# pangenome/gfasort

Measured on AMD Instinct MI355X. Metric: SGD term-updates/sec, -p Y, 1M-node synthetic GFA, higher is better.
Workload: dtype f64

## Files before the change

gfasort_amd/csrc/capi.hip:

```cpp
#include "capi_ctx.h"
#include "index_set.h"
#include "set_seed.h"
#include "set_state_plan.h"

#include <algorithm>
#include <chrono>
#include <cmath>
#include <cstdio>
#include <cstdlib>
#include <cstring>
#include <memory>
#include <new>
#include <numeric>

extern "C" {

const char *gfs_version(void) { return "gfasort_hip 0.1.0 (gfx950)"; }
int gfs_device_count(void) {
    int n = 0;
    if (hipGetDeviceCount(&n) != hipSuccess) return 0;
    return n;
}

int gfs_warmup(int device) {
// ... 39 lines not shown
    c->d_zetas.reset();
    c->d_x.reset();
    c->d_rng.reset();
    c->d_lead.reset();
    c->d_counters.reset();
    c->d_trace.reset();
    c->d_trace_cnt.reset();
    c->d_its.reset();
    c->d_its_all.reset();
    c->d_pool.reset();
    c->configured = false;
}

static int seed_streams(gfs_ctx *c) {
    const uint64_t T = c->shape.n_streams;
    std::vector<uint64_t> st(4 * T);
    for (uint64_t t = 0; t < T; ++t) {
        uint64_t sm = c->params.seed + c->cfg.stream_base + t;
        for (int k = 0; k < 4; ++k) st[(uint64_t)k * T + t] = gfs::splitmix64(sm);
    }
    HIPCHK(hipMemcpy(c->d_rng, st.data(), st.size() * 8, hipMemcpyHostToDevice));
    HIPCHK(hipMemset(c->d_counters, 0, kCounterBytes));
    if (c->d_trace_cnt) HIPCHK(hipMemset(c->d_trace_cnt, 0, T * sizeof(uint32_t)));
    c->events_used = 0; c->kernel_ms_harvested = 0.0; c->iterations = 0; c->total_ms = 0.0;
    return GFS_OK;
}

static int upload_zeta_table(gfs_ctx *c, const gfs_sgd_params *p, const double *zetas) {
    const uint64_t zlen_full = c->shape.zlen_full;
    std::vector<double> ztab;
    if (!zetas) {
        gfs_sgd_params q = *p;
        q.space = gfs::zeta_clamped_space(*p, c->shape.zlen_staged);
        std::vector<double> part(gfs_zeta_table_len(&q));
        gfs_zeta_table(&q, part.data());
        ztab.assign(zlen_full, 0.0);
        std::copy(part.begin(), part.begin() + std::min<size_t>(part.size(), ztab.size()), ztab.begin());
        zetas = ztab.data();
    }
    HIPCHK(c->d_zetas.grow(zlen_full * 8));
    HIPCHK(hipMemcpy(c->d_zetas, zetas, zlen_full * 8, hipMemcpyHostToDevice));
    return GFS_OK;
}

gfs::IterConsts gfs::iter_consts(const gfs_ctx *c, uint64_t k) { return gfs::iter_consts(c->params, c->etas, c->shape, k); }

void gfs::schedule_table(const gfs_sgd_params &p, const std::vector<double> &etas, const gfs::LaunchShape &s, gfs::IterConsts *out) {
    for (uint64_t k = 0; k <= p.iter_max; ++k) out[k] = gfs::iter_consts(p, etas, s, k);
}
static int upload_schedule(gfs_ctx *c) {
    std::vector<gfs::IterConsts> all(c->params.iter_max + 1);
    gfs::schedule_table(c->params, c->etas, c->shape, all.data());
    HIPCHK(hipMemcpy(c->d_its_all, all.data(), all.size() * sizeof(gfs::IterConsts), hipMemcpyHostToDevice));
    return GFS_OK;
}

static const void *iteration_kernel(const gfs::KernelShape &s) {
    if (s.dims == 0) return gfs::iteration_kernel_1d(s);
    if (s.bundle <= 1) return gfs::iteration_kernel_nd(s);
    return s.dims <= 3 ? gfs::iteration_kernel_nd_team(s) : gfs::iteration_kernel_nd_team_wide(s);
}
static const void *fused_kernel(const gfs::KernelShape &s, bool pooled) {
    if (s.dims == 0) return gfs::fused_kernel_1d(s, pooled);
    if (s.bundle <= 1) return gfs::fused_kernel_nd(s, pooled);
    return s.dims <= 3 ? gfs::fused_kernel_nd_team(s, pooled) : gfs::fused_kernel_nd_team_wide(s, pooled);
}
static int resident_blocks_per_cu(const gfs::LaunchShape &s, const void *fn, int *per_cu, std::string *err) {
    hipFuncAttributes attr;
    hipError_t e = hipFuncGetAttributes(&attr, fn);
    if (e != hipSuccess) { *err = std::string("hipFuncGetAttributes(&attr, fn): ") + hipGetErrorString(e); return GFS_E_HIP; }
    e = hipOccupancyMaxActiveBlocksPerMultiprocessor(per_cu, fn, (int)s.block, s.lds_bytes);
    if (e != hipSuccess) { *err = std::string("hipOccupancyMaxActiveBlocksPerMultiprocessor: ") + hipGetErrorString(e); return GFS_E_HIP; }
    return GFS_OK;
}

static hipError_t launch(const gfs_ctx *c, const void *fn, gfs::KArgs &a, const gfs::IterConsts *its, uint32_t n_iters, uint32_t *pool,
                         hipStream_t st) {
    void *args[] = {&a, &its, &n_iters, &pool};
    const gfs::LaunchShape &s = c->shape;
    const dim3 block(s.block), grid((unsigned)((s.n_streams + s.block - 1) / s.block));
    return hipLaunchKernel(fn, grid, block, args, s.lds_bytes, st);
}

static int plan_launches(int cu_count, gfs::LaunchShape &s, LaunchPlan &pl, std::string *err) {
    pl = LaunchPlan{};
    const gfs::KernelShape shape{s.dims, s.bundle, s.lds_tables, s.atomic_loads, s.trace};
    const bool team = s.team, ref = s.bundle == 1;
    const bool free_running = (s.flags & GFS_F_DBG_FREE_RUNNING) != 0;
    pl.iteration = iteration_kernel(shape);
    if (s.phased) pl.window_iteration = iteration_kernel({0, 1, s.lds_tables, s.atomic_loads, s.trace});
    const void *pooled_kernel = s.phased ? gfs::phased_fused_kernel(s.lds_tables) : (team || ref) ? fused_kernel(shape, true) : nullptr;
    const void *free_kernel = team && !s.phased && free_running ? fused_kernel(shape, false) : nullptr;
    if (!pl.iteration || (s.phased && !pl.window_iteration) || ((team || ref) && !pooled_kernel) ||
        (team && !s.phased && free_running && !free_kernel)) {
        *err = "no kernel is built for dims=" + std::to_string(s.dims) + " bundle=" + std::to_string(s.bundle) +
               " lds_tables=" + std::to_string(s.lds_tables) + " atomic_loads=" + std::to_string(s.atomic_loads) +
               " trace=" + std::to_string(s.trace) + " phased=" + std::to_string(s.phased);
        return GFS_E_UNSUPPORTED;
    }
    int per_cu = 0;
    if (team) {
        int rc = resident_blocks_per_cu(s, pooled_kernel, &per_cu, err);
        if (rc) return rc;
    }
    gfs::shape_after_residency(per_cu, gfs::DeviceFacts{cu_count}, &s);
    if (s.fused) pl.fused = s.pooled ? pooled_kernel : free_kernel;
    return GFS_OK;
}

int gfs::plan_setup(const gfs_ctx *c, const gfs_sgd_params *p, int dims, const gfs_launch_config *cfg, const double *etas,
                    gfs::SetupPlan *out, std::string *err) {
    gfs::SetupPlan &sp = *out;
    sp = gfs::SetupPlan{};
    sp.params = *p;
    sp.cfg = cfg ? *cfg : gfs_launch_config{};
    sp.dims = dims;
    sp.rc = GFS_NOTHING_TO_DO;
    if (c->n_nodes == 0) return sp.rc;
    sp.x_len = dims ? c->n_nodes * 2 * (uint64_t)dims : c->n_nodes;
    if (!c->valid_paths) return sp.rc;

    const gfs::GraphFacts graph{c->n_nodes, c->n_steps, c->n_paths, c->max_path_steps, c->valid_paths, c->path_counts.data()};
    int rc = gfs::shape_before_residency(graph, gfs::DeviceFacts{c->cu_count}, p, dims, cfg, &sp.shape, err);
    if (rc) return rc;
    rc = plan_launches(c->cu_count, sp.shape, sp.plan, err);
    if (rc) return rc;
    sp.etas.resize(p->iter_max + 1);
    if (etas) std::copy(etas, etas + p->iter_max + 1, sp.etas.begin());
    else gfs_sgd_schedule(p, sp.etas.data());
    return sp.rc = GFS_OK;
}

void gfs::commit_setup(gfs_ctx *c, gfs::SetupPlan &&sp) {
    const bool has_work = sp.rc == GFS_OK;
    c->params = sp.params; c->cfg = sp.cfg; c->dims = sp.dims; c->x_len = sp.x_len;
    c->shape = has_work ? sp.shape : gfs::LaunchShape{};
    c->plan = has_work ? sp.plan : LaunchPlan{};
    if (!has_work) return;
    c->etas = std::move(sp.etas);
    c->events_used = 0; c->kernel_ms_harvested = 0.0; c->iterations = 0; c->total_ms = 0.0;
}

static int setup_common(gfs_ctx *c, const gfs_sgd_params *p, int dims, const gfs_launch_config *cfg,
                        const double *etas, const double *zetas) {
    if (!c) return fail(GFS_E_ARG, "ctx is null");
    std::string err;
    int rc = gfs::check_setup_args(p, dims, cfg, &err);
    if (rc) return fail(rc, err);
    HIPCHK(hipSetDevice(c->device));
    gfs::free_sgd_state(c);
    gfs::SetupPlan sp;
    const int planned = gfs::plan_setup(c, p, dims, cfg, etas, &sp, &err);
    uint64_t bytes[GFS_STATE_KINDS];
    for (uint32_t k = 0; k < GFS_STATE_KINDS; ++k) bytes[k] = gfs::state_bytes(sp, k);
    gfs::commit_setup(c, std::move(sp));
    if (c->x_len) {
        HIPCHK(c->d_x.grow(bytes[GFS_STATE_POSITIONS]));
        HIPCHK(hipMemset(c->d_x, 0, bytes[GFS_STATE_POSITIONS]));
    }
    if (planned < 0) return fail(planned, err);
    if (planned == GFS_NOTHING_TO_DO) { c->configured = true; return GFS_NOTHING_TO_DO; }

    rc = upload_zeta_table(c, p, zetas);
    if (rc) return rc;
    HIPCHK(c->d_rng.grow(bytes[GFS_STATE_RNG]));
    if (bytes[GFS_STATE_LEAD]) {
        HIPCHK(c->d_lead.grow(bytes[GFS_STATE_LEAD]));
        HIPCHK(hipMemset(c->d_lead, 0, bytes[GFS_STATE_LEAD]));
    }
    HIPCHK(c->d_counters.grow(bytes[GFS_STATE_COUNTERS]));
    if (bytes[GFS_STATE_TRACE]) {
        HIPCHK(c->d_trace.grow(bytes[GFS_STATE_TRACE]));
        HIPCHK(hipMemset(c->d_trace, 0, bytes[GFS_STATE_TRACE]));
        HIPCHK(c->d_trace_cnt.grow(bytes[GFS_STATE_TRACE_COUNTS]));
    }
    rc = seed_streams(c);
    if (rc) return rc;
    if (bytes[GFS_STATE_SCHEDULE]) {
        HIPCHK(c->d_its_all.grow(bytes[GFS_STATE_SCHEDULE]));
        rc = upload_schedule(c);
        if (rc) return rc;
    }
    c->configured = true;
    return GFS_OK;
}

extern "C" {

int gfs_ctx_create(const gfs_graph_view *g, int device, gfs_ctx **out) {
    return gfs_ctx_create_with_layout(g, device, nullptr, out);
}

int gfs_ctx_create_with_layout(const gfs_graph_view *g, int device, const uint32_t *node_perm, gfs_ctx **out) {
    if (!g || !out) return fail(GFS_E_ARG, "null argument");
    *out = nullptr;
    if (int bad = gfs::check_view_counts(g, "")) return bad;
    if (int bad = gfs::check_view_paths(g, "")) return bad;
    int ndev = 0;
    if (hipGetDeviceCount(&ndev) != hipSuccess || ndev == 0)
        return fail(GFS_E_HIP, "no HIP device available (libgfasort_hip has no CPU fallback)");
    if (device < 0 || device >= ndev) return fail(GFS_E_ARG, "bad device index");
    gfs::Laps laps{"gfs_ctx_create", false};
    laps.lap("validate");
    std::unique_ptr<gfs_ctx, decltype(&gfs_ctx_destroy)> owner(new (std::nothrow) gfs_ctx(), gfs_ctx_destroy);
    gfs_ctx *c = owner.get();
    if (!c) return fail(GFS_E_NOMEM, "out of memory");
    c->device = device;
    c->n_nodes = g->n_nodes; c->n_steps = g->n_steps; c->n_paths = g->n_paths;
    hipDeviceProp_t prop;
    if (hipSetDevice(device) != hipSuccess || hipGetDeviceProperties(&prop, device) != hipSuccess)
        return fail(GFS_E_HIP, "hipGetDeviceProperties failed");
    c->cu_count = prop.multiProcessorCount;

    c->perm.assign(g->n_nodes, 0xFFFFFFFFu);
    if (node_perm) {
        std::vector<uint8_t> seen(g->n_nodes, 0);
        for (uint64_t k = 0; k < g->n_nodes; ++k) {
            if (node_perm[k] >= g->n_nodes || seen[node_perm[k]]) return fail(GFS_E_ARG, "node_perm is not a permutation");
            seen[node_perm[k]] = 1; c->perm[k] = node_perm[k];
        }
    }
    if (int bad = gfs::path_facts(g, c, "")) return bad;
    gfs_ctx_set_info info{};
    if (int bad = gfs::build_contexts(&g, &c, 1, c->arena, node_perm, false, &laps, &info)) return bad;
    laps.lap("free tmp");
    *out = owner.release();
    return GFS_OK;
}

void gfs_ctx_destroy(gfs_ctx *c) {
    if (!c || c->set_item) return;
    (void)hipSetDevice(c->device);
    delete c;
// ... 22 lines not shown
    hipError_t e = hipMemcpy(d_stage.p, host, n * 8, hipMemcpyHostToDevice);
    if (e == hipSuccess) e = gfs::reorder_positions_device(d_stage.as<double>(), c->d_x, c->d_perm, c->n_nodes, (uint32_t)c->dims, 1, 0);
    if (e == hipSuccess) e = hipDeviceSynchronize();
    if (e != hipSuccess) return fail(GFS_E_HIP, std::string("upload_positions: ") + hipGetErrorString(e));
    return GFS_OK;
}
int gfs_ctx_init_positions(gfs_ctx *c) {
    if (!c) return fail(GFS_E_ARG, "ctx is null");
    if (!c->d_x || c->dims != 0) return fail(GFS_E_STATE, "needs a 1D context that has been set up");
    HIPCHK(hipSetDevice(c->device));
    HIPCHK(hipDeviceSynchronize());
    hipError_t e = gfs::init_positions_device(c->d_node_len, c->d_perm, c->d_x, c->n_nodes);
    if (e != hipSuccess) return fail(GFS_E_HIP, std::string("init_positions: ") + hipGetErrorString(e));
    return GFS_OK;
}
int gfs_ctx_download_positions(gfs_ctx *c, double *host, uint64_t n) {
    if (!c || !host) return fail(GFS_E_ARG, "null argument");
    if (!c->d_x) return fail(GFS_E_STATE, "context not set up");
    if (n != c->x_len) return fail(GFS_E_ARG, "positions length mismatch");
    HIPCHK(hipSetDevice(c->device));
    HIPCHK(hipDeviceSynchronize());
    gfs::Buffer d_stage;
    if (int rc = d_stage.reserve(n * 8)) return rc;
    hipError_t e = gfs::reorder_positions_device(c->d_x, d_stage.as<double>(), c->d_perm, c->n_nodes, (uint32_t)c->dims, 0, 0);
    if (e == hipSuccess) e = hipMemcpy(host, d_stage.p, n * 8, hipMemcpyDeviceToHost);
    if (e != hipSuccess) return fail(GFS_E_HIP, std::string("download_positions: ") + hipGetErrorString(e));
    return GFS_OK;
}
int gfs_ctx_node_layout(const gfs_ctx *c, uint32_t *perm_out, uint64_t n) {
    if (!c || !perm_out) return fail(GFS_E_ARG, "null argument");
    if (n != c->n_nodes) return fail(GFS_E_ARG, "layout length mismatch");
    std::copy(c->perm.begin(), c->perm.end(), perm_out);
    return GFS_OK;
}
void *gfs_ctx_positions_device(gfs_ctx *c) { return c ? (void *)c->d_x : nullptr; }
int gfs_ctx_bind_positions(gfs_ctx *c, void *device_ptr) {
    if (!c || !device_ptr) return fail(GFS_E_ARG, "null argument");
    if (!c->configured || !c->x_len) return fail(GFS_E_STATE, "context not set up");
    HIPCHK(hipSetDevice(c->device));
    HIPCHK(c->d_x.borrow(device_ptr));
    return GFS_OK;
}
int gfs_ctx_reset_streams(gfs_ctx *c) {
    if (c && c->configured && !c->valid_paths) return GFS_NOTHING_TO_DO;
    if (!c || !c->d_rng) return fail(GFS_E_STATE, "context not set up");
    HIPCHK(hipSetDevice(c->device));
    HIPCHK(hipDeviceSynchronize());
    if (c->d_lead) HIPCHK(hipMemset(c->d_lead, 0, 8 * c->shape.n_streams * sizeof(uint32_t)));
    return seed_streams(c);
}

}

void gfs::fill_kargs(const gfs_ctx *c, gfs::KArgs &a) {
    a.step_rec = c->d_step_rec; a.path_rec = c->d_path_rec; a.path_len = c->d_path_len;
    a.zetas = c->d_zetas; a.x = c->d_x; a.rng = c->d_rng; a.counters = c->d_counters;
    a.trace = c->d_trace; a.trace_cnt = c->d_trace_cnt; a.lead = c->d_lead;
    a.n_steps = c->n_steps;
    const bool wide = gfs::wide_index(c->n_steps, c->cfg.flags);
    a.steps_thresh = wide ? (0ull - c->n_steps) % c->n_steps
                          : (uint64_t)((uint32_t)(0u - (uint32_t)c->n_steps) % (uint32_t)c->n_steps);
    a.n_paths = (uint32_t)c->n_paths;
    a.zlen_full = (uint32_t)c->shape.zlen_full; a.zlen_staged = (uint32_t)c->shape.zlen_staged;
    a.n_streams = (uint32_t)c->shape.n_streams;
    a.quota_base = (uint32_t)(c->shape.quota_total / c->shape.n_streams);
    a.quota_rem = (uint32_t)(c->shape.quota_total % c->shape.n_streams);
    a.attempt_factor = (uint32_t)c->shape.attempt_factor;
    a.trace_per_stream = (uint32_t)c->cfg.trace_per_stream;
    a.space = (uint32_t)std::min<uint64_t>(c->params.space, 0xFFFFFFFFull);
    a.space_max = (uint32_t)std::min<uint64_t>(c->params.space_max, 0xFFFFFFFFull);
    a.space_q = (uint32_t)std::min<uint64_t>(c->params.space_quantization_step, 0xFFFFFFFFull);
    a.dbg = (c->cfg.flags >> 8) & 0x7Fu;
    if (c->cfg.flags & GFS_F_DBG_NO_FUSED_TRIP) a.dbg |= 0x100u;
    a.bundle = c->shape.bundle;
    a.chain = c->shape.chain;
    a.partners = c->shape.partners;
    a.dbg2 = 0;
    if (const char *e = std::getenv("GFS_DBG2")) a.dbg2 = (uint32_t)std::atol(e);
    a.chunk = c->dims ? gfs::ND_TEAM_CHUNK : gfs::TEAM_CHUNK;
    a.ref_chunk = gfs::REF_CHUNK_PER_LANE;
    if (const char *e = std::getenv("GFS_DBG_REF_CHUNK")) { const long v = std::atol(e); if (v >= 1 && v <= 4096) a.ref_chunk = (uint32_t)v; }
    a.n_nodes = (uint32_t)c->n_nodes;
    a.kshift = c->kshift_override >= 0 ? c->kshift_override : gfs::crowd_kshift(c->n_steps, c->shape.n_streams);
}

extern "C" {

static int next_event_pair(gfs_ctx *c, gfs::EventPair *&ev) {
    if (c->events_used == c->events.size()) {
        if (c->events.size() >= 4096) {
            HIPCHK(hipEventSynchronize(c->events.back().e1));
            for (auto &p : c->events) {
                float t = 0.f;
                if (p.elapsed(&t)) c->kernel_ms_harvested += t;
            }
            c->events_used = 0;
        } else {
            c->events.emplace_back();
            if (int rc = c->events.back().ready()) { c->events.pop_back(); return rc; }
        }
    }
    ev = &c->events[c->events_used++];
    return GFS_OK;
}

int gfs_ctx_run_iteration(gfs_ctx *c, uint64_t k, void *hip_stream) {
    if (!c) return fail(GFS_E_ARG, "ctx is null");
    if (!c->configured) return fail(GFS_E_STATE, "context not set up");
    if (!c->valid_paths || c->n_nodes == 0) return GFS_NOTHING_TO_DO;
    if (k > c->params.iter_max) return fail(GFS_E_ARG, "iteration beyond iter_max");
    HIPCHK(hipSetDevice(c->device));
    hipStream_t st = (hipStream_t)hip_stream;
    gfs::KArgs a{};
    fill_kargs(c, a);
    a.it = gfs::iter_consts(c, k);
    const bool window = gfs::in_window(c->shape, k);
    if (window) a.bundle = 1;
    gfs::EventPair *ev = nullptr;
    int rc = next_event_pair(c, ev);
    if (rc) return rc;
    HIPCHK(ev->start(st));
    hipError_t e = launch(c, window ? c->plan.window_iteration : c->plan.iteration, a, nullptr, 0, nullptr, st);
    if (e != hipSuccess) return fail(GFS_E_HIP, std::string("kernel launch: ") + hipGetErrorString(e));
    HIPCHK(ev->stop(st));
    c->iterations++;
    c->launches++;
    return GFS_OK;
}

int gfs_ctx_run_range(gfs_ctx *c, const uint64_t *ks, uint64_t n, void *hip_stream) {
    if (!c || (!ks && n)) return fail(GFS_E_ARG, "null argument");
    if (!c->configured) return fail(GFS_E_STATE, "context not set up");
    if (!c->valid_paths || c->n_nodes == 0) return GFS_NOTHING_TO_DO;
    for (uint64_t i = 0; i < n; ++i) if (ks[i] > c->params.iter_max) return fail(GFS_E_ARG, "iteration beyond iter_max");
    const LaunchPlan &pl = c->plan;
    uint32_t one_chunk = c->shape.one_chunk;
    bool fuse_one = c->shape.fuse_one;
    if (const char *e = std::getenv("GFS_DBG_ONE_CHUNK")) {
        const long v = std::atol(e);
        if (v >= 64 && v <= 4096 && !(v & (v - 1))) { one_chunk = (uint32_t)v; fuse_one = c->shape.fuse_one_probe; }
    }
    if (!pl.fused || n == 0 || (n == 1 && !fuse_one) || n > 0xFFFFFFFFull) {
        for (uint64_t i = 0; i < n; ++i) { int rc = gfs_ctx_run_iteration(c, ks[i], hip_stream); if (rc) return rc; }
        return GFS_OK;
    }
    constexpr uint64_t kMaxFusedIterations = 4096;
    if (n > kMaxFusedIterations) {
        for (uint64_t off = 0; off < n; off += kMaxFusedIterations) {
            const uint64_t m = std::min(kMaxFusedIterations, n - off);
            int rc = m > 1 ? gfs_ctx_run_range(c, ks + off, m, hip_stream) : gfs_ctx_run_iteration(c, ks[off], hip_stream);
            if (rc) return rc;
        }
        return GFS_OK;
    }
    HIPCHK(hipSetDevice(c->device));
    hipStream_t st = (hipStream_t)hip_stream;
    bool consecutive = c->d_its_all != nullptr;
    for (uint64_t i = 1; i < n && consecutive; ++i) consecutive = ks[i] == ks[0] + i;
    const gfs::IterConsts *d_slice = nullptr;
    if (consecutive) {
        d_slice = c->d_its_all + ks[0];
    } else {
        std::vector<gfs::IterConsts> its(n);
        for (uint64_t i = 0; i < n; ++i) its[i] = gfs::iter_consts(c, ks[i]);
        if (int rc = c->d_its.reserve(n * sizeof(gfs::IterConsts))) return rc;
        d_slice = c->d_its.as<gfs::IterConsts>();
        HIPCHK(hipMemcpyAsync(c->d_its.p, its.data(), n * sizeof(gfs::IterConsts), hipMemcpyHostToDevice, st));
        HIPCHK(hipStreamSynchronize(st));
    }
    gfs::KArgs a{};
    fill_kargs(c, a);
    if (n == 1 && c->shape.bundle > 1) a.chunk = one_chunk;
    if (const char *e = std::getenv("GFS_DBG_CHUNK")) {
        const long v = std::atol(e);
        if (c->shape.bundle > 1 && v >= 64 && v <= 16384 && !(v & (v - 1))) a.chunk = (uint32_t)v;
    }
    a.it = gfs::iter_consts(c, ks[0]);
    uint32_t *pool = nullptr;
    if (c->shape.pooled) {
        if (int rc = c->d_pool.reserve(gfs::pool_bytes(n))) return rc;
        pool = c->d_pool.as<uint32_t>();
        HIPCHK(hipMemsetAsync(pool, 0, gfs::pool_bytes(n), st));
    }
    gfs::EventPair *ev = nullptr;
    int rc = next_event_pair(c, ev);
    if (rc) return rc;
    HIPCHK(ev->start(st));
    hipError_t e = launch(c, pl.fused, a, d_slice, (uint32_t)n, pool, st);
    if (e != hipSuccess) return fail(GFS_E_HIP, std::string("fused kernel launch: ") + hipGetErrorString(e));
    HIPCHK(ev->stop(st));
    c->iterations += n;
    c->launches++;
    return GFS_OK;
}

int gfs_ctx_synchronize(gfs_ctx *c, void *hip_stream) {
    if (!c) return fail(GFS_E_ARG, "ctx is null");
    HIPCHK(hipSetDevice(c->device));
    HIPCHK(hipStreamSynchronize((hipStream_t)hip_stream));
    return GFS_OK;
}

int gfs_ctx_run(gfs_ctx *c, void *hip_stream) {
    if (!c) return fail(GFS_E_ARG, "ctx is null");
    if (!c->configured) return fail(GFS_E_STATE, "context not set up");
    if (!c->valid_paths || c->n_nodes == 0) return GFS_NOTHING_TO_DO;
    auto t0 = std::chrono::steady_clock::now();
    {
        std::vector<uint64_t> ks(c->params.iter_max + 1);
        std::iota(ks.begin(), ks.end(), (uint64_t)0);
        int rc = gfs_ctx_run_range(c, ks.data(), ks.size(), hip_stream);
        if (rc) return rc;
    }
    int rc = gfs_ctx_synchronize(c, hip_stream);
    if (rc) return rc;
    c->total_ms += std::chrono::duration<double, std::milli>(std::chrono::steady_clock::now() - t0).count();
    return GFS_OK;
}

int gfs_ctx_stats(gfs_ctx *c, gfs_stats *out) {
    if (!c || !out) return fail(GFS_E_ARG, "null argument");
    std::memset(out, 0, sizeof *out);
    if (!c->d_counters) return GFS_OK;
    HIPCHK(hipSetDevice(c->device));
    HIPCHK(hipDeviceSynchronize());
    std::vector<unsigned long long> cnt(kCounterBytes / 8);
    HIPCHK(hipMemcpy(cnt.data(), c->d_counters, kCounterBytes, hipMemcpyDeviceToHost));
    for (size_t s = 0; s < cnt.size(); s += 8) { out->term_updates += cnt[s]; out->attempts += cnt[s + 1]; }
    out->iterations = c->iterations; out->n_streams = c->shape.n_streams; out->bundle = c->shape.bundle; out->run_trips = c->shape.chain;
    double ms = c->kernel_ms_harvested;
    for (size_t k = 0; k < c->events_used; ++k) {
        float t = 0.f;
        if (c->events[k].elapsed(&t)) ms += t;
    }
    out->kernel_ms = ms; out->total_ms = c->total_ms; out->launches = c->launches;
    return GFS_OK;
}

int gfs_ctx_trace(gfs_ctx *c, gfs_term *out, uint64_t n_terms, uint64_t *counts, uint64_t n_streams) {
    if (!c || !out) return fail(GFS_E_ARG, "null argument");
    if (!c->d_trace) return fail(GFS_E_STATE, "trace_per_stream was 0");
    if (n_terms != c->shape.n_streams * c->cfg.trace_per_stream) return fail(GFS_E_ARG, "trace length mismatch");
    HIPCHK(hipSetDevice(c->device));
    HIPCHK(hipDeviceSynchronize());
    HIPCHK(hipMemcpy(out, c->d_trace, n_terms * sizeof(gfs_term), hipMemcpyDeviceToHost));
    {
        std::vector<uint32_t> inv(c->n_nodes);
        for (uint64_t k = 0; k < c->n_nodes; ++k) inv[c->perm[k]] = (uint32_t)k;
        for (uint64_t t = 0; t < n_terms; ++t) {
            if (c->dims == 0) { if (out[t].d_ij != 0.0) { out[t].i = inv[out[t].i]; out[t].j = inv[out[t].j]; } }
            else if (out[t].d_ij != 0.0) { out[t].i = inv[out[t].i >> 1] * 2 + (out[t].i & 1); out[t].j = inv[out[t].j >> 1] * 2 + (out[t].j & 1); }
        }
    }
    if (counts) {
        if (n_streams != c->shape.n_streams) return fail(GFS_E_ARG, "counts length mismatch");
        std::vector<uint32_t> tmp(c->shape.n_streams);
        HIPCHK(hipMemcpy(tmp.data(), c->d_trace_cnt, tmp.size() * 4, hipMemcpyDeviceToHost));
        for (uint64_t t = 0; t < c->shape.n_streams; ++t) counts[t] = tmp[t];
    }
    return GFS_OK;
}

int gfs_ctx_debug_step_records(const gfs_ctx *c, uint32_t *out, uint64_t n_words) {
    if (!c || !out) return fail(GFS_E_ARG, "null argument");
    if (n_words != 4 * (c->n_steps + 1)) return fail(GFS_E_ARG, "step records length mismatch");
    if (!c->d_step_rec) return fail(GFS_E_STATE, "no step records");
    HIPCHK(hipSetDevice(c->device));
    HIPCHK(hipDeviceSynchronize());
    HIPCHK(hipMemcpy(out, c->d_step_rec, (c->n_steps + 1) * sizeof(uint4), hipMemcpyDeviceToHost));
    return GFS_OK;
}
int gfs_ctx_debug_sgd_state(gfs_ctx *c, uint32_t which, void *out, uint64_t bytes) {
    if (!c) return fail(GFS_E_ARG, "ctx is null");
    const uint32_t kind = which & ~GFS_STATE_SIZE_OF;
    if (kind >= GFS_STATE_KINDS) return fail(GFS_E_ARG, "no such state array");
    if (!c->configured) return fail(GFS_E_STATE, "context not set up");
    const void *arrays[GFS_STATE_KINDS] = {c->d_x.p, c->d_counters.p, c->d_lead.p, c->d_trace.p, c->d_trace_cnt.p, c->d_rng.p, c->d_zetas.p, c->d_its_all.p};
    const uint64_t size = arrays[kind] ? gfs::state_bytes(kind, c->d_rng.p != nullptr, c->x_len, c->shape, c->params, c->cfg) : 0;
    if (which & GFS_STATE_SIZE_OF) {
        if (!out || bytes != sizeof(uint64_t)) return fail(GFS_E_ARG, "the size of a state array is one uint64_t");
        *static_cast<uint64_t *>(out) = size;
        return GFS_OK;
    }
    if (bytes != size) return fail(GFS_E_ARG, "state array length mismatch: it has " + std::to_string(size) + " bytes");
    if (!size) return GFS_OK;
    if (!out) return fail(GFS_E_ARG, "null argument");
    HIPCHK(hipSetDevice(c->device));
    HIPCHK(hipDeviceSynchronize());
    HIPCHK(hipMemcpy(out, arrays[kind], size, hipMemcpyDeviceToHost));
    return GFS_OK;
}
int gfs_ctx_debug_kshift(gfs_ctx *c, int32_t set, int32_t *kshift_out) {
    if (!c) return fail(GFS_E_ARG, "ctx is null");
    if (set >= -1) c->kshift_override = set;
    if (kshift_out) {
        if (!c->configured || !c->shape.n_streams) return fail(GFS_E_STATE, "context not set up");
        gfs::KArgs a{};
        fill_kargs(c, a);
        *kshift_out = a.kshift;
    }
    return GFS_OK;
}

int gfs_ctx_phase_window(gfs_ctx *c, int64_t set_begin, int64_t set_end, uint64_t *begin_out, uint64_t *end_out) {
    if (!c) return fail(GFS_E_ARG, "ctx is null");
    if (!c->configured || !(c->cfg.flags & GFS_F_PHASED)) return fail(GFS_E_STATE, "context not set up with GFS_F_PHASED");
    if (set_begin >= 0 || set_end >= 0) {
        if (set_begin < 0 || set_end < 0 || set_begin > set_end || (uint64_t)set_end > c->params.iter_max + 1)
            return fail(GFS_E_ARG, "phase window: need 0 <= begin <= end <= iter_max + 1");
        if (!c->shape.phased) return fail(GFS_E_STATE, "GFS_F_PHASED is a no-op on this context (the auto policy did not pick bundles of 64)");
        c->shape.win_begin = (uint64_t)set_begin; c->shape.win_end = (uint64_t)set_end;
        if (c->d_its_all) {
            HIPCHK(hipSetDevice(c->device));
            HIPCHK(hipDeviceSynchronize());
            int rc = upload_schedule(c);
            if (rc) return rc;
        }
    }
    if (begin_out) *begin_out = c->shape.win_begin;
    if (end_out) *end_out = c->shape.win_end;
    return GFS_OK;
}

int gfs_ctx_sort_order(gfs_ctx *c, uint64_t *order, uint64_t n) {
    if (!c || (!order && n)) return fail(GFS_E_ARG, "null argument");
    if (!c->d_x || c->dims != 0) return fail(GFS_E_STATE, "needs a 1D context that has been set up");
    if (n != c->n_nodes) return fail(GFS_E_ARG, "order length mismatch");
    HIPCHK(hipSetDevice(c->device));
    HIPCHK(hipDeviceSynchronize());
    gfs::Buffer d_tmp;
    if (int rc = d_tmp.reserve(gfs::sort_order_scratch_bytes(n))) return rc;
    uint32_t *d_order = nullptr;
    hipError_t e = gfs::sort_order_device(c->d_x, c->d_perm, n, 1, d_tmp.p, &d_order);
    if (e != hipSuccess) return fail(GFS_E_HIP, std::string("sort_order_device: ") + hipGetErrorString(e));
    std::vector<uint32_t> tmp(n);
    e = hipMemcpy(tmp.data(), d_order, n * 4, hipMemcpyDeviceToHost);
    if (e != hipSuccess) return fail(GFS_E_HIP, std::string("hipMemcpy order: ") + hipGetErrorString(e));
    for (uint64_t k = 0; k < n; ++k) order[k] = tmp[k];
    return GFS_OK;
}

}

int gfs::check_step_distances(const uint64_t *zs, uint64_t n_z, const gfs_pair_error *out) {
    if ((!zs || !out) && n_z) return fail(GFS_E_ARG, "null argument");
    if (n_z > 65535) return fail(GFS_E_ARG, "at most 65535 step distances per call");
    for (uint64_t k = 0; k < n_z; ++k) if (zs[k] == 0) return fail(GFS_E_ARG, "a step distance of 0");
    return GFS_OK;
}
int gfs::check_diagnosis(uint64_t z, double ratio) {
    if (z == 0) return fail(GFS_E_ARG, "a step distance of 0");
    if (!(ratio >= 0.0)) return fail(GFS_E_ARG, "ratio must be a number >= 0");
    return GFS_OK;
}
gfs_pair_error gfs::unpack_pair_error(uint64_t z, const uint64_t *w) {
    gfs_pair_error o{};
    o.step_distance = z; o.pairs = w[0];
    std::memcpy(&o.sum_rel_sq, &w[1], 8); std::memcpy(&o.max_rel_sq, &w[2], 8);
    std::memcpy(&o.sum_abs, &w[3], 8); std::memcpy(&o.sum_sq, &w[4], 8);
    return o;
}
gfs_sort_quality gfs::unpack_sort_quality(const uint64_t *w) {
    gfs_sort_quality o{w[0], w[1], w[2], 0.0};
    std::memcpy(&o.sq_err_sum, &w[3], 8);
    return o;
}
int gfs::check_sorted_length(uint64_t total_bp, int64_t batch_item) {
    if (total_bp < (1ull << 53)) return GFS_OK;
    return fail(GFS_E_UNSUPPORTED, (batch_item < 0 ? "" : "batch item " + std::to_string(batch_item) + ": ") + "a graph of 2^53 bp or more");
}

extern "C" {

static uint64_t *scratch_words(const gfs_ctx *c, uint64_t part) { return gfs::Region::at<uint64_t>(c->d_quality.p, part); }
static void start_if_timing(gfs::EventPair &timer, hipStream_t st) { if (std::getenv("GFS_TIMING")) (void)timer.start(st); }
static void report_timing(const gfs::EventPair &timer, const char *what, uint64_t count, uint64_t n_steps, const char *before = "z = ", const char *after = "") {
    float ms = 0.f;
    if (timer.elapsed(&ms))
        std::fprintf(stderr, "[%s] %s%llu%s, %llu steps: kernels %.4f ms\n", what, before, (unsigned long long)count, after,
                     (unsigned long long)n_steps, ms);
}

int gfs_ctx_pair_errors(gfs_ctx *c, const uint64_t *zs, uint64_t n_z, gfs_pair_error *out, void *hip_stream) {
    if (!c) return fail(GFS_E_ARG, "ctx is null");
// ... 294 lines not shown
```

gfasort_amd/csrc/capi_ctx.h:

```cpp
#pragma once
#include "../../include/gfasort_hip.h"
#include "device_memory.h"
#include "sgd_kernel_common.h"
#include "launch_policy.h"
#include "sgd_host.h"
#include "readout_region.h"

#include <chrono>
#include <cstdio>
#include <cstdlib>
#include <string>
#include <vector>

static inline int fail(int code, const std::string &msg) { return gfs_set_error(code, msg); }

static_assert(sizeof(gfs_path_error) == 8 * 8, "K7d / K7h write gfs_path_error as 8 words");
static_assert(sizeof(gfs_stretched_pair) == 5 * 8, "K7e / K7i write gfs_stretched_pair as 5 words");
static_assert(sizeof(gfs_node_error) == 3 * 8, "K7f / K7j write gfs_node_error as 3 words");

static constexpr size_t kCounterBytes = gfs::COUNTER_SLOTS * 8 * sizeof(unsigned long long);

struct LaunchPlan {
    const void *iteration = nullptr;
    const void *window_iteration = nullptr;
    const void *fused = nullptr;
};

struct gfs_ctx {
    int device = 0;
    int cu_count = 0;
    uint64_t n_nodes = 0, n_steps = 0, n_paths = 0;
    uint32_t max_path_steps = 0;
    bool valid_paths = false;
    bool set_item = false;
    std::vector<uint32_t> path_counts;
    std::vector<uint32_t> perm;
    gfs::Buffer arena;
    gfs::Array<uint4> d_step_rec;
    gfs::Array<uint4> d_path_rec;
    gfs::Array<uint64_t> d_path_len;
    gfs::Array<uint32_t> d_perm;
    gfs::Array<uint32_t> d_node_len;
    int dims = 0;
    bool configured = false;
    gfs_sgd_params params{};
    gfs_launch_config cfg{};
    std::vector<double> etas;
    gfs::Array<double> d_zetas;
    gfs::Array<double> d_x; uint64_t x_len = 0;
    gfs::Array<uint64_t> d_rng;
    gfs::Array<uint32_t> d_lead;
    gfs::Array<unsigned long long> d_counters;
    gfs::Array<gfs_term> d_trace; gfs::Array<uint32_t> d_trace_cnt;
    gfs::Buffer d_its;
    gfs::Array<gfs::IterConsts> d_its_all;
    gfs::Buffer d_pool;
    gfs::LaunchShape shape;
    LaunchPlan plan;
    int32_t kshift_override = -1;
    gfs::Buffer d_quality;
    std::vector<gfs::EventPair> events;
    size_t events_used = 0;
    double kernel_ms_harvested = 0.0;
    uint64_t iterations = 0;
    uint64_t launches = 0;
    double total_ms = 0.0;
};

namespace gfs {
static inline int check_view_counts(const gfs_graph_view *g, const std::string &prefix) {
    if (g->n_steps > (1ull << 40)) return fail(GFS_E_UNSUPPORTED, prefix + "more than 2^40 path steps");
    if (g->n_nodes > 0x7FFFFFFFull) return fail(GFS_E_UNSUPPORTED, prefix + "more than 2^31-1 nodes");
    if (g->n_paths > 0x7FFFFFFFull) return fail(GFS_E_UNSUPPORTED, prefix + "more than 2^31-1 paths");
    if (g->n_steps && (!g->step_node || !g->step_is_rev)) return fail(GFS_E_ARG, prefix + "null step arrays");
    if (!g->path_first_step) return fail(GFS_E_ARG, prefix + "null path_first_step");
    if (g->n_nodes && !g->node_len) return fail(GFS_E_ARG, prefix + "null node_len");
    return GFS_OK;
}
static inline int check_view_paths(const gfs_graph_view *g, const std::string &prefix) {
    if (g->path_first_step[0] != 0 || g->path_first_step[g->n_paths] != g->n_steps)
        return fail(GFS_E_ARG, prefix + "path_first_step must start at 0 and end at n_steps");
    for (uint64_t p = 0; p < g->n_paths; ++p)
        if (g->path_first_step[p + 1] < g->path_first_step[p]) return fail(GFS_E_ARG, prefix + "path_first_step not monotone");
    return GFS_OK;
}
static inline int path_facts(const gfs_graph_view *g, gfs_ctx *c, const std::string &prefix) {
    c->path_counts.reserve(g->n_paths);
    for (uint64_t p = 0; p < g->n_paths; ++p) {
        const uint64_t b = g->path_first_step[p], e = g->path_first_step[p + 1];
        if (e - b > 0xFFFFFFFFull) return fail(GFS_E_UNSUPPORTED, prefix + "a path with more than 2^32-1 steps");
        const uint32_t cnt = (uint32_t)(e - b);
        c->path_counts.push_back(cnt);
        if (cnt > 1) c->valid_paths = true;
        if (cnt > c->max_path_steps) c->max_path_steps = cnt;
    }
    uint32_t max_len = 0;
    for (uint64_t k = 0; k < g->n_nodes; ++k) if (g->node_len[k] > max_len) max_len = g->node_len[k];
    for (uint64_t p = 0; p < g->n_paths; ++p) {
        const uint64_t b = g->path_first_step[p], e = g->path_first_step[p + 1];
        if ((unsigned __int128)(e - b) * max_len < ((unsigned __int128)1 << 55)) continue;
        unsigned __int128 bp = 0;
        for (uint64_t s = b; s < e; ++s) { const uint32_t n = g->step_node[s]; if (n < g->n_nodes) bp += g->node_len[n]; }
        if (bp >= ((unsigned __int128)1 << 55)) return fail(GFS_E_UNSUPPORTED, prefix + "a path of 2^55 bp or more");
    }
    return GFS_OK;
}
}

namespace gfs {
struct Laps {
    const char *tag;
    bool cumulative;
    bool on = std::getenv("GFS_TIMING") != nullptr;
    std::chrono::steady_clock::time_point t = std::chrono::steady_clock::now();
    void lap(const char *what) {
        if (!on) return;
        const auto now = std::chrono::steady_clock::now();
        std::fprintf(stderr, cumulative ? "[%s] %-10s %8.2f ms\n" : "[%s] %-12s %8.2f ms\n", tag, what,
                     std::chrono::duration<double, std::milli>(now - t).count());
        if (!cumulative) t = now;
    }
// ... 50 lines not shown
```

gfasort_amd/csrc/capi_set.hip:

```cpp
#include "capi_ctx.h"
#include "index_set.h"
#include "set_seed.h"
#include "set_state_plan.h"

#include <algorithm>
#include <chrono>
#include <cstring>
#include <memory>
#include <new>

struct gfs_ctx_set {
    int device = 0;
    gfs::Buffer arena;
    gfs::Buffer state_arena;
    gfs::Buffer h_stage{true};
    std::vector<std::unique_ptr<gfs_ctx>> items;
    gfs_ctx_set_info info{};
    gfs_ctx_set_setup_info setup_info{};
};

namespace {
constexpr int KINDS = gfs::SET_KINDS;
std::string item_prefix(uint64_t i) { return "set item " + std::to_string(i) + ": "; }
}

int gfs::build_contexts(const gfs_graph_view *const *graphs, gfs_ctx *const *ctxs, uint64_t n, gfs::Buffer &arena, const uint32_t *node_perm,
                        bool staged, gfs::Laps *laps, gfs_ctx_set_info *info) {
    const std::string set = staged ? "set " : "";
    auto lap = [laps](const char *what) { if (laps && laps->on) { (void)hipDeviceSynchronize(); laps->lap(what); } };
    int rc = GFS_OK;
    auto ok = [&rc, &set](const char *call, const char *what, hipError_t err) {
        if (err != hipSuccess) rc = fail(GFS_E_HIP, std::string(call) + " " + set + what + ": " + hipGetErrorString(err));
        return err == hipSuccess;
    };
    std::vector<uint64_t> counts(3 * n), offsets(KINDS * n);
    uint64_t N = 0, S = 0, P = 0;
    for (uint64_t i = 0; i < n; ++i) {
        counts[i] = ctxs[i]->n_nodes; counts[n + i] = ctxs[i]->n_steps; counts[2 * n + i] = ctxs[i]->n_paths;
        N += ctxs[i]->n_nodes; S += ctxs[i]->n_steps; P += ctxs[i]->n_paths;
    }
    const uint64_t arena_bytes = gfs::set_arena_plan(counts.data(), counts.data() + n, counts.data() + 2 * n, n, offsets.data());
    const uint64_t perm_begin = offsets[3], nlen_begin = offsets[4];
    const uint64_t perm_bytes = nlen_begin - perm_begin, nlen_bytes = arena_bytes - nlen_begin;

    const gfs::SetInputHead in = gfs::set_input_head(S, P, n);
    uint64_t work_bytes = 0;
    hipError_t e = gfs::index_set_work_bytes(N, S, &work_bytes);
    if (e != hipSuccess) return fail(GFS_E_HIP, std::string("rocPRIM temporary storage: ") + hipGetErrorString(e));
    gfs::Buffer h_stage{true}, d_scratch;
    if ((rc = arena.reserve(std::max<uint64_t>(arena_bytes, 256), ("hipMalloc " + set + "arena").c_str()))) return rc;
    if ((rc = d_scratch.reserve(in.bytes + work_bytes, ("hipMalloc " + set + "scratch").c_str()))) return rc;
    if (staged && (rc = h_stage.reserve(std::max(in.bytes + nlen_bytes, perm_bytes), "hipHostMalloc set staging"))) return rc;
    info->device_allocations = staged ? 3 : 2;
    if (!ok("hipMemset", "arena", hipMemsetAsync(arena.p, 0, std::max<uint64_t>(arena_bytes, 256), 0))) return rc;
    ++info->launches;

    std::vector<gfs::SetItem> items(n + 1);
    uint64_t node_off = 0, step_off = 0, path_off = 0;
    for (uint64_t i = 0; i <= n; ++i) {
        items[i] = gfs::SetItem{node_off, step_off, path_off, 0, 0, 0, 0, 0};
        if (i == n) break;
        const uint64_t *at = &offsets[KINDS * i];
        items[i].rec = at[0]; items[i].prec = at[1]; items[i].plen = at[2]; items[i].perm = at[3]; items[i].nlen = at[4];
        node_off += ctxs[i]->n_nodes; step_off += ctxs[i]->n_steps; path_off += ctxs[i]->n_paths;
    }
    unsigned char *h = h_stage.as<unsigned char>(), *d_in = d_scratch.as<unsigned char>(), *d_arena = arena.as<unsigned char>();
    if (staged) {
        auto *h_step_node = reinterpret_cast<uint32_t *>(h);
        auto *h_first = reinterpret_cast<uint64_t *>(h + in.at_first);
        uint8_t *h_rev = h + in.at_rev;
        unsigned char *h_nlen = h + in.bytes;
        std::memset(h_nlen, 0, nlen_bytes);
        for (uint64_t i = 0; i < n; ++i) {
            const gfs_graph_view *g = graphs[i];
            const gfs::SetItem &it = items[i];
            if (g->n_steps) {
                std::memcpy(h_step_node + it.step_off, g->step_node, g->n_steps * 4);
                std::memcpy(h_rev + it.step_off, g->step_is_rev, g->n_steps);
            }
            for (uint64_t p = 0; p < g->n_paths; ++p) h_first[it.path_off + p] = it.step_off + g->path_first_step[p];
            if (g->n_nodes) std::memcpy(h_nlen + (it.nlen - nlen_begin), g->node_len, g->n_nodes * 4);
        }
        h_first[P] = S;
        std::memcpy(h + in.at_items, items.data(), items.size() * sizeof(gfs::SetItem));
        if (!ok("hipMemcpy", "inputs", hipMemcpyAsync(d_in, h, in.bytes, hipMemcpyHostToDevice, 0))) return rc;
        if (nlen_bytes && !ok("hipMemcpy", "node_len", hipMemcpyAsync(d_arena + nlen_begin, h_nlen, nlen_bytes, hipMemcpyHostToDevice, 0))) return rc;
    } else {
        const gfs_graph_view *g = graphs[0];
        if (N && !ok("hipMemcpy", "node_len", hipMemcpy(d_arena + nlen_begin, g->node_len, N * 4, hipMemcpyHostToDevice))) return rc;
        if (S && !ok("hipMemcpy", "step_node", hipMemcpy(d_in, g->step_node, S * 4, hipMemcpyHostToDevice))) return rc;
        if (!ok("hipMemcpy", "path_first", hipMemcpy(d_in + in.at_first, g->path_first_step, (P + 1) * 8, hipMemcpyHostToDevice))) return rc;
        if (!ok("hipMemcpy", "item table", hipMemcpy(d_in + in.at_items, items.data(), items.size() * sizeof(gfs::SetItem), hipMemcpyHostToDevice))) return rc;
        if (S && !ok("hipMemcpy", "step_is_rev", hipMemcpy(d_in + in.at_rev, g->step_is_rev, S, hipMemcpyHostToDevice))) return rc;
        if (N && node_perm && !ok("hipMemcpy", "perm", hipMemcpy(d_arena + perm_begin, ctxs[0]->perm.data(), N * 4, hipMemcpyHostToDevice))) return rc;
    }
    lap("step upload");

    gfs::SetUnion u{};
    u.n_items = (uint32_t)n; u.n_nodes = N; u.n_steps = S; u.n_paths = P;
    u.step_node = reinterpret_cast<const uint32_t *>(d_in);
    u.path_first = reinterpret_cast<const uint64_t *>(d_in + in.at_first);
    u.items = reinterpret_cast<const gfs::SetItem *>(d_in + in.at_items);
    u.step_is_rev = d_in + in.at_rev;
    u.arena = d_arena;
    uint32_t bad_item = gfs::SET_NO_BAD_ITEM;
    e = gfs::index_set_layout_device(u, d_in + in.bytes, node_perm != nullptr, &bad_item, &info->launches);
    lap("node layout");
    if (e == hipSuccess && bad_item == gfs::SET_NO_BAD_ITEM) e = gfs::index_set_records_device(u, d_in + in.bytes, &info->launches);
    if (e != hipSuccess || bad_item != gfs::SET_NO_BAD_ITEM) (void)hipDeviceSynchronize();
    if (e != hipSuccess) return fail(GFS_E_HIP, std::string("build_index_set: ") + hipGetErrorString(e));
    if (bad_item != gfs::SET_NO_BAD_ITEM) return fail(GFS_E_ARG, (staged ? item_prefix(bad_item) : "") + "step_node out of range");
    if (staged) {
        if (!ok("hipMemcpy", "perm", hipMemcpy(h, d_arena + perm_begin, std::max<uint64_t>(perm_bytes, 4), hipMemcpyDeviceToHost))) return rc;
    } else if (N && !node_perm) {
        if (!ok("hipMemcpy", "perm", hipMemcpy(ctxs[0]->perm.data(), d_arena + perm_begin, N * 4, hipMemcpyDeviceToHost))) return rc;
    }
    if ((e = hipDeviceSynchronize()) != hipSuccess) return fail(GFS_E_HIP, std::string("hipDeviceSynchronize: ") + hipGetErrorString(e));
    lap("K3");
    for (uint64_t i = 0; i < n; ++i) {
        gfs_ctx *c = ctxs[i];
        const uint64_t *at = &offsets[KINDS * i];
        if (staged) {
            const uint32_t *perm = reinterpret_cast<const uint32_t *>(h + (at[3] - perm_begin));
            c->perm.assign(perm, perm + c->n_nodes);
        }
        (void)c->d_step_rec.borrow(d_arena + at[0]);
        (void)c->d_path_rec.borrow(d_arena + at[1]);
        (void)c->d_path_len.borrow(d_arena + at[2]);
        (void)c->d_perm.borrow(d_arena + at[3]);
        (void)c->d_node_len.borrow(d_arena + at[4]);
    }
    info->items = n; info->total_nodes = N; info->total_steps = S; info->total_paths = P;
    info->arena_bytes = arena_bytes;
    return GFS_OK;
}

static int set_setup(gfs_ctx_set *s, const std::vector<const gfs_sgd_params *> &params, const std::vector<int> &dims,
                     const gfs_launch_config *cfgs, int32_t *item_rc) {
    const auto t0 = std::chrono::steady_clock::now();
    const uint64_t n = s->items.size();
    std::string err;
    for (uint64_t i = 0; i < n; ++i) {
        if (dims[i] < 0) return fail(GFS_E_UNSUPPORTED, item_prefix(i) + "dimensions must be 1..8");
        if (int rc = gfs::check_setup_args(params[i], dims[i], cfgs ? &cfgs[i] : nullptr, &err)) return fail(rc, item_prefix(i) + err);
    }
    HIPCHK(hipSetDevice(s->device));

    std::vector<gfs::SetupPlan> plans(n);
    for (uint64_t i = 0; i < n; ++i) {
        const int rc = gfs::plan_setup(s->items[i].get(), params[i], dims[i], cfgs ? &cfgs[i] : nullptr, nullptr, &plans[i], &err);
        if (rc < 0) return fail(rc, item_prefix(i) + err);
    }
    constexpr int K = gfs::SET_STATE_KINDS;
    std::vector<uint64_t> bytes(K * n), offsets(K * n);
    gfs_ctx_set_setup_info info{};
    info.items = n;
    std::vector<gfs::SeedItem> seeds;
    std::vector<uint64_t> seed_of;
    uint64_t total_blocks = 0;
    for (uint64_t i = 0; i < n; ++i) {
        const gfs::SetupPlan &sp = plans[i];
        for (int k = 0; k < K; ++k) bytes[K * i + k] = gfs::state_bytes(sp, (uint32_t)k);
        if (sp.rc != GFS_OK) { ++info.nothing_to_do; continue; }
        ++info.configured;
        info.total_streams += sp.shape.n_streams;
        seeds.push_back(gfs::SeedItem{nullptr, sp.params.seed + sp.cfg.stream_base, (uint32_t)sp.shape.n_streams, (uint32_t)total_blocks});
        seed_of.push_back(i);
        total_blocks += (sp.shape.n_streams + gfs::SEED_BLOCK - 1) / gfs::SEED_BLOCK;
        if (total_blocks > 0x7FFFFFFFull) return fail(GFS_E_UNSUPPORTED, "set items 0.." + std::to_string(i) + " have more streams together than one seeding launch holds");
    }
    const uint64_t arrays_end = gfs::set_state_plan(bytes.data(), n, offsets.data());
    const uint64_t zero_end = gfs::set_state_kind_begin(offsets.data(), GFS_STATE_RNG);
    const uint64_t upload_begin = gfs::set_state_kind_begin(offsets.data(), GFS_STATE_ZETAS);
    const uint64_t seeds_at = arrays_end, blocks_at = seeds_at + gfs::round256(seeds.size() * sizeof(gfs::SeedItem));
    const uint64_t arena_bytes = blocks_at + gfs::round256(total_blocks * sizeof(uint32_t)), stage_bytes = arena_bytes - upload_begin;
    info.state_bytes = arena_bytes;

    HIPCHK(hipDeviceSynchronize());
    for (auto &c : s->items) gfs::free_sgd_state(c.get());
    int rc = GFS_OK;
    auto ok = [&rc, s](const char *what, hipError_t e) {
        if (e == hipSuccess) return true;
        (void)hipDeviceSynchronize();
        s->state_arena.reset();
        rc = fail(GFS_E_HIP, std::string(what) + ": " + hipGetErrorString(e));
        return false;
    };
    if (s->state_arena.bytes < arena_bytes) {
        ++info.device_allocations;
        if ((rc = s->state_arena.reserve(arena_bytes, "hipMalloc set state arena"))) return rc;
    }
    if (s->h_stage.bytes < stage_bytes) {
        ++info.device_allocations;
        if ((rc = s->h_stage.reserve(stage_bytes, "hipHostMalloc set state staging"))) { s->state_arena.reset(); return rc; }
    }
    unsigned char *d_arena = s->state_arena.as<unsigned char>(), *h = s->h_stage.as<unsigned char>();
    auto staged = [h, upload_begin](uint64_t arena_offset) { return h + (arena_offset - upload_begin); };

    if (stage_bytes) std::memset(h, 0, stage_bytes);
    {
        std::vector<gfs_sgd_params> clamped(n);
// ... 158 lines not shown
```

gfasort_amd/csrc/index_set.h:

```cpp
#pragma once
#include "index_set_plan.h"
#include <hip/hip_runtime.h>
#include <stdint.h>

namespace gfs {

struct SetItem {
    uint64_t node_off, step_off, path_off;
    uint64_t rec, prec, plen, perm, nlen;
};
static_assert(sizeof(SetItem) == SET_ITEM_BYTES, "the item table of the input head (index_set_plan.h)");

struct SetUnion {
    uint32_t n_items;
    uint64_t n_nodes, n_steps, n_paths;
    const SetItem *items;
    const uint32_t *step_node;
    const uint8_t *step_is_rev;
    const uint64_t *path_first;
    unsigned char *arena;
};

constexpr uint32_t SET_NO_BAD_ITEM = 0xFFFFFFFFu;
constexpr unsigned SET_STEP_BLOCKS = 2048, SET_NODE_BLOCKS = 1024, SET_PATH_BLOCKS = 64, SET_BLOCK = 256;

hipError_t index_set_work_bytes(uint64_t n_nodes, uint64_t n_steps, uint64_t *bytes);
hipError_t index_set_layout_device(const SetUnion &u, void *d_work, bool layout_given, uint32_t *bad_item, uint64_t *launches);
hipError_t index_set_records_device(const SetUnion &u, void *d_work, uint64_t *launches);
hipError_t warm_module_index_set();

}
```

gfasort_amd/csrc/index_set_kernels.hip:

```cpp
#include "index_set.h"
#include "device_memory.h"
#include <hip/hip_runtime.h>
#include <algorithm>
#include <stdint.h>
#include <type_traits>
#include <rocprim/device/device_radix_sort.hpp>
#include <rocprim/device/device_scan.hpp>
#include <rocprim/iterator/counting_iterator.hpp>
#include <rocprim/iterator/transform_iterator.hpp>

namespace gfs {

constexpr uint32_t NO_NODE_U32 = 0xFFFFFFFFu;
constexpr unsigned KEY_BITS = 43;
constexpr int JUMP_ROUNDS = 40, JUMP_CHUNK = 4;

__host__ __device__ __forceinline__ uint32_t item_of(const SetItem *items, uint32_t n_items, uint64_t v, uint64_t SetItem::*off) {
    uint32_t lo = 0, hi = n_items;
    while (hi - lo > 1) { const uint32_t mid = lo + ((hi - lo) >> 1); if (items[mid].*off <= v) lo = mid; else hi = mid; }
    return lo;
}
__host__ __device__ __forceinline__ uint32_t path_of(const uint64_t *path_first, uint32_t n_paths, uint64_t s) {
    uint32_t lo = 0, hi = n_paths;
    while (hi - lo > 1) { const uint32_t mid = lo + ((hi - lo) >> 1); if (path_first[mid] <= s) lo = mid; else hi = mid; }
// ... 26 lines not shown
        ids[v] = (uint32_t)v;
    }
}
__global__ void set_run_up_kernel(SetUnion u, const unsigned long long *first, uint32_t *up) {
    const uint64_t stride = (uint64_t)gridDim.x * blockDim.x;
    for (uint64_t v = (uint64_t)blockIdx.x * blockDim.x + threadIdx.x; v < u.n_nodes; v += stride) {
        const unsigned long long f = first[v];
        uint32_t w = (uint32_t)v;
        if (f != ~0ull && !set_is_path_start(u.path_first, (uint32_t)u.n_paths, f)) {
            const uint32_t p = u.step_node[f - 1];
            if (p != NO_NODE_U32) {
                const uint64_t q = u.items[item_of(u.items, u.n_items, v, &SetItem::node_off)].node_off + p;
                if (first[q] == f - 1) w = (uint32_t)q;
            }
        }
        up[v] = w;
    }
}
__global__ void set_jump_kernel(const uint32_t *in, uint32_t *out, uint64_t n_nodes, uint32_t *changed) {
    const uint64_t stride = (uint64_t)gridDim.x * blockDim.x;
    for (uint64_t v = (uint64_t)blockIdx.x * blockDim.x + threadIdx.x; v < n_nodes; v += stride) {
        const uint32_t a = in[v], b = in[a];
        out[v] = b;
        if (b != a) *changed = 1;
    }
}
__global__ void set_anchor_kernel(SetUnion u, const unsigned long long *first, const uint32_t *head, uint32_t *anc) {
    const uint64_t stride = (uint64_t)gridDim.x * blockDim.x;
    for (uint64_t v = (uint64_t)blockIdx.x * blockDim.x + threadIdx.x; v < u.n_nodes; v += stride) {
        uint32_t a = (uint32_t)v;
        if (first[v] != ~0ull) {
            const unsigned long long fh = first[head[v]];
            if (!set_is_path_start(u.path_first, (uint32_t)u.n_paths, fh)) {
                const uint32_t p = u.step_node[fh - 1];
                if (p != NO_NODE_U32) a = (uint32_t)(u.items[item_of(u.items, u.n_items, v, &SetItem::node_off)].node_off + p);
            }
        }
        anc[v] = a;
    }
}
__global__ void set_branch_key_kernel(SetUnion u, const unsigned long long *first, const uint32_t *root, const uint32_t *ids_by_first,
                                      unsigned long long *key) {
    const uint64_t stride = (uint64_t)gridDim.x * blockDim.x;
    for (uint64_t r = (uint64_t)blockIdx.x * blockDim.x + threadIdx.x; r < u.n_nodes; r += stride) {
        const uint32_t v = ids_by_first[r];
        const unsigned long long f = first[v];
        const uint32_t t = root[v];
        key[r] = f == ~0ull ? unvisited_key(u.items, item_of(u.items, u.n_items, v, &SetItem::node_off))
                            : (t == v ? 4ull * (f + 1ull) : 4ull * (first[t] + 1ull) + 1ull);
    }
}
__global__ void set_scatter_rank_kernel(SetUnion u, const uint32_t *sorted_node) {
    const uint64_t stride = (uint64_t)gridDim.x * blockDim.x;
    for (uint64_t r = (uint64_t)blockIdx.x * blockDim.x + threadIdx.x; r < u.n_nodes; r += stride) {
        const uint64_t v = sorted_node[r];
        const SetItem it = u.items[item_of(u.items, u.n_items, v, &SetItem::node_off)];
        reinterpret_cast<uint32_t *>(u.arena + it.perm)[v - it.node_off] = (uint32_t)(r - it.node_off);
    }
}

struct SetStepLen {
    SetUnion u;
    __host__ __device__ uint64_t operator()(uint64_t s) const {
        if (s >= u.n_steps) return 0;
        const uint32_t n = u.step_node[s];
        if (n == NO_NODE_U32) return 0ull;
        const SetItem &it = u.items[item_of(u.items, u.n_items, s, &SetItem::step_off)];
        return (uint64_t)reinterpret_cast<const uint32_t *>(u.arena + it.nlen)[n];
    }
};
__global__ void set_node_stats_kernel(SetUnion u, uint32_t *cnt, uint32_t *rep) {
    const uint64_t stride = (uint64_t)gridDim.x * blockDim.x;
    for (uint64_t s = (uint64_t)blockIdx.x * blockDim.x + threadIdx.x; s < u.n_steps; s += stride) {
        const uint32_t n = u.step_node[s];
        if (n == NO_NODE_U32) continue;
        const uint64_t v = u.items[item_of(u.items, u.n_items, s, &SetItem::step_off)].node_off + n;
        atomicAdd(&cnt[v], 1u);
        const uint64_t begin = u.path_first[path_of(u.path_first, (uint32_t)u.n_paths, s)], from = s - begin > 63 ? s - 63 : begin;
        uint32_t c = 1;
        for (uint64_t t = from; t < s; ++t) c += u.step_node[t] == n;
        if (c > 1 && rep[v] < c) atomicMax(&rep[v], c);
    }
}
__global__ void set_fill_records_kernel(SetUnion u, const uint64_t *scan, const uint32_t *cnt, const uint32_t *rep) {
    const uint64_t stride = (uint64_t)gridDim.x * blockDim.x;
    for (uint64_t s = (uint64_t)blockIdx.x * blockDim.x + threadIdx.x; s < u.n_steps; s += stride) {
        const uint32_t p = path_of(u.path_first, (uint32_t)u.n_paths, s);
        const SetItem it = u.items[item_of(u.items, u.n_items, s, &SetItem::step_off)];
        const uint64_t pos = scan[s] - scan[u.path_first[p]];
        const uint32_t n = u.step_node[s];
        uint4 r;
        r.x = n == NO_NODE_U32 ? NO_NODE_U32 : reinterpret_cast<const uint32_t *>(u.arena + it.perm)[n];
        uint32_t crowd = 0;
        if (n != NO_NODE_U32) {
            const uint32_t a = set_ceil_log2(cnt[it.node_off + n]), b = set_ceil_log2(rep[it.node_off + n]);
            crowd = ((a > 63u ? 63u : a) << 23) | ((b > 7u ? 7u : b) << 29);
        }
        r.y = (uint32_t)(p - it.path_off) | ((uint32_t)(u.step_is_rev[s] & 1) << 31);
        r.z = (uint32_t)pos; r.w = ((uint32_t)(pos >> 32) & 0x7FFFFFu) | crowd;
        reinterpret_cast<uint4 *>(u.arena + it.rec)[s - it.step_off] = r;
    }
}
__global__ void set_paths_kernel(SetUnion u, const uint64_t *scan) {
    const uint64_t stride = (uint64_t)gridDim.x * blockDim.x, total = u.n_paths + u.n_items;
    for (uint64_t t = (uint64_t)blockIdx.x * blockDim.x + threadIdx.x; t < total; t += stride) {
        if (t >= u.n_paths) {
            const uint32_t i = (uint32_t)(t - u.n_paths);
            reinterpret_cast<uint4 *>(u.arena + u.items[i].rec)[u.items[i + 1].step_off - u.items[i].step_off] = make_uint4(0, 0, 0, 0);
            continue;
        }
        const SetItem it = u.items[item_of(u.items, u.n_items, t, &SetItem::path_off)];
        const uint64_t fb = u.path_first[t], fe = u.path_first[t + 1], b = fb - it.step_off;
        const uint32_t c = (uint32_t)(fe - fb);
        reinterpret_cast<uint4 *>(u.arena + it.prec)[t - it.path_off] = make_uint4((uint32_t)b, c, c ? (uint32_t)(0u - c) % c : 0u, (uint32_t)(b >> 32));
        reinterpret_cast<uint64_t *>(u.arena + it.plen)[t - it.path_off] = scan ? scan[fe] - scan[fb] : 0ull;
    }
}

namespace {
struct Work {
    unsigned long long *first, *key_a, *key_b;
    uint32_t *ids_a, *ids_b, *a, *b, *cnt, *rep;
    uint64_t *scan;
    uint32_t *flags;
    void *tmp;
    size_t tmp_bytes;
    uint64_t cnt_rep_bytes, bytes;
};
hipError_t plan_work(uint64_t N, uint64_t S, void *d_work, Work &w) {
    size_t sort_tmp = 0, scan_tmp = 0;
    hipError_t e = hipSuccess;
    if (N) e = rocprim::radix_sort_pairs(nullptr, sort_tmp, (uint64_t *)nullptr, (uint64_t *)nullptr, (uint32_t *)nullptr, (uint32_t *)nullptr,
                                         (size_t)N, 0, KEY_BITS, 0);
    if (e != hipSuccess) return e;
    if (S) {
        auto lens = rocprim::make_transform_iterator(rocprim::counting_iterator<uint64_t>(0), SetStepLen{SetUnion{}});
        e = rocprim::exclusive_scan(nullptr, scan_tmp, lens, (uint64_t *)nullptr, (uint64_t)0, (size_t)(S + 1), rocprim::plus<uint64_t>(), 0);
        if (e != hipSuccess) return e;
    }
    const uintptr_t base = reinterpret_cast<uintptr_t>(d_work);
    uint64_t at = 0;
    auto take = [&at, base](auto *&piece, uint64_t bytes) {
        piece = reinterpret_cast<std::remove_reference_t<decltype(piece)>>(base + at);
        at += round256(bytes ? bytes : 1);
    };
    take(w.first, N * 8); take(w.key_a, N * 8); take(w.key_b, N * 8);
    take(w.ids_a, N * 4); take(w.ids_b, N * 4); take(w.a, N * 4); take(w.b, N * 4);
    take(w.cnt, N * 4); take(w.rep, N * 4);
    w.cnt_rep_bytes = round256(N ? N * 4 : 1) + N * 4;
    take(w.scan, S ? (S + 1) * 8 : 0);
    take(w.flags, (1 + 2 * JUMP_ROUNDS) * sizeof(uint32_t));
    w.tmp_bytes = std::max(sort_tmp, scan_tmp);
    take(w.tmp, w.tmp_bytes);
    w.bytes = at;
    return hipSuccess;
}
const dim3 over_steps(SET_STEP_BLOCKS), over_nodes(SET_NODE_BLOCKS), block(SET_BLOCK);
}

hipError_t index_set_work_bytes(uint64_t n_nodes, uint64_t n_steps, uint64_t *bytes) {
    Work w{};
    const hipError_t e = plan_work(n_nodes, n_steps, nullptr, w);
    *bytes = w.bytes;
    return e;
}

hipError_t index_set_layout_device(const SetUnion &u, void *d_work, bool layout_given, uint32_t *bad_item, uint64_t *launches) {
    *bad_item = SET_NO_BAD_ITEM;
    const uint64_t N = u.n_nodes, S = u.n_steps;
    Work w{};
    hipError_t e = plan_work(N, S, d_work, w);
    if (e != hipSuccess) return e;
    if ((e = hipMemsetAsync(w.flags, 0xFF, sizeof(uint32_t), 0)) != hipSuccess) return e;
    if ((e = hipMemsetAsync(w.flags + 1, 0, 2 * JUMP_ROUNDS * sizeof(uint32_t), 0)) != hipSuccess) return e;
    *launches += 2;
    if (N) {
        if ((e = hipMemsetAsync(w.first, 0xFF, N * 8, 0)) != hipSuccess) return e;
        ++*launches;
    }
    if (S) {
        hipLaunchKernelGGL(set_first_visit_kernel, over_steps, block, 0, 0, u, w.first, w.flags);
        ++*launches;
        if ((e = hipMemcpy(bad_item, w.flags, sizeof(uint32_t), hipMemcpyDeviceToHost)) != hipSuccess) return e;
        if (*bad_item != SET_NO_BAD_ITEM) return hipSuccess;
    }
    if (!N || layout_given) return hipGetLastError();
    hipLaunchKernelGGL(set_first_key_kernel, over_nodes, block, 0, 0, u, w.first, w.key_a, w.ids_a);
    e = rocprim::radix_sort_pairs(w.tmp, w.tmp_bytes, (uint64_t *)w.key_a, (uint64_t *)w.key_b, w.ids_a, w.ids_b, (size_t)N, 0, KEY_BITS, 0);
    *launches += 2;
    if (e != hipSuccess) return e;
    uint32_t *d_ids = w.ids_b, *d_ids_other = w.ids_a;
    if (S) {
        uint32_t *d_a = w.a, *d_b = w.b;
        auto jump_to_fixpoint = [&](uint32_t *&cur, uint32_t *&other, uint32_t *flags) -> hipError_t {
            for (int round = 0; round < JUMP_ROUNDS; round += JUMP_CHUNK) {
                for (int k = 0; k < JUMP_CHUNK; ++k) {
                    hipLaunchKernelGGL(set_jump_kernel, over_nodes, block, 0, 0, cur, other, N, flags + round + k);
                    std::swap(cur, other);
                }
                *launches += JUMP_CHUNK;
                uint32_t changed[JUMP_CHUNK];
                const hipError_t err = hipMemcpy(changed, flags + round, sizeof changed, hipMemcpyDeviceToHost);
                if (err != hipSuccess) return err;
                if (std::find(changed, changed + JUMP_CHUNK, 0u) != changed + JUMP_CHUNK) break;
            }
            return hipSuccess;
        };
        hipLaunchKernelGGL(set_run_up_kernel, over_nodes, block, 0, 0, u, w.first, d_a);
        ++*launches;
        if ((e = jump_to_fixpoint(d_a, d_b, w.flags + 1)) != hipSuccess) return e;
        hipLaunchKernelGGL(set_anchor_kernel, over_nodes, block, 0, 0, u, w.first, d_a, d_b);
        std::swap(d_a, d_b);
        ++*launches;
        if ((e = jump_to_fixpoint(d_a, d_b, w.flags + 1 + JUMP_ROUNDS)) != hipSuccess) return e;
        hipLaunchKernelGGL(set_branch_key_kernel, over_nodes, block, 0, 0, u, w.first, d_a, d_ids, w.key_a);
        e = rocprim::radix_sort_pairs(w.tmp, w.tmp_bytes, (uint64_t *)w.key_a, (uint64_t *)w.key_b, d_ids, d_ids_other, (size_t)N, 0, KEY_BITS, 0);
        *launches += 2;
        if (e != hipSuccess) return e;
        std::swap(d_ids, d_ids_other);
    }
    hipLaunchKernelGGL(set_scatter_rank_kernel, over_nodes, block, 0, 0, u, d_ids);
    ++*launches;
    return hipGetLastError();
}

hipError_t index_set_records_device(const SetUnion &u, void *d_work, uint64_t *launches) {
    const uint64_t N = u.n_nodes, S = u.n_steps;
    Work w{};
    hipError_t e = plan_work(N, S, d_work, w);
    if (e != hipSuccess) return e;
    if (S) {
        auto lens = rocprim::make_transform_iterator(rocprim::counting_iterator<uint64_t>(0), SetStepLen{u});
        e = rocprim::exclusive_scan(w.tmp, w.tmp_bytes, lens, w.scan, (uint64_t)0, (size_t)(S + 1), rocprim::plus<uint64_t>(), 0);
        if (e != hipSuccess) return e;
        if ((e = hipMemsetAsync(w.cnt, 0, w.cnt_rep_bytes, 0)) != hipSuccess) return e;
        hipLaunchKernelGGL(set_node_stats_kernel, over_steps, block, 0, 0, u, w.cnt, w.rep);
        hipLaunchKernelGGL(set_fill_records_kernel, over_steps, block, 0, 0, u, w.scan, w.cnt, w.rep);
        *launches += 4;
    }
    hipLaunchKernelGGL(set_paths_kernel, dim3(SET_PATH_BLOCKS), block, 0, 0, u, S ? w.scan : (const uint64_t *)nullptr);
    ++*launches;
    return hipGetLastError();
}

hipError_t warm_module_index_set() {
    hipFuncAttributes attr;
    return hipFuncGetAttributes(&attr, reinterpret_cast<const void *>(&set_paths_kernel));
}

}
```

gfasort_amd/csrc/launch_policy.h:

```cpp
#pragma once
#include "../../include/gfasort_hip.h"
#include "sgd_limits.h"

#include <algorithm>
#include <cmath>
#include <cstdint>
#include <string>
#include <vector>

namespace gfs {

struct GraphFacts {
    uint64_t n_nodes = 0, n_steps = 0, n_paths = 0;
    uint32_t max_path_steps = 0;
    bool valid_paths = false;
    const uint32_t *path_counts = nullptr;
};
struct DeviceFacts { int cu_count = 0; };

struct LaunchShape {
    int dims = 0;
    uint32_t flags = 0;
    bool trace = false, explicit_streams = false;
    uint32_t block = 256;
    uint64_t n_streams = 0, quota_total = 0, attempt_factor = 0;
    uint32_t bundle = 1;
    uint32_t partners = 1;
    uint32_t chain = 1;
    bool phased = false;
    uint64_t win_begin = 0, win_end = 0;
    bool lds_tables = true, atomic_loads = true;
    size_t lds_bytes = 0;
    uint64_t zlen_full = 0, zlen_staged = 0;
    bool team = false;
    uint64_t fused_resident_blocks = 0;
    bool fused = false;
    bool pooled = false;
    bool fuse_one = false;
    bool fuse_one_probe = false;
    uint32_t one_chunk = 0;
};

inline bool has_fused_team_kernel(int dims, uint32_t bundle) { return (dims == 0 && bundle >= 16) || (dims >= 2 && bundle == 64); }

inline int check_setup_args(const gfs_sgd_params *p, int dims, const gfs_launch_config *cfg, std::string *err) {
    if (!p) { *err = "params is null"; return GFS_E_ARG; }
    if (!(p->theta >= 0.0 && p->theta < 1.0)) { *err = "theta must be in [0,1)"; return GFS_E_ARG; }
    if (p->space_quantization_step == 0) { *err = "space_quantization_step must be > 0"; return GFS_E_ARG; }
    if (!(p->eta_max > 0.0)) { *err = "eta_max must be > 0"; return GFS_E_ARG; }
    if (dims < 0 || dims > GFS_MAX_DIMS) { *err = "dimensions must be 1..8"; return GFS_E_UNSUPPORTED; }
    if (cfg && (cfg->flags & GFS_F_PHASED)) {
        if (dims != 0) { *err = "GFS_F_PHASED is a sampler of the 1D sort: layouts have none"; return GFS_E_ARG; }
        const uint32_t b = (cfg->flags >> 16) & 0xFFu;
        if (b != 0 && b != 64) { *err = "GFS_F_PHASED switches between reference streams and bundles of 64: GFS_F_BUNDLE must be 0 or 64"; return GFS_E_ARG; }
    }
    return GFS_OK;
}

inline uint64_t auto_stream_count(const GraphFacts &g, const DeviceFacts &dev, int dims, uint64_t quota_total, bool team) {
    const uint64_t chip = (uint64_t)dev.cu_count * ((team && dims == 0) ? 1024 : (team && dims >= 2) ? 256u * (unsigned)nd_team_waves(dims) : 976);
    const uint64_t by_work = ((quota_total + 7) / 8 + 63) / 64 * 64;
    const uint64_t by_nodes = (team ? g.n_nodes * 3 / 4 : g.n_nodes / 4) / 64 * 64;
    return std::max<uint64_t>(64, std::min(chip, std::min(by_work, by_nodes)));
}

inline int choose_bundle(const GraphFacts &g, int dims, uint32_t flags, LaunchShape *s, std::string *err) {
    uint32_t b = (flags >> 16) & 0xFFu;
    const bool b_auto = b == 0;
    if (b > 1 && (s->n_streams % 64 != 0 || (b != 4 && b != 8 && b != 16 && b != 32 && b != 64))) {
        *err = "bundled sampling needs n_streams % 64 == 0 and a bundle of 4, 8, 16, 32 or 64"; return GFS_E_ARG;
    }
    if (b > 1 && dims != 0 && b == 4) { *err = "bundled layout kernels exist for 1..8 dimensions and bundles of 8..64"; return GFS_E_UNSUPPORTED; }
    if (b == 0) {
        b = 1;
        if (s->n_streams % 64 == 0 && dims <= 3 && g.n_nodes >= 16384) {
            for (uint32_t cand : {64u, 32u, 16u, 8u, 4u}) {
                if (cand == 4u && dims != 0) continue;
                uint64_t long_steps = 0;
                for (uint64_t p = 0; p < g.n_paths; ++p) if (g.path_counts[p] >= 4 * cand) long_steps += g.path_counts[p];
                if ((double)long_steps >= 0.95 * (double)g.n_steps) { b = cand; break; }
            }
        }
    }
    s->bundle = b;
    uint32_t k = (flags >> 24) & 0xFFu;
    if (k > 64 || (k & (k - 1))) { *err = "GFS_F_CHAIN: the run length in trips must be a power of two <= 64"; return GFS_E_ARG; }
    const bool k_auto = k == 0;
    if (k == 0) k = dims ? 16 : 64;
    s->partners = (b == 64 && has_fused_team_kernel(dims, b) && !(flags & GFS_F_ONE_PARTNER)) ? 2u : 1u;
    if (k_auto && b_auto && b == 64) while (k > 1 && s->quota_total / (64ull * k * s->partners) < 64) k >>= 1;
    s->chain = b == 64 ? k : 1;
    return GFS_OK;
}

inline int shape_before_residency(const GraphFacts &g, const DeviceFacts &dev, const gfs_sgd_params *p, int dims, const gfs_launch_config *cfg_in,
                                  LaunchShape *shape, std::string *err) {
    int rc = check_setup_args(p, dims, cfg_in, err);
    if (rc) return rc;
    if (g.n_nodes == 0 || !g.valid_paths) return GFS_NOTHING_TO_DO;
    const gfs_launch_config cfg = cfg_in ? *cfg_in : gfs_launch_config{};
    LaunchShape s;
    s.dims = dims; s.flags = cfg.flags; s.trace = cfg.trace_per_stream != 0; s.explicit_streams = cfg.n_streams != 0;

    s.zlen_full = gfs_zeta_table_len(p);
    if (s.zlen_full > 0xFFFFFFFFull) { *err = "zeta table too long"; return GFS_E_UNSUPPORTED; }
    const uint64_t maxjump = std::min<uint64_t>(p->space, g.max_path_steps ? g.max_path_steps - 1 : 0);
    const uint64_t last_idx = maxjump > p->space_max
                                  ? p->space_max + (maxjump - p->space_max) / p->space_quantization_step + 1
                                  : maxjump;
    s.zlen_staged = std::min<uint64_t>(last_idx + 1, s.zlen_full);

    s.quota_total = cfg.term_updates_per_iteration ? cfg.term_updates_per_iteration : p->min_term_updates;
    s.block = cfg.block_size ? cfg.block_size : 256;
    if (s.block % 64 || s.block > 1024) { *err = "block_size must be a multiple of 64, <= 1024"; return GFS_E_ARG; }
    s.n_streams = cfg.n_streams ? cfg.n_streams : auto_stream_count(g, dev, dims, s.quota_total, false);
    if (s.n_streams > 0x7FFFFFFFull) { *err = "n_streams too large"; return GFS_E_ARG; }
    if (s.quota_total / s.n_streams + 1 > 0xFFFFFFFFull) { *err = "per-stream quota exceeds 2^32"; return GFS_E_UNSUPPORTED; }
    s.attempt_factor = cfg.attempt_factor ? cfg.attempt_factor : 64;
    if (s.attempt_factor > 0xFFFFFFFFull) { *err = "attempt_factor too large"; return GFS_E_ARG; }
    rc = choose_bundle(g, dims, cfg.flags, &s, err);
    if (rc) return rc;
    if (!cfg.n_streams && s.bundle > 1) s.n_streams = auto_stream_count(g, dev, dims, s.quota_total, true);
    if (cfg.flags & GFS_F_PHASED) {
        s.phased = s.bundle == 64;
        if (s.phased) gfs_phase_window(p, &s.win_begin, &s.win_end);
        else if (s.bundle == 1) { s.win_begin = 0; s.win_end = p->iter_max + 1; }
    }
    if (dims != 0 && s.bundle > 1 && s.block > 256) { *err = "the layout team kernels are built for workgroups of at most 256 lanes"; return GFS_E_ARG; }
    s.atomic_loads = !(cfg.flags & GFS_F_PLAIN_LOADS);
    const size_t lds = (size_t)g.n_paths * 16 + (size_t)s.zlen_staged * 8;
    s.lds_tables = !(cfg.flags & GFS_F_NO_LDS_TABLES) && lds <= 48 * 1024;
    s.lds_bytes = s.lds_tables ? lds : 0;
    s.team = has_fused_team_kernel(dims, s.bundle);
    *shape = s;
    return GFS_OK;
}

inline void shape_after_residency(int per_cu, const DeviceFacts &dev, LaunchShape *shape) {
    LaunchShape &s = *shape;
    const bool ref = s.bundle == 1;
    const bool free_running = (s.flags & GFS_F_DBG_FREE_RUNNING) != 0;
    s.fused_resident_blocks = 0;
    if (s.team) {
        s.fused_resident_blocks = (uint64_t)std::max(per_cu, 0) * dev.cu_count;
        const uint64_t resident = s.fused_resident_blocks * s.block;
        if (!s.explicit_streams && s.n_streams > resident && resident >= 64) s.n_streams = resident;
    }
    const uint64_t n_waves = (s.n_streams + 63) / 64;
    const bool pool_ok = n_waves <= 0xFFFFFFFFull &&
                         s.quota_total / (s.dims != 0 && s.bundle > 1 ? 1u : pool_slots((uint32_t)n_waves)) < (1ull << 31);
    const bool team_fusable = s.team && (s.phased ? pool_ok && !free_running : pool_ok || free_running) &&
                              (s.n_streams + s.block - 1) / s.block <= s.fused_resident_blocks;
    s.pooled = pool_ok && !(free_running && s.bundle > 1);
    s.fused = (team_fusable || (ref && pool_ok)) && s.atomic_loads && !s.trace && !(s.flags & GFS_F_NO_FUSE);
    s.one_chunk = s.dims ? ND_TEAM_CHUNK : TEAM_CHUNK;
    s.fuse_one_probe = team_fusable && pool_ok;
    s.fuse_one = s.fuse_one_probe && s.dims != 0 && s.quota_total / n_waves >= 4ull * s.one_chunk;
}

inline bool in_window(const LaunchShape &s, uint64_t k) { return s.phased && k >= s.win_begin && k < s.win_end; }

inline IterConsts iter_consts(const gfs_sgd_params &p, const std::vector<double> &etas, const LaunchShape &s, uint64_t k) {
    IterConsts it;
    double fc = std::floor(p.cooling_start * (double)p.iter_max);
    uint64_t first_cooling = !(fc > 0.0) ? 0 : (fc >= 18446744073709551616.0 ? UINT64_MAX : (uint64_t)fc);
    bool cooling = k > first_cooling;
    double theta = cooling ? 0.001 : p.theta;
    it.eta = etas[k];
    it.cooling = cooling ? 1 : 0;
    it.zeta2theta = 1.0 + gfs_fast_precise_pow(0.5, theta);
    double omt = 1.0 - theta;
    it.omt_e = h_sat_i32(omt); it.omt_fb = omt - (double)it.omt_e;
    double alpha = 1.0 / (1.0 - theta);
    it.alpha_e = h_sat_i32(alpha); it.alpha_fb = alpha - (double)it.alpha_e;
    it._pad = in_window(s, k) ? 1 : 0;
    return it;
}

inline int32_t crowd_kshift(uint64_t n_steps, uint64_t n_streams) {
    const uint64_t per = n_steps / std::max<uint64_t>(2 * n_streams, 1);
    int lg = 0; while (lg < 63 && (per >> (lg + 1)) != 0) ++lg;
    return lg + 2;
}

inline bool wide_index(uint64_t n_steps, uint32_t flags) { return n_steps > 0xFFFFFFFFull || (flags & GFS_F_DBG_WIDE_INDEX); }

inline bool batch_eligible(const LaunchShape &s, bool trace, bool has_resident_schedule, bool idle) {
    return !idle && s.bundle == 1 && !s.phased && s.fused && s.pooled && !trace && has_resident_schedule;
}

}
```

gfasort_amd/csrc/sgd_1d.h:

```cpp
#pragma once
#include "sgd_kernel_common.h"

namespace gfs {

struct RefTerm1D { uint32_t i, j; int crowd; double term_dist; };

template <bool LDS_TABLES>
__device__ __forceinline__ bool ref_sample_1d(const KArgs &a, const uint4 *path_tab, const double *zeta_tab, Rng &rng,
                                              const uint64_t step_idx, const uint4 &ra, RefTerm1D &t) {
    uint4 rb; uint64_t sa, sb; uint32_t cnt, path;
    if (!sample_pair_from<LDS_TABLES>(a, path_tab, zeta_tab, rng, step_idx, ra, rb, sa, sb, cnt, path)) return false;
    t.term_dist = fabs(rec_pos(ra) - rec_pos(rb));
    if (t.term_dist == 0.0) return false;
    t.crowd = crowd_shift<false>(a, ra, rb);
    t.i = ra.x; t.j = rb.x;
    return t.i != 0xFFFFFFFFu && t.j != 0xFFFFFFFFu;
}

template <bool LDS_TABLES, bool ATOMIC_LOADS, bool TRACE>
__device__ __forceinline__ void ref_run_1d(const KArgs &a, const uint4 *path_tab, const double *zeta_tab, Rng &rng,
                                           const uint32_t quota, const uint64_t max_att, const uint32_t tid,
                                           uint32_t &done, uint32_t &att, uint32_t &ntr) {
    double *x = a.x;
    uint32_t d = 0; uint64_t t = 0;
    uint64_t s_a = 0; uint4 r_a = make_uint4(0, 0, 0, 0); bool drawn = false;
    while (d < quota && t < max_att) {
        ++t;
        if (!drawn) { s_a = sample_step(a, rng); r_a = a.step_rec[s_a]; }
        drawn = false;
        RefTerm1D cur;
        if (!ref_sample_1d<LDS_TABLES>(a, path_tab, zeta_tab, rng, s_a, r_a, cur)) continue;
        const double mu = crowd_scale(fmin(a.it.eta * (1.0 / cur.term_dist), 1.0), cur.crowd);
        double dx;
        if (a.dbg & 2u) dx = (double)cur.i - (double)cur.j;
        else dx = load_pos<ATOMIC_LOADS>(x + cur.i) - load_pos<ATOMIC_LOADS>(x + cur.j);
        if (dx == 0.0) dx = 1e-9;
        const double mag = fabs(dx);
        const double delta = mu * (mag - cur.term_dist) / 2.0;
        const double r = delta / mag;
        const double r_x = r * dx;
        if (d + 1u < quota && t < max_att) { s_a = sample_step(a, rng); r_a = a.step_rec[s_a]; drawn = true; }
        if (a.dbg & 1u) { asm volatile("" :: "v"(r_x)); }
        else {
            add_pos(x + cur.i, -r_x);
            add_pos(x + cur.j, r_x);
        }
        ++d;
        if (TRACE) record_trace(a, tid, ntr, cur.i, cur.j, cur.term_dist);
    }
    done += d;
    att += t > 0xFFFFFFFFull ? 0xFFFFFFFFu : (uint32_t)t;
}

struct TeamState {
    Rng rng;
    Leader L = {0, 0, 0, 0, 0, 0, 0, 0};
    uint32_t left = 0, cool = 0, colour = 0, seg = 0;
    uint32_t p = 0;
    uint32_t done = 0, att = 0, ntr = 0;
};

struct Trip {
    uint64_t sa = 0, sb = 0;
    uint4 ra = make_uint4(0, 0, 0, 0), rb = make_uint4(0, 0, 0, 0);
    uint4 rc = make_uint4(0, 0, 0, 0);
    bool twin = false;
    bool valid = false;
    int mshift = 0;
    bool two = false;
    bool fused = false;
    uint32_t k = 1;
    uint32_t off = 0;
};

template <int B>
__device__ __forceinline__ void expand_trip(const KArgs &a, const Leader &L, int t, uint32_t seg, uint32_t p, uint32_t colour, int sub, int q, Trip &tr) {
    constexpr int RUNS = 64 / B;
    const int ll = t * RUNS + q;
    const uint32_t okw = bcast<B>(L.ok, ll), cnt = bcast<B>(L.cnt, ll);
    const uint32_t ok = leader_ok(okw, p);
    const uint32_t ra0 = p ? bcast<B>(L.ra1, ll) : bcast<B>(L.ra0, ll), rb0 = p ? bcast<B>(L.rb1, ll) : bcast<B>(L.rb0, ll);
    const uint64_t first = bcast_first<B>(L, ll);
    tr.k = (B == 64 && ((okw | (okw >> 8)) & 1u) && cnt >= 2u * B) ? run_trips(a.chain, (uint32_t)B, cnt) : 1u;
    tr.off = B == 64 ? run_offset((uint32_t)B, cnt, tr.k, ra0, rb0, seg) : 0u;
    tr.mshift = merged_trip_shift<B>(ok, cnt, ra0, rb0, tr.off);
    const bool two = !(a.dbg & 0x08u) && two_colour<B>(ok, cnt, ra0, rb0);
    tr.two = B == 64 ? two : (__any(two) != 0);
    tr.ra = make_uint4(0, 0, 0, 0); tr.rb = make_uint4(0, 0, 0, 0); tr.rc = make_uint4(0, 0, 0, 0);
    tr.fused = B == 64 && tr.mshift != 0 && colour == 0 && two && !(a.dbg & 0x100u);
    tr.twin = B == 64 && p == 0u && a.partners == 2u && (okw & 3u) == 3u && ((okw >> 8) & 3u) == 3u && !(a.dbg & 0x04u);
    const uint32_t rb1 = bcast<B>(L.rb1, ll);
    if (tr.twin) {
        const int64_t gap = (int64_t)rb0 - (int64_t)rb1, lim = 192;
        if (gap < lim && gap > -lim) tr.twin = false;
    }
    if (tr.twin) {
        tr.sa = first + ra0 + tr.off + (uint32_t)sub;
        tr.sb = first + rb0 + tr.off + (((uint32_t)sub + ((okw >> 2) & 7u)) & 63u);
        const uint64_t sc = first + rb1 + tr.off + (((uint32_t)sub + ((okw >> 10) & 7u)) & 63u);
        tr.valid = true;
        tr.ra = a.step_rec[tr.sa]; tr.rb = a.step_rec[tr.sb]; tr.rc = a.step_rec[sc];
        return;
    }
    if (tr.fused) {
        const int dst = sub + tr.mshift;
        tr.sa = first + merged_trip_base(cnt, ra0, tr.off) + (uint32_t)sub;
        tr.sb = (uint64_t)((int64_t)tr.sa + tr.mshift);
        tr.valid = dst < 0 || dst > 63;
        tr.ra = a.step_rec[tr.sa];
        tr.rb = a.step_rec[tr.sb];
        return;
    }
    tr.valid = expand_run<B>(ok, first, cnt, ra0, rb0, sub, colour, tr.off, tr.sa, tr.sb);
    if (tr.valid) { tr.ra = a.step_rec[tr.sa]; tr.rb = a.step_rec[tr.sb]; }
}

__device__ __forceinline__ double term_move(const KArgs &a, double term_dist, double xi, double xj, int crowd) {
    double mu = crowd_scale(fmin(a.it.eta * (1.0 / term_dist), 1.0), crowd);
    double dx = xi - xj;
    if (dx == 0.0) dx = 1e-9;
    double mag = fabs(dx);
    double delta = mu * (mag - term_dist) / 2.0;
    double r = delta / mag;
    return r * dx;
}

__device__ __forceinline__ double shfl_f64(double v, int src) { return __shfl(v, src, 64); }

template <bool ATOMIC_LOADS, bool TRACE>
__device__ __forceinline__ bool fused_trip(const KArgs &a, TeamState &ts, const Trip &cur, const int lane,
                                           const uint32_t tid, const uint64_t wave_quota, uint64_t &wave_done) {
    double *x = a.x;
    const int s = cur.mshift, z = s < 0 ? -s : s;
    const int dst = lane + s, src = lane - s;
    const bool out = cur.valid;
    const int dstc = out ? lane : dst, srcc = (src < 0 || src > 63) ? lane : src;
    const uint32_t grp = ((cur.off + (uint32_t)lane) / (uint32_t)z) & 1u;
    const uint32_t node = cur.ra.x, pnode = cur.rb.x;
    double xo = 0.0, xp = 0.0;
    if (!(a.dbg & 2u)) {
        if (node != 0xFFFFFFFFu) xo = load_pos<ATOMIC_LOADS>(x + node);
        if (out && pnode != 0xFFFFFFFFu) xp = load_pos<ATOMIC_LOADS>(x + pnode);
    } else { xo = (double)node; xp = (double)pnode; }
    const double term_dist = fabs(rec_pos(cur.ra) - rec_pos(cur.rb));
    const int crowd = crowd_shift<true>(a, cur.ra, cur.rb);
    const bool term_ok = term_dist != 0.0 && node != 0xFFFFFFFFu && pnode != 0xFFFFFFFFu;
    double acc = 0.0;
    bool touched = false, second = true;
#pragma unroll
    for (uint32_t colour = 0; colour < 2u; ++colour) {
        ++ts.att;
        const bool valid = quota_cut(term_ok && grp == colour, lane, wave_quota, wave_done);
        const double xpart_in = shfl_f64(xo, dstc);
        const double xj = out ? xp : xpart_in;
        double r_x = 0.0;
        if (valid) {
            r_x = term_move(a, term_dist, xo, xj, crowd);
            ++ts.done;
            if (TRACE) record_trace(a, tid, ts.ntr, node, pnode, term_dist);
        }
        const double rv = shfl_f64(r_x, srcc);
        const int vsrc = __shfl((int)valid, srcc, 64);
        const bool recv = src >= 0 && src <= 63 && vsrc != 0;
        if (valid) xo = xo - r_x;
        if (recv) xo = xo + rv;
        if (valid) { acc = touched ? acc - r_x : -r_x; touched = true; }
        if (recv) { acc = touched ? acc + rv : rv; touched = true; }
        if (valid && out && !(a.dbg & 1u)) add_pos(x + pnode, r_x);
        if (colour == 0 && wave_done >= wave_quota) { second = false; break; }
    }
    if (touched && !(a.dbg & 1u)) add_pos(x + node, acc);
    return second;
}

template <bool ATOMIC_LOADS, bool TRACE>
__device__ __forceinline__ bool twin_trip(const KArgs &a, TeamState &ts, const Trip &cur, const int lane,
                                          const uint32_t tid, const uint64_t wave_quota, uint64_t &wave_done) {
    double *x = a.x;
    const uint32_t node = cur.ra.x, nb = cur.rb.x, nc = cur.rc.x;
    double xa = 0.0, xb = 0.0, xc = 0.0;
    if (!(a.dbg & 2u)) {
        if (node != 0xFFFFFFFFu) xa = load_pos<ATOMIC_LOADS>(x + node);
        if (nb != 0xFFFFFFFFu) xb = load_pos<ATOMIC_LOADS>(x + nb);
        if (nc != 0xFFFFFFFFu) xc = load_pos<ATOMIC_LOADS>(x + nc);
    } else { xa = (double)node; xb = (double)nb; xc = (double)nc; }
    const double pa = rec_pos(cur.ra);
    double acc = 0.0;
    bool touched = false, second = true;
#pragma unroll
    for (uint32_t p = 0; p < 2u; ++p) {
        ++ts.att;
        const uint4 &rp = p ? cur.rc : cur.rb;
        const uint32_t pn = p ? nc : nb;
        const double term_dist = fabs(pa - rec_pos(rp));
        const bool valid = quota_cut(term_dist != 0.0 && node != 0xFFFFFFFFu && pn != 0xFFFFFFFFu,
                                     lane, wave_quota, wave_done);
        if (valid) {
            const double r_x = term_move(a, term_dist, xa, p ? xc : xb, crowd_shift<true>(a, cur.ra, rp));
            ++ts.done;
            if (TRACE) record_trace(a, tid, ts.ntr, node, pn, term_dist);
            xa = xa - r_x;
            acc = touched ? acc - r_x : -r_x; touched = true;
            if (!(a.dbg & 1u)) add_pos(x + pn, r_x);
        }
        if (p == 0u && wave_done >= wave_quota) { second = false; break; }
    }
    if (touched && !(a.dbg & 1u)) add_pos(x + node, acc);
    return second;
}

template <int B, bool LDS_TABLES, bool ATOMIC_LOADS, bool TRACE>
__device__ __forceinline__ void team_iteration(const KArgs &a, const uint4 *path_tab, const double *zeta_tab,
                                               TeamState &ts, const uint32_t tid, const uint64_t wave_quota, const IterConsts *itp = nullptr) {
    const int lane = threadIdx.x & 63;
    const int sub = lane & (B - 1);
    const int q = lane / B;
    const uint64_t max_passes = (uint64_t)a.attempt_factor * (wave_quota / (64u * B) + 1u) + 16u;
    uint64_t wave_done = 0, passes = 0;
    double *x = a.x;
    while (wave_done < wave_quota && passes < max_passes) {
        if (ts.left == 0 || ts.cool != (uint32_t)a.it.cooling) {
            ++passes;
            KArgs as;
            reload_kargs(as);
            if (itp) {
                const IterConsts *ip = itp;
                asm volatile("" : "+s"(ip));
                as.it = *ip;
            }
            ts.L = sample_leader<LDS_TABLES>(as, path_tab, zeta_tab, ts.rng);
            ts.left = B; ts.cool = (uint32_t)a.it.cooling; ts.colour = 0; ts.seg = 0; ts.p = 0;
        }
        const Leader &L = ts.L;
        int t = B - (int)ts.left;
        uint32_t colour = ts.colour, seg = ts.seg, p = ts.p;
        Trip cur;
        expand_trip<B>(a, L, t, seg, p, colour, sub, q, cur);
        for (;;) {
            int t_n = t; uint32_t colour_n = 0u, seg_n = seg, p_n = p;
            if (colour == 0 && cur.two && !cur.fused) colour_n = 1u;
            else if (p == 0u && a.partners == 2u && !cur.twin) p_n = 1u;
            else if (seg + 1u < cur.k) { seg_n = seg + 1u; p_n = 0u; }
            else { t_n = t + 1; seg_n = 0u; p_n = 0u; }
            const bool have_n = t_n < B;
            Trip nxt;
            if (have_n) expand_trip<B>(a, L, t_n, seg_n, p_n, colour_n, sub, q, nxt);
            if (B == 64 && cur.twin) {
                if (!twin_trip<ATOMIC_LOADS, TRACE>(a, ts, cur, lane, tid, wave_quota, wave_done)) {
                    ts.colour = 0u; ts.seg = seg; ts.p = 1u;
                    break;
                }
                ts.colour = 0u; ts.seg = seg_n; ts.p = 0u;
                if (t_n != t) --ts.left;
                if (wave_done >= wave_quota || !have_n) break;
                cur = nxt; t = t_n; colour = colour_n; seg = seg_n; p = p_n;
                continue;
            }
            if (B == 64 && cur.fused) {
                if (!fused_trip<ATOMIC_LOADS, TRACE>(a, ts, cur, lane, tid, wave_quota, wave_done)) {
                    ts.colour = 1u; ts.seg = seg; ts.p = p;
                    break;
                }
                ts.colour = 0u; ts.seg = seg_n; ts.p = p_n;
                if (t_n != t) --ts.left;
                if (wave_done >= wave_quota || !have_n) break;
                cur = nxt; t = t_n; colour = colour_n; seg = seg_n; p = p_n;
                continue;
            }
            ++ts.att;
            ts.colour = colour_n; ts.seg = seg_n; ts.p = p_n;
            if (t_n != t) --ts.left;
            bool valid = cur.valid;
            const uint4 ra = cur.ra, rb = cur.rb;
            const int mshift = cur.mshift;
            double term_dist = 0.0;
            uint32_t i = 0, j = 0;
            if (valid) {
                term_dist = fabs(rec_pos(ra) - rec_pos(rb));
                i = ra.x; j = rb.x;
                valid = term_dist != 0.0 && i != 0xFFFFFFFFu && j != 0xFFFFFFFFu;
            }
            valid = quota_cut(valid, lane, wave_quota, wave_done);
            double xi = 0.0, xj = 0.0;
            if (valid) {
                if (a.dbg & 2u) { xi = (double)i; xj = (double)j; }
                else { xi = load_pos<ATOMIC_LOADS>(x + i); xj = load_pos<ATOMIC_LOADS>(x + j); }
            }
            double r_x = 0.0;
            if (valid) {
                r_x = term_move(a, term_dist, xi, xj, crowd_shift<true>(a, ra, rb));
                ++ts.done;
                if (TRACE) record_trace(a, tid, ts.ntr, i, j, term_dist);
            }
            bool o1f = valid, o2f = valid; uint32_t o1s = i, o2s = j; double o1v = -r_x, o2v = r_x;
            if (B == 64 && mshift != 0) {
                const int z = mshift < 0 ? -mshift : mshift;
                const int src = lane - mshift;
                const int srcc = src < 0 ? 0 : (src > 63 ? 63 : src);
                const double rv = __shfl(r_x, srcc, 64);
                const uint32_t js = (uint32_t)__shfl((int)j, srcc, 64);
                const int vs = __shfl((int)valid, srcc, 64);
                const bool resting = (((cur.off + (uint32_t)lane) / (uint32_t)z) & 1u) != colour;
                if (resting && src >= 0 && src < 64 && vs) { o1f = true; o1s = js; o1v = rv; }
                const int dst = lane + mshift;
                o2f = valid && (dst < 0 || dst > 63);
            }
            if (!(a.dbg & 1u)) {
                if (o1f) add_pos(x + o1s, o1v);
                if (o2f) add_pos(x + o2s, o2v);
            }
            if (wave_done >= wave_quota) break;
            if (!have_n) break;
            cur = nxt; t = t_n; colour = colour_n; seg = seg_n; p = p_n;
        }
    }
}

}
```

gfasort_amd/csrc/sgd_device.h:

```cpp
#pragma once
#include <hip/hip_runtime.h>
#include <stdint.h>
#include "sgd_limits.h"

namespace gfs {

__device__ __forceinline__ int32_t sat_i32(double v) {
    if (v != v) return 0;
    if (v <= -2147483648.0) return INT32_MIN;
    if (v >= 2147483647.0) return INT32_MAX;
    return (int32_t)v;
}

__device__ __forceinline__ double fpp_split(double a, int32_t e, double fb) {
    int32_t high = (int32_t)((uint64_t)__double_as_longlong(a) >> 32);
    int32_t diff = (int32_t)((uint32_t)high - 1072632447u);
    int32_t new_high = sat_i32(fb * (double)diff + 1072632447.0);
    double frac = __longlong_as_double((long long)(((uint64_t)(uint32_t)new_high) << 32));
    double base = a, r = 1.0;
    int32_t ex = e;
    while (ex != 0) {
        if (ex & 1) r *= base;
        base *= base;
        ex >>= 1;
    }
    return r * frac;
}

struct Rng {
    uint64_t s0, s1, s2, s3;
    __device__ __forceinline__ uint64_t next() {
        uint64_t result = s0 + s3;
        uint64_t t = s1 << 17;
        s2 ^= s0; s3 ^= s1; s1 ^= s2; s0 ^= s3;
        s2 ^= t;
        s3 = (s3 << 45) | (s3 >> 19);
        return result;
    }
    __device__ __forceinline__ uint32_t flip() { return (uint32_t)(next() >> 63); }
    __device__ __forceinline__ double f64() {
        return (double)(next() >> 11) * (1.0 / 9007199254740992.0);
    }
    __device__ __forceinline__ uint32_t uniform32(uint32_t n, uint32_t thresh) {
        for (;;) {
            uint64_t m = (uint64_t)(uint32_t)(next() >> 32) * (uint64_t)n;
            if ((uint32_t)m >= thresh) return (uint32_t)(m >> 32);
        }
    }
    __device__ __forceinline__ uint64_t uniform64(uint64_t n, uint64_t thresh) {
        for (;;) {
            const uint64_t r = next();
            if (r * n >= thresh) return __umul64hi(r, n);
        }
    }
};


struct KArgs {
    const uint4    *step_rec;
    const uint4    *path_rec;
    const uint64_t *path_len;
    const double   *zetas;
    double         *x;
    uint64_t       *rng;
    unsigned long long *counters;
    void           *trace;
    uint32_t       *trace_cnt;
    uint32_t       *lead;
    uint64_t n_steps, steps_thresh;
    uint32_t n_paths, zlen_full;
    uint32_t zlen_staged;
    uint32_t n_streams;
    uint32_t quota_base, quota_rem;
    uint32_t attempt_factor, trace_per_stream;
    uint32_t space, space_max, space_q;
    uint32_t dbg;
    uint32_t bundle, n_nodes;
    int32_t  kshift;
    uint32_t chain;
    uint32_t partners;
    uint32_t ref_chunk;
    uint32_t dbg2;
    uint32_t chunk;
    IterConsts it;
};

__device__ __forceinline__ uint64_t sample_step(const KArgs &a, Rng &rng) {
    if (a.n_steps <= 0xFFFFFFFFull && !(a.dbg & 0x40u)) return rng.uniform32((uint32_t)a.n_steps, (uint32_t)a.steps_thresh);
    return rng.uniform64(a.n_steps, a.steps_thresh);
}
__device__ __forceinline__ uint64_t path_first(const uint4 &pr) { return ((uint64_t)pr.w << 32) | pr.x; }
constexpr uint32_t PATH_MASK = 0x7FFFFFFFu;
constexpr uint32_t POS_HI_MASK = 0x7FFFFFu;
__device__ __forceinline__ uint64_t rec_pos_u64(const uint4 &r) { return ((uint64_t)(r.w & POS_HI_MASK) << 32) | (uint64_t)r.z; }
__device__ __forceinline__ uint32_t rec_path(const uint4 &r) { return r.y & PATH_MASK; }

template <bool RUNS>
__device__ __forceinline__ int crowd_shift(const KArgs &a, const uint4 &ra, const uint4 &rb) {
    const int aa = (int)((ra.w >> 23) & 63u) - a.kshift, ab = (int)((rb.w >> 23) & 63u) - a.kshift;
    const int ba = RUNS ? (int)((ra.w >> 29) & 7u) : 0, bb = RUNS ? (int)((rb.w >> 29) & 7u) : 0;
    int k = aa > ab ? aa : ab;
    const int b = ba > bb ? ba : bb;
    k = k > b ? k : b;
    return k > 0 ? k : 0;
}
__device__ __forceinline__ double crowd_scale(double mu, int k) { return k ? ldexp(mu, -k) : mu; }

template <int D>
__device__ __forceinline__ double *coord_ptr(const KArgs &a, uint32_t slot, bool end) {
    return a.x + (end ? (uint64_t)a.n_nodes * D : 0ull) + slot;
}
__device__ __forceinline__ uint64_t coord_step(const KArgs &a) { return (uint64_t)a.n_nodes; }

__device__ __forceinline__ uint32_t space_index(const KArgs &a, uint32_t jump) {
    uint32_t idx = jump > a.space_max ? a.space_max + (jump - a.space_max) / a.space_q + 1 : jump;
    uint32_t last = a.zlen_full - 1;
    return idx < last ? idx : last;
}

__device__ __forceinline__ uint32_t dirty_zipf(const IterConsts &c, uint32_t jump, double zeta, double u) {
    double uz = u * zeta;
    if (uz < 1.0) return 1u;
    if (uz < c.zeta2theta) return 2u;
    double n = (double)jump;
    double eta = (1.0 - fpp_split(2.0 / n, c.omt_e, c.omt_fb)) / (1.0 - c.zeta2theta / zeta);
    double v = eta * u - eta + 1.0;
    double result = 1.0 + n * fpp_split(v, c.alpha_e, c.alpha_fb);
    if (!(result > 0.0)) return 0u;
    if (result >= 4294967296.0) return jump;
    uint32_t r = (uint32_t)result;
    return r < jump ? r : jump;
}

template <bool LDS_TABLES>
__device__ __forceinline__ bool sample_pair_from(const KArgs &a, const uint4 *path_tab, const double *zeta_tab,
                                                 Rng &rng, const uint64_t step_idx, const uint4 &ra, uint4 &rb, uint64_t &sa, uint64_t &sb,
                                                 uint32_t &cnt_out, uint32_t &path_out) {
    uint32_t path = rec_path(ra);
    uint4 pr = path_tab[path];
    const uint64_t first = path_first(pr); const uint32_t cnt = pr.y;
    if (cnt == 1u) return false;
    uint32_t rank_a = (uint32_t)(step_idx - first);
    uint32_t rank_b = rank_a;
    if (a.it.cooling || rng.flip() == 1u) {
        bool back = false, fwd = false;
        if (rank_a > 0u && (rng.flip() == 1u || rank_a == cnt - 1u)) back = true;
        else if (rank_a < cnt - 1u) fwd = true;
        if (back || fwd) {
            uint32_t room = back ? rank_a : (cnt - rank_a - 1u);
// ... 147 lines not shown
```

gfasort_amd/csrc/sgd_host.h:

```cpp
#pragma once
#include <hip/hip_runtime.h>
#include <stdint.h>
#include <type_traits>
#include "capi_error.h"
#include "sgd_limits.h"

namespace gfs {

struct KernelShape { int dims; uint32_t bundle; bool lds_tables, atomic_loads, trace; };

template <typename... A> inline const void *kernel_addr(void (*k)(A...)) { return reinterpret_cast<const void *>(k); }
template <typename F> inline auto with_flag(bool b, F f) { return b ? f(std::true_type{}) : f(std::false_type{}); }

const void *iteration_kernel_1d(const KernelShape &s);
const void *iteration_kernel_nd(const KernelShape &s);
const void *iteration_kernel_nd_team(const KernelShape &s);
const void *iteration_kernel_nd_team_wide(const KernelShape &s);

const void *fused_kernel_1d(const KernelShape &s, bool pooled);
const void *phased_fused_kernel(bool lds_tables);
const void *fused_kernel_nd(const KernelShape &s, bool pooled);
const void *fused_kernel_nd_team(const KernelShape &s, bool pooled);
const void *fused_kernel_nd_team_wide(const KernelShape &s, bool pooled);

const void *batch_fused_kernel(int dims, bool lds_tables);

hipError_t warm_module_1d();
hipError_t warm_module_1d_phased();
hipError_t warm_module_nd();
hipError_t warm_module_nd_team();
hipError_t warm_module_nd_team_wide();
hipError_t warm_module_index();
hipError_t warm_module_quality();

hipError_t init_positions_device(const uint32_t *d_node_len, const uint32_t *d_perm, double *d_x, uint64_t n);
hipError_t reorder_positions_device(const double *d_src, double *d_dst, const uint32_t *d_perm, uint64_t N, uint32_t D,
                                    int to_device, hipStream_t st);
hipError_t sort_order_device(const double *d_x_layout, const uint32_t *d_perm, uint64_t n, uint64_t stride_doubles,
                             void *d_tmp, uint32_t **d_order_out);
inline uint64_t sort_order_scratch_bytes(uint64_t n) { return n * (2 * 8 + 2 * 4); }

struct ReadoutItem {
    double *x;
    const uint32_t *perm, *node_len;
    uint64_t offset;
    uint32_t n, padded;
};
static_assert(sizeof(ReadoutItem) == 40, "a multiple of 8 bytes: the next part of a read-out's region starts where the table ends (readout_region.h)");
hipError_t batch_init_positions_device(const ReadoutItem *d_items, uint32_t count, hipStream_t st);
hipError_t sort_segments_device(const ReadoutItem *d_items, uint32_t count, uint32_t padded, double *d_positions, uint32_t *d_order,
                                hipStream_t st);

struct CoordItem {
    double *x;
    const uint32_t *perm;
    uint64_t offset;
    uint32_t n, first_block, dims, _pad;
};
static_assert(sizeof(CoordItem) == 40, "a multiple of 8 bytes: the next part of a read-out's region starts where the table ends (readout_region.h)");
hipError_t batch_coords_device(const CoordItem *d_items, const uint32_t *d_block_item, uint64_t blocks, double *d_packed, int to_device,
                               hipStream_t st);
struct QualityItem {
    const uint4 *step_rec;
    const double *x;
    uint64_t n_steps, n_nodes;
    uint32_t first_block, blocks;
};
static_assert(sizeof(QualityItem) == 40, "a multiple of 8 bytes: the next part of a read-out's region starts where the table ends (readout_region.h)");
hipError_t batch_pair_errors_device(const QualityItem *d_items, const uint32_t *d_block_item, uint32_t n_items, uint64_t row_blocks,
                                    uint32_t dims, const uint64_t *d_zs, uint32_t n_z, uint64_t *d_partials, uint64_t *d_out, hipStream_t st);

struct DiagItem {
    const uint4 *step_rec, *path_rec;
    const double *x;
    const uint32_t *perm;
    uint64_t n_steps, n_nodes, n_paths;
    uint64_t first_tile, first_path, first_node, first_pair;
    uint32_t first_block, blocks;
};
static_assert(sizeof(DiagItem) == 96, "a multiple of 8 bytes: the next part of a read-out's region starts where the table ends (readout_region.h)");
hipError_t batch_path_errors_device(const DiagItem *d_items, const uint32_t *d_tile_item, uint32_t n_items, uint64_t n_tiles, uint64_t n_paths,
                                    uint32_t dims, uint64_t z, double ratio, uint64_t *d_head, uint64_t *d_tail, uint64_t *d_out,
                                    uint64_t max_blocks, hipStream_t st);
hipError_t batch_stretched_scan_bytes(uint64_t n_tiles, size_t *bytes);
hipError_t batch_stretched_pairs_device(const DiagItem *d_items, const uint32_t *d_tile_item, uint64_t n_tiles, uint32_t dims, uint64_t z,
                                        double ratio, uint64_t *d_counts, uint64_t *d_offsets, void *d_list, uint64_t cap, void *d_tmp,
                                        size_t tmp_bytes, uint64_t max_blocks, hipStream_t st);
hipError_t batch_node_errors_device(const DiagItem *d_items, const uint32_t *d_block_item, uint32_t n_items, uint64_t row_blocks, uint64_t n_nodes,
                                    uint32_t dims, uint64_t z, double ratio, uint64_t *d_slots, uint64_t *d_out, hipStream_t st);

hipError_t batch_sorted_positions_device(const ReadoutItem *d_items, uint32_t count, uint32_t padded, uint64_t *d_spos, uint64_t *d_totals,
                                         hipStream_t st);
// ... 37 lines not shown
```

gfasort_amd/csrc/sgd_kernels_1d.hip:

```cpp
#include "sgd_1d.h"
#include "sgd_host.h"

namespace gfs {

template <bool LDS_TABLES, bool ATOMIC_LOADS, bool TRACE>
__global__ void sgd1d_kernel(const KArgs a) {
    extern __shared__ __align__(16) unsigned char smem[];
    const uint4 *path_tab; const double *zeta_tab;
    stage_tables<LDS_TABLES>(a, smem, path_tab, zeta_tab);

    const uint32_t tid = blockIdx.x * blockDim.x + threadIdx.x;
    const bool live = tid < a.n_streams;
    uint32_t done = 0, att = 0;
    if (live) {
        Rng rng;
        load_rng(a, tid, rng);
        const uint32_t quota = a.quota_base + (tid < a.quota_rem ? 1u : 0u);
        const uint64_t max_att64 = (uint64_t)a.attempt_factor * quota + 1024u;
        const uint64_t max_att = max_att64 > 0xFFFFFFFFull ? 0xFFFFFFFFull : max_att64;
        uint32_t ntr = TRACE ? a.trace_cnt[tid] : 0;
        ref_run_1d<LDS_TABLES, ATOMIC_LOADS, TRACE>(a, path_tab, zeta_tab, rng, quota, max_att, tid, done, att, ntr);
        store_rng(a, tid, rng);
        if (TRACE) a.trace_cnt[tid] = ntr;
    }
    flush_counters(a, done, att);
}

template <bool LDS_TABLES>
__global__ void sgd1d_fused_kernel(const KArgs a0, const IterConsts *its, const uint32_t n_iters, uint32_t *pool) {
    extern __shared__ __align__(16) unsigned char smem[];
    const uint4 *path_tab; const double *zeta_tab;
    stage_tables<LDS_TABLES>(a0, smem, path_tab, zeta_tab);
    const uint32_t tid = blockIdx.x * blockDim.x + threadIdx.x;
    if ((tid & ~63u) >= a0.n_streams) return;
    const bool live = tid < a0.n_streams;
    KArgs a = a0;
    Rng rng = {0, 0, 0, 0};
    if (live) load_rng(a, tid, rng);
    uint32_t done = 0, att = 0, ntr = 0;
    ref_pooled_walk(a, its, n_iters, pool, tid, [&](const uint32_t share, const uint64_t max_att) {
        ref_run_1d<LDS_TABLES, true, false>(a, path_tab, zeta_tab, rng, share, max_att, tid, done, att, ntr);
    });
    if (live) store_rng(a, tid, rng);
    flush_counters(a, done, att);
}


template <int B, bool LDS_TABLES, bool ATOMIC_LOADS, bool TRACE>
__global__ void __attribute__((amdgpu_waves_per_eu(4, 4))) sgd1d_team_kernel(const KArgs a) {
    extern __shared__ __align__(16) unsigned char smem[];
    const uint4 *path_tab; const double *zeta_tab;
    stage_tables<LDS_TABLES>(a, smem, path_tab, zeta_tab);
    const uint32_t tid = blockIdx.x * blockDim.x + threadIdx.x;
    if (tid >= a.n_streams) return;
    TeamState ts;
    uint32_t no_flips = 0;
    load_rng(a, tid, ts.rng);
    ts.ntr = TRACE ? a.trace_cnt[tid] : 0;
    load_pass(a, tid, ts, no_flips);
    const uint64_t wq = wave_quota_of(a, tid & ~63u);
    for (uint64_t done = 0; done < wq; done += a.chunk)
        team_iteration<B, LDS_TABLES, ATOMIC_LOADS, TRACE>(a, path_tab, zeta_tab, ts, tid, wq - done < a.chunk ? wq - done : a.chunk);
    store_rng(a, tid, ts.rng);
    if (TRACE) a.trace_cnt[tid] = ts.ntr;
    store_pass(a, tid, ts, 0u);
    flush_counters(a, ts.done, ts.att);
}

template <int B, bool LDS_TABLES, bool POOL>
__global__ void __attribute__((amdgpu_waves_per_eu(4, 4))) sgd1d_team_fused_kernel(const KArgs a0, const IterConsts *its, const uint32_t n_iters,
                                                                                   uint32_t *pool) {
    constexpr bool ATOMIC_LOADS = true;
    extern __shared__ __align__(16) unsigned char smem[];
    const uint4 *path_tab; const double *zeta_tab;
    stage_tables<LDS_TABLES>(a0, smem, path_tab, zeta_tab);
    const uint32_t tid = blockIdx.x * blockDim.x + threadIdx.x;
    if (tid >= a0.n_streams) return;
    KArgs a = a0;
    TeamState ts;
    uint32_t no_flips = 0;
    load_rng(a, tid, ts.rng);
    load_pass(a, tid, ts, no_flips);
    if (POOL) {
        const uint32_t wave = (uint32_t)__builtin_amdgcn_readfirstlane((int)(tid >> 6));
        pool_walk(a, its, n_iters, pool, pool_share(a0, wave, a0.n_streams >> 6), [&]() __attribute__((always_inline)) { return a0.chunk; },
                  [&](const uint32_t k, const uint32_t m) __attribute__((always_inline)) {
            team_iteration<B, LDS_TABLES, ATOMIC_LOADS, false>(a, path_tab, zeta_tab, ts, tid, m, its + k);
        });
    } else {
        const uint64_t wq = wave_quota_of(a, tid & ~63u);
        for (uint32_t k = 0; k < n_iters; ++k) {
            a.it = its[k];
            for (uint64_t done = 0; done < wq; done += a.chunk)
                team_iteration<B, LDS_TABLES, ATOMIC_LOADS, false>(a, path_tab, zeta_tab, ts, tid, wq - done < a.chunk ? wq - done : a.chunk, its + k);
        }
    }
    store_rng(a, tid, ts.rng);
    store_pass(a, tid, ts, 0u);
    flush_counters(a, ts.done, ts.att);
}

__global__ void merge_prepare_kernel(const double *x, const double *x_prev, float *buf, uint64_t n) {
    const uint64_t stride = (uint64_t)gridDim.x * blockDim.x * 2;
    for (uint64_t k = ((uint64_t)blockIdx.x * blockDim.x + threadIdx.x) * 2; k < n; k += stride) {
        if (k + 1 < n) {
            const double2 a = *reinterpret_cast<const double2 *>(x + k), b = *reinterpret_cast<const double2 *>(x_prev + k);
            const float d0 = (float)(a.x - b.x), d1 = (float)(a.y - b.y);
            *reinterpret_cast<float2 *>(buf + k) = make_float2(d0, d1);
            if (n & 1) { buf[n + k] = d0 != 0.f ? 1.f : 0.f; buf[n + k + 1] = d1 != 0.f ? 1.f : 0.f; }
            else *reinterpret_cast<float2 *>(buf + n + k) = make_float2(d0 != 0.f ? 1.f : 0.f, d1 != 0.f ? 1.f : 0.f);
        } else {
            const float d = (float)(x[k] - x_prev[k]);
            buf[k] = d; buf[n + k] = d != 0.f ? 1.f : 0.f;
        }
    }
}
__global__ void merge_apply_kernel(double *x, double *x_prev, const float *buf, uint64_t n, double scale_all) {
    const uint64_t stride = (uint64_t)gridDim.x * blockDim.x;
    for (uint64_t k = (uint64_t)blockIdx.x * blockDim.x + threadIdx.x; k < n; k += stride) {
        const double c = (double)buf[n + k];
        const double div = scale_all > 0.0 ? scale_all : (c > 1.0 ? c : 1.0);
        const double v = x_prev[k] + (double)buf[k] / div;
        x_prev[k] = v; x[k] = v;
    }
}
hipError_t launch_merge_prepare(const double *x, const double *x_prev, float *buf, uint64_t n, hipStream_t st) {
    hipLaunchKernelGGL(merge_prepare_kernel, dim3(2048), dim3(256), 0, st, x, x_prev, buf, n);
    return hipGetLastError();
}
hipError_t launch_merge_apply(double *x, double *x_prev, const float *buf, uint64_t n, double scale_all, hipStream_t st) {
    hipLaunchKernelGGL(merge_apply_kernel, dim3(2048), dim3(256), 0, st, x, x_prev, buf, n, scale_all);
    return hipGetLastError();
}

template <int B>
static const void *team_fused_kernel_1d(const KernelShape &s, bool pooled) {
    return with_flag(pooled, [&](auto P) { return with_flag(s.lds_tables, [&](auto L) { return kernel_addr(sgd1d_team_fused_kernel<B, L(), P()>); }); });
}
const void *fused_kernel_1d(const KernelShape &s, bool pooled) {
    switch (s.bundle) {
        case 16: return team_fused_kernel_1d<16>(s, pooled);
        case 32: return team_fused_kernel_1d<32>(s, pooled);
        case 64: return team_fused_kernel_1d<64>(s, pooled);
        case 0: case 1: return pooled ? with_flag(s.lds_tables, [](auto L) { return kernel_addr(sgd1d_fused_kernel<L()>); }) : nullptr;
        default: return nullptr;
    }
}

template <int B>
static const void *team_kernel_1d(const KernelShape &s) {
    return with_flag(s.lds_tables, [&](auto L) { return with_flag(s.atomic_loads, [&](auto A) { return with_flag(s.trace, [&](auto T) {
        return kernel_addr(sgd1d_team_kernel<B, L(), A() || T(), T()>);
    }); }); });
}
const void *iteration_kernel_1d(const KernelShape &s) {
    switch (s.bundle) {
        case 0: case 1:
            return with_flag(s.lds_tables, [&](auto L) { return with_flag(s.atomic_loads, [&](auto A) { return with_flag(s.trace, [&](auto T) {
                return kernel_addr(sgd1d_kernel<L(), A(), T()>);
            }); }); });
        case 4:  return team_kernel_1d<4>(s);
        case 8:  return team_kernel_1d<8>(s);
        case 16: return team_kernel_1d<16>(s);
        case 32: return team_kernel_1d<32>(s);
        case 64: return team_kernel_1d<64>(s);
        default: return nullptr;
    }
}

hipError_t warm_module_1d() {
    hipFuncAttributes attr;
    return hipFuncGetAttributes(&attr, reinterpret_cast<const void *>(&merge_prepare_kernel));
}

}
```

gfasort_amd/hip.py:

```python
import ctypes as C
import os

import numpy as np

from . import build as _build
from .quality import sort_quality_figures

NO_NODE = 0xFFFFFFFF
MAX_DIMS = 8
OK, NOTHING_TO_DO = 0, 1
F_PLAIN_LOADS, F_NO_LDS_TABLES, F_NO_FUSE = 1, 2, 4


F_DBG_NO_ATOMICS, F_DBG_NO_XLOADS, F_DBG_ONE_COLOUR = 0x100, 0x200, 0x800
F_DBG_NO_ALIGN, F_DBG_ALIGN_FIRST, F_DBG_WIDE_INDEX, F_DBG_NO_FUSED_TRIP = 0x1000, 0x2000, 0x4000, 0x8000
F_ONE_PARTNER, F_DBG_NO_TWIN_TRIP, F_DBG_FREE_RUNNING = 0x10, 0x400, 0x20
F_PHASED = 0x40


def F_CHAIN(k):
    return (int(k) & 0xFF) << 24


def F_BUNDLE(n):
    return (int(n) & 0xFF) << 16


class GfsError(RuntimeError):
    def __init__(self, code, msg):
        super().__init__(f"gfasort_hip error {code}: {msg}")
        self.code = code


class GraphView(C.Structure):
    _fields_ = [("n_nodes", C.c_uint64), ("n_steps", C.c_uint64), ("n_paths", C.c_uint64),
                ("node_len", C.c_void_p), ("step_node", C.c_void_p),
                ("step_is_rev", C.c_void_p), ("path_first_step", C.c_void_p)]


class SgdParams(C.Structure):
    _fields_ = [("iter_max", C.c_uint64), ("iter_with_max_learning_rate", C.c_uint64),
                ("min_term_updates", C.c_uint64), ("delta", C.c_double), ("eps", C.c_double),
                ("eta_max", C.c_double), ("theta", C.c_double), ("space", C.c_uint64),
                ("space_max", C.c_uint64), ("space_quantization_step", C.c_uint64),
                ("cooling_start", C.c_double), ("nthreads", C.c_uint64),
                ("progress", C.c_uint8), ("_pad", C.c_uint8 * 7), ("seed", C.c_uint64)]


class LayoutParams(C.Structure):
    _fields_ = [("dimensions", C.c_uint64), ("sgd", SgdParams)]


class LaunchConfig(C.Structure):
    _fields_ = [("n_streams", C.c_uint64), ("stream_base", C.c_uint64),
                ("term_updates_per_iteration", C.c_uint64), ("attempt_factor", C.c_uint64),
                ("block_size", C.c_uint32), ("flags", C.c_uint32), ("trace_per_stream", C.c_uint64)]


class Stats(C.Structure):
    _fields_ = [("term_updates", C.c_uint64), ("attempts", C.c_uint64), ("iterations", C.c_uint64),
                ("n_streams", C.c_uint64), ("bundle", C.c_uint64), ("kernel_ms", C.c_double),
                ("total_ms", C.c_double), ("launches", C.c_uint64), ("run_trips", C.c_uint64)]


class RankConfig(C.Structure):
    _fields_ = [("rank", C.c_uint32), ("world", C.c_uint32), ("device", C.c_int32), ("sharding", C.c_uint32),
                ("merge_every", C.c_uint32), ("merge_rule", C.c_uint32), ("payload", C.c_uint32), ("exchange", C.c_uint32),
                ("launch", LaunchConfig)]


class RankInfo(C.Structure):
    _fields_ = [("quota", C.c_uint64), ("shard_steps", C.c_uint64), ("span_lo", C.c_uint64), ("span_hi", C.c_uint64),
                ("shared_slots", C.c_uint64), ("exchange_count", C.c_uint64), ("positions_len", C.c_uint64),
                ("windows", C.c_uint64), ("last_merge_kernels_ms", C.c_double), ("idle", C.c_uint32), ("_pad", C.c_uint32)]


class PairError(C.Structure):
    _fields_ = [("step_distance", C.c_uint64), ("pairs", C.c_uint64), ("sum_rel_sq", C.c_double), ("max_rel_sq", C.c_double),
                ("sum_abs", C.c_double), ("sum_sq", C.c_double)]


class SortQuality(C.Structure):
    _fields_ = [("steps", C.c_uint64), ("abs_err_sum", C.c_uint64), ("genomic_sum", C.c_uint64), ("sq_err_sum", C.c_double)]


class BatchConfig(C.Structure):
    _fields_ = [("max_blocks_per_launch", C.c_uint64), ("reserved", C.c_uint64 * 3)]


class BatchStats(C.Structure):
    _fields_ = [("items", C.c_uint64), ("items_run", C.c_uint64), ("launches", C.c_uint64), ("blocks", C.c_uint64),
                ("term_updates", C.c_uint64), ("attempts", C.c_uint64), ("kernel_ms", C.c_double), ("total_ms", C.c_double)]


class ContextSetInfo(C.Structure):
    _fields_ = [("items", C.c_uint64), ("total_nodes", C.c_uint64), ("total_steps", C.c_uint64), ("total_paths", C.c_uint64),
                ("launches", C.c_uint64), ("device_allocations", C.c_uint64), ("arena_bytes", C.c_uint64), ("build_ms", C.c_double)]


class ContextSetSetupInfo(C.Structure):
    _fields_ = [("items", C.c_uint64), ("configured", C.c_uint64), ("nothing_to_do", C.c_uint64), ("total_streams", C.c_uint64),
                ("state_bytes", C.c_uint64), ("device_allocations", C.c_uint64), ("copies", C.c_uint64), ("launches", C.c_uint64),
                ("setup_ms", C.c_double)]


STATE_POSITIONS, STATE_COUNTERS, STATE_LEAD, STATE_TRACE, STATE_TRACE_COUNTS, STATE_RNG, STATE_ZETAS, STATE_SCHEDULE = range(8)
STATE_KINDS, STATE_SIZE_OF = 8, 0x100
ITER_CONSTS_DTYPE = np.dtype([("eta", "<f8"), ("zeta2theta", "<f8"), ("omt_fb", "<f8"), ("alpha_fb", "<f8"), ("omt_e", "<i4"),
                              ("alpha_e", "<i4"), ("cooling", "<i4"), ("_pad", "<i4")])

PAIR_ERROR_DTYPE = np.dtype([("step_distance", "<u8"), ("pairs", "<u8"), ("sum_rel_sq", "<f8"), ("max_rel_sq", "<f8"),
                             ("sum_abs", "<f8"), ("sum_sq", "<f8")])

SORT_QUALITY_DTYPE = np.dtype([("steps", "<u8"), ("abs_err_sum", "<u8"), ("genomic_sum", "<u8"), ("sq_err_sum", "<f8")])

PATH_ERROR_DTYPE = np.dtype([("steps", "<u8"), ("reverse_steps", "<u8"), ("pairs", "<u8"), ("sum_rel_sq", "<f8"), ("max_rel_sq", "<f8"),
                             ("sum_abs", "<f8"), ("sum_sq", "<f8"), ("stretched", "<u8")])
STRETCHED_PAIR_DTYPE = np.dtype([("step_a", "<u8"), ("step_b", "<u8"), ("path", "<u8"), ("d_path", "<f8"), ("d_layout", "<f8")])
NODE_ERROR_DTYPE = np.dtype([("pairs", "<u8"), ("stretched", "<u8"), ("max_rel_sq", "<f8")])

ALLREDUCE_FN = C.CFUNCTYPE(C.c_int, C.c_void_p, C.c_void_p, C.c_uint64, C.c_int, C.c_void_p)
MERGE_RULES = {"anneal": 0, "sum": 1, "mean": 2, "touch": 3}

TERM_DTYPE = np.dtype([("i", "<u4"), ("j", "<u4"), ("d_ij", "<f8")], align=True)

EXPORTS = [
    "gfs_version", "gfs_last_error", "gfs_device_count", "gfs_warmup", "gfs_fast_precise_pow", "gfs_sgd_schedule",
    "gfs_zeta_table_len", "gfs_zeta_table", "gfs_init_positions", "gfs_init_layout_dim0", "gfs_init_layout",
    "gfs_sort_order", "gfs_path_linear_sgd", "gfs_path_sgd_sort", "gfs_path_linear_sgd_layout", "gfs_ctx_create",
    "gfs_ctx_create_with_layout", "gfs_ctx_node_layout",
    "gfs_ctx_destroy", "gfs_ctx_setup_1d", "gfs_ctx_setup_nd", "gfs_ctx_positions_len", "gfs_ctx_init_positions",
    "gfs_ctx_upload_positions", "gfs_ctx_download_positions", "gfs_ctx_positions_device",
    "gfs_ctx_bind_positions", "gfs_ctx_reset_streams", "gfs_ctx_run_iteration", "gfs_ctx_run_range", "gfs_ctx_run",
    "gfs_ctx_synchronize", "gfs_ctx_stats", "gfs_ctx_sort_order", "gfs_ctx_trace", "gfs_merge_prepare", "gfs_merge_apply",
    "gfs_shard_paths", "gfs_shard_quotas", "gfs_shared_node_layout", "gfs_exchange_plan",
    "gfs_rank_create", "gfs_rank_destroy", "gfs_rank_ctx", "gfs_rank_get_info", "gfs_rank_set_positions",
    "gfs_rank_positions_changed", "gfs_rank_get_positions", "gfs_rank_exchange_count", "gfs_rank_exchange_buffer",
    "gfs_rank_bind_exchange_buffer", "gfs_rank_window_begin", "gfs_rank_window_end", "gfs_rank_finish_begin",
    "gfs_rank_finish_buffer", "gfs_rank_finish_end", "gfs_rank_run",
    "gfs_ctx_debug_step_records", "gfs_ctx_debug_kshift", "gfs_phase_window", "gfs_ctx_phase_window",
    "gfs_ctx_pair_errors", "gfs_stress_sample_pairs", "gfs_ctx_stress_of_pairs", "gfs_ctx_sort_quality", "gfs_pair_errors",
    "gfs_sort_quality_of", "gfs_batch_sort_quality",
    "gfs_ctx_path_errors", "gfs_ctx_stretched_pairs", "gfs_ctx_node_errors", "gfs_diagnose",
    "gfs_batch_plan", "gfs_batch_create", "gfs_batch_run", "gfs_batch_get_stats", "gfs_batch_destroy",
    "gfs_batch_result_offsets", "gfs_batch_init_positions", "gfs_batch_results", "gfs_batch_debug_sort_cap",
    "gfs_batch_upload_coords", "gfs_batch_coords", "gfs_batch_pair_errors",
    "gfs_batch_path_offsets", "gfs_batch_path_errors", "gfs_batch_stretched_pairs", "gfs_batch_node_errors", "gfs_batch_debug_tile_blocks",
    "gfs_ctx_set_plan", "gfs_ctx_set_create", "gfs_ctx_set_size", "gfs_ctx_set_item", "gfs_ctx_set_get_info", "gfs_ctx_set_destroy",
    "gfs_ctx_set_state_plan", "gfs_ctx_set_setup_1d", "gfs_ctx_set_setup_nd", "gfs_ctx_set_get_setup_info", "gfs_ctx_debug_sgd_state",
]
SEGMENT_SORT_CAP = 8192

_lib = None


def lib_path():
    return _build.LIB


def lib():
    global _lib
    if _lib is None:
        path = os.environ.get("GFS_LIB_PATH") or _build.LIB
        if not os.path.exists(path):
            raise ImportError(f"{path} is not built: run `python -m gfasort_amd.build` "
                              "(hipcc, gfx950). There is no CPU fallback.")
        L = C.CDLL(path)
        L.gfs_version.restype = C.c_char_p
        L.gfs_last_error.restype = C.c_char_p
        L.gfs_fast_precise_pow.restype = C.c_double
        L.gfs_fast_precise_pow.argtypes = [C.c_double, C.c_double]
        L.gfs_zeta_table_len.restype = C.c_uint64
        L.gfs_ctx_positions_len.restype = C.c_uint64
        L.gfs_ctx_positions_len.argtypes = [C.c_void_p]
        L.gfs_ctx_init_positions.argtypes = [C.c_void_p]
        L.gfs_ctx_positions_device.restype = C.c_void_p
        L.gfs_ctx_positions_device.argtypes = [C.c_void_p]
        L.gfs_ctx_destroy.argtypes = [C.c_void_p]
        L.gfs_ctx_destroy.restype = None
        L.gfs_ctx_run_iteration.argtypes = [C.c_void_p, C.c_uint64, C.c_void_p]
        L.gfs_ctx_run.argtypes = [C.c_void_p, C.c_void_p]
        L.gfs_ctx_run_range.argtypes = [C.c_void_p, C.c_void_p, C.c_uint64, C.c_void_p]
        L.gfs_ctx_synchronize.argtypes = [C.c_void_p, C.c_void_p]
        L.gfs_ctx_bind_positions.argtypes = [C.c_void_p, C.c_void_p]
        L.gfs_ctx_reset_streams.argtypes = [C.c_void_p]
        L.gfs_ctx_upload_positions.argtypes = [C.c_void_p, C.c_void_p, C.c_uint64]
        L.gfs_ctx_download_positions.argtypes = [C.c_void_p, C.c_void_p, C.c_uint64]
        L.gfs_ctx_stats.argtypes = [C.c_void_p, C.c_void_p]
        L.gfs_ctx_sort_order.argtypes = [C.c_void_p, C.c_void_p, C.c_uint64]
        L.gfs_ctx_trace.argtypes = [C.c_void_p, C.c_void_p, C.c_uint64, C.c_void_p, C.c_uint64]
        L.gfs_ctx_node_layout.argtypes = [C.c_void_p, C.c_void_p, C.c_uint64]
        L.gfs_ctx_debug_step_records.argtypes = [C.c_void_p, C.c_void_p, C.c_uint64]
        L.gfs_ctx_debug_kshift.argtypes = [C.c_void_p, C.c_int32, C.c_void_p]
        L.gfs_phase_window.argtypes = [C.c_void_p, C.c_void_p, C.c_void_p]
        L.gfs_ctx_phase_window.argtypes = [C.c_void_p, C.c_int64, C.c_int64, C.c_void_p, C.c_void_p]
        L.gfs_ctx_setup_1d.argtypes = [C.c_void_p] + [C.c_void_p] * 4
        L.gfs_ctx_setup_nd.argtypes = [C.c_void_p] + [C.c_void_p] * 4
        L.gfs_sort_order.argtypes = [C.c_void_p, C.c_uint64, C.c_void_p]
        L.gfs_merge_prepare.argtypes = [C.c_void_p, C.c_void_p, C.c_void_p, C.c_uint64, C.c_void_p]
        L.gfs_merge_apply.argtypes = [C.c_void_p, C.c_void_p, C.c_void_p, C.c_uint64, C.c_double, C.c_void_p]
        L.gfs_shard_paths.argtypes = [C.c_void_p, C.c_uint32, C.c_uint32, C.c_void_p, C.c_void_p]
        L.gfs_shard_quotas.argtypes = [C.c_uint64, C.c_void_p, C.c_uint32, C.c_void_p]
        L.gfs_shared_node_layout.argtypes = [C.c_void_p, C.c_void_p]
        L.gfs_exchange_plan.argtypes = [C.c_void_p, C.c_void_p, C.c_void_p, C.c_uint32] + [C.c_void_p] * 9
        L.gfs_rank_create.argtypes = [C.c_void_p, C.c_void_p, C.c_uint64, C.c_void_p, C.c_void_p]
        L.gfs_rank_destroy.argtypes = [C.c_void_p]
        L.gfs_rank_destroy.restype = None
        L.gfs_rank_ctx.argtypes = [C.c_void_p]
        L.gfs_rank_ctx.restype = C.c_void_p
        L.gfs_rank_get_info.argtypes = [C.c_void_p, C.c_void_p]
        L.gfs_rank_set_positions.argtypes = [C.c_void_p, C.c_void_p, C.c_uint64]
        L.gfs_rank_positions_changed.argtypes = [C.c_void_p, C.c_void_p]
        L.gfs_rank_get_positions.argtypes = [C.c_void_p, C.c_void_p, C.c_uint64]
        L.gfs_rank_exchange_count.argtypes = [C.c_void_p]
        L.gfs_rank_exchange_count.restype = C.c_uint64
        L.gfs_rank_exchange_buffer.argtypes = [C.c_void_p]
        L.gfs_rank_exchange_buffer.restype = C.c_void_p
        L.gfs_rank_bind_exchange_buffer.argtypes = [C.c_void_p, C.c_void_p]
        L.gfs_rank_window_begin.argtypes = [C.c_void_p, C.c_void_p, C.c_uint64, C.c_void_p]
        L.gfs_rank_window_end.argtypes = [C.c_void_p, C.c_void_p]
        L.gfs_rank_finish_begin.argtypes = [C.c_void_p, C.c_void_p, C.c_void_p]
        L.gfs_rank_finish_buffer.argtypes = [C.c_void_p]
        L.gfs_rank_finish_buffer.restype = C.c_void_p
        L.gfs_rank_finish_end.argtypes = [C.c_void_p, C.c_void_p, C.c_void_p]
        L.gfs_rank_run.argtypes = [C.c_void_p, ALLREDUCE_FN, C.c_void_p, C.c_void_p]
        L.gfs_ctx_pair_errors.argtypes = [C.c_void_p, C.c_void_p, C.c_uint64, C.c_void_p, C.c_void_p]
        L.gfs_stress_sample_pairs.argtypes = [C.c_void_p, C.c_uint64, C.c_uint64, C.c_void_p, C.c_void_p, C.c_void_p]
        L.gfs_ctx_stress_of_pairs.argtypes = [C.c_void_p, C.c_void_p, C.c_void_p, C.c_uint64, C.c_void_p, C.c_void_p, C.c_void_p]
        L.gfs_ctx_sort_quality.argtypes = [C.c_void_p, C.c_void_p]
        L.gfs_pair_errors.argtypes = [C.c_void_p, C.c_uint64, C.c_void_p, C.c_void_p, C.c_uint64, C.c_void_p]
        L.gfs_ctx_path_errors.argtypes = [C.c_void_p, C.c_uint64, C.c_double, C.c_void_p, C.c_uint64, C.c_void_p]
        L.gfs_ctx_stretched_pairs.argtypes = [C.c_void_p, C.c_uint64, C.c_double, C.c_void_p, C.c_uint64, C.c_void_p, C.c_void_p]
        L.gfs_ctx_node_errors.argtypes = [C.c_void_p, C.c_uint64, C.c_double, C.c_void_p, C.c_uint64, C.c_void_p]
        L.gfs_diagnose.argtypes = [C.c_void_p, C.c_uint64, C.c_void_p, C.c_uint64, C.c_double, C.c_void_p, C.c_void_p, C.c_uint64, C.c_void_p]
        L.gfs_batch_plan.argtypes = [C.c_void_p, C.c_uint64, C.c_uint64, C.c_void_p, C.c_void_p]
        L.gfs_batch_create.argtypes = [C.c_void_p, C.c_uint64, C.c_void_p, C.c_void_p]
        L.gfs_batch_run.argtypes = [C.c_void_p, C.c_void_p]
        L.gfs_batch_get_stats.argtypes = [C.c_void_p, C.c_void_p]
        L.gfs_batch_destroy.argtypes = [C.c_void_p]
        L.gfs_batch_destroy.restype = None
        L.gfs_batch_result_offsets.argtypes = [C.c_void_p, C.c_void_p, C.c_uint64]
        L.gfs_batch_init_positions.argtypes = [C.c_void_p, C.c_void_p]
        L.gfs_batch_results.argtypes = [C.c_void_p, C.c_void_p, C.c_void_p, C.c_uint64, C.c_void_p, C.c_void_p]
        L.gfs_batch_debug_sort_cap.argtypes = [C.c_void_p, C.c_uint64]
        L.gfs_batch_upload_coords.argtypes = [C.c_void_p, C.c_void_p, C.c_uint64, C.c_void_p]
        L.gfs_batch_coords.argtypes = [C.c_void_p, C.c_void_p, C.c_uint64, C.c_void_p, C.c_void_p]
        L.gfs_batch_pair_errors.argtypes = [C.c_void_p, C.c_void_p, C.c_uint64, C.c_void_p, C.c_void_p, C.c_void_p]
        L.gfs_batch_path_offsets.argtypes = [C.c_void_p, C.c_void_p, C.c_uint64]
        L.gfs_batch_path_errors.argtypes = [C.c_void_p, C.c_uint64, C.c_double, C.c_void_p, C.c_uint64, C.c_void_p, C.c_void_p]
        L.gfs_batch_stretched_pairs.argtypes = [C.c_void_p, C.c_uint64, C.c_double, C.c_void_p, C.c_uint64, C.c_void_p, C.c_void_p, C.c_void_p]
        L.gfs_batch_node_errors.argtypes = [C.c_void_p, C.c_uint64, C.c_double, C.c_void_p, C.c_uint64, C.c_void_p, C.c_void_p]
        L.gfs_batch_debug_tile_blocks.argtypes = [C.c_void_p, C.c_uint64]
        L.gfs_sort_quality_of.argtypes = [C.c_void_p, C.c_void_p, C.c_void_p]
        L.gfs_batch_sort_quality.argtypes = [C.c_void_p, C.c_void_p, C.c_uint64, C.c_void_p, C.c_void_p]
        L.gfs_ctx_set_plan.argtypes = [C.c_void_p, C.c_void_p, C.c_void_p, C.c_uint64, C.c_void_p, C.c_void_p]
        L.gfs_ctx_set_create.argtypes = [C.c_void_p, C.c_uint64, C.c_int, C.c_void_p]
        L.gfs_ctx_set_size.argtypes = [C.c_void_p]
        L.gfs_ctx_set_size.restype = C.c_uint64
        L.gfs_ctx_set_item.argtypes = [C.c_void_p, C.c_uint64]
        L.gfs_ctx_set_item.restype = C.c_void_p
        L.gfs_ctx_set_get_info.argtypes = [C.c_void_p, C.c_void_p]
        L.gfs_ctx_set_destroy.argtypes = [C.c_void_p]
        L.gfs_ctx_set_destroy.restype = None
        L.gfs_ctx_set_state_plan.argtypes = [C.c_void_p, C.c_uint64, C.c_void_p, C.c_void_p]
        L.gfs_ctx_set_setup_1d.argtypes = [C.c_void_p] * 4
        L.gfs_ctx_set_setup_nd.argtypes = [C.c_void_p] * 4
        L.gfs_ctx_set_get_setup_info.argtypes = [C.c_void_p, C.c_void_p]
        L.gfs_ctx_debug_sgd_state.argtypes = [C.c_void_p, C.c_uint32, C.c_void_p, C.c_uint64]
        _lib = L
    return _lib


def check(rc):
    if rc < 0:
        raise GfsError(rc, lib().gfs_last_error().decode())
    return rc
# ... 346 lines not shown
    def sort_order(self):
        order = np.zeros(self.graph.n_nodes, dtype=np.uint64)
        check(lib().gfs_ctx_sort_order(self._h, _ptr(order), C.c_uint64(order.shape[0])))
        return order

    def trace(self):
        st = self.stats()
        k = int(self.cfg.trace_per_stream)
        T = int(st.n_streams)
        out = np.zeros(T * k, dtype=TERM_DTYPE)
        counts = np.zeros(T, dtype=np.uint64)
        check(lib().gfs_ctx_trace(self._h, _ptr(out), T * k, _ptr(counts), T))
        return out.reshape(T, k), counts

    def pair_errors(self, zs, stream=None):
        zs = np.ascontiguousarray(zs, dtype=np.uint64)
        out = np.zeros(zs.shape[0], dtype=PAIR_ERROR_DTYPE)
        check(lib().gfs_ctx_pair_errors(self._h, _ptr(zs), C.c_uint64(zs.shape[0]), _ptr(out), C.c_void_p(stream or 0)))
        return out

    def stress_of_pairs(self, step_a, step_b):
        sa = np.ascontiguousarray(step_a, dtype=np.uint64)
        sb = np.ascontiguousarray(step_b, dtype=np.uint64)
        if sa.shape != sb.shape:
            raise ValueError("step_a and step_b differ in length")
        rel = np.zeros(sa.shape[0], dtype=np.float64)
        counted, stress = C.c_uint64(0), C.c_double(0.0)
        check(lib().gfs_ctx_stress_of_pairs(self._h, _ptr(sa), _ptr(sb), C.c_uint64(sa.shape[0]), _ptr(rel), C.byref(counted),
                                            C.byref(stress)))
        return float(stress.value), int(counted.value), rel

    def sampled_stress(self, samples=10000, seed=12345):
        sa, sb = stress_sample_pairs(self.graph, samples, seed)
        return self.stress_of_pairs(sa, sb)[0]

    def sort_quality(self):
        q = SortQuality()
        check(lib().gfs_ctx_sort_quality(self._h, C.byref(q)))
        return sort_quality_figures(q.steps, q.abs_err_sum, q.genomic_sum, q.sq_err_sum)

    def path_errors(self, z=1, ratio=10.0, stream=None):
        out = np.zeros(self.graph.n_paths, dtype=PATH_ERROR_DTYPE)
        check(lib().gfs_ctx_path_errors(self._h, C.c_uint64(z), C.c_double(ratio), _ptr(out), C.c_uint64(out.shape[0]),
                                        C.c_void_p(stream or 0)))
        return out

    def stretched_pairs(self, z=1, ratio=10.0, cap=1024, out=None, stream=None):
        cap = int(cap)
        if out is None and cap:
            out = np.zeros(cap, dtype=STRETCHED_PAIR_DTYPE)
        if cap and (out.dtype != STRETCHED_PAIR_DTYPE or out.shape[0] < cap or not out.flags.c_contiguous):
            raise ValueError("out must be a contiguous STRETCHED_PAIR_DTYPE array of at least cap entries")
        total = C.c_uint64(0)
        check(lib().gfs_ctx_stretched_pairs(self._h, C.c_uint64(z), C.c_double(ratio), _ptr(out) if cap else None, C.c_uint64(cap),
                                            C.byref(total), C.c_void_p(stream or 0)))
        n = min(cap, int(total.value))
        return (out[:n] if cap else np.zeros(0, dtype=STRETCHED_PAIR_DTYPE)), int(total.value)

    def node_errors(self, z=1, ratio=10.0, stream=None):
        out = np.zeros(self.graph.n_nodes, dtype=NODE_ERROR_DTYPE)
        check(lib().gfs_ctx_node_errors(self._h, C.c_uint64(z), C.c_double(ratio), _ptr(out), C.c_uint64(out.shape[0]),
                                        C.c_void_p(stream or 0)))
        return out

    def step_records(self):
        out = np.zeros((self.graph.n_steps + 1, 4), dtype=np.uint32)
        check(lib().gfs_ctx_debug_step_records(self._h, _ptr(out), C.c_uint64(out.size)))
        return out

    def debug_sgd_state(self, which):
        dtype = {STATE_POSITIONS: np.float64, STATE_ZETAS: np.float64, STATE_SCHEDULE: ITER_CONSTS_DTYPE, STATE_TRACE: TERM_DTYPE,
                 STATE_RNG: np.uint64, STATE_COUNTERS: np.uint64, STATE_LEAD: np.uint32, STATE_TRACE_COUNTS: np.uint32}[int(which)]
        size = C.c_uint64(0)
        check(lib().gfs_ctx_debug_sgd_state(self._h, C.c_uint32(int(which) | STATE_SIZE_OF), C.byref(size), C.c_uint64(8)))
        out = np.zeros(int(size.value) // np.dtype(dtype).itemsize, dtype=dtype)
        check(lib().gfs_ctx_debug_sgd_state(self._h, C.c_uint32(int(which)), _ptr(out), C.c_uint64(out.nbytes)))
        return out

    def kshift(self, set=None):
        v = C.c_int32(0)
        check(lib().gfs_ctx_debug_kshift(self._h, C.c_int32(-2 if set is None else int(set)), C.byref(v)))
        return int(v.value)

    def phase_window(self, set_begin=-1, set_end=-1):
        b, e = C.c_uint64(0), C.c_uint64(0)
        check(lib().gfs_ctx_phase_window(self._h, C.c_int64(int(set_begin)), C.c_int64(int(set_end)), C.byref(b), C.byref(e)))
        return int(b.value), int(e.value)


def ctx_set_plan(n_nodes, n_steps, n_paths):
    nn, ns, npth = (np.ascontiguousarray(a, dtype=np.uint64) for a in (n_nodes, n_steps, n_paths))
    n = nn.shape[0]
    if ns.shape[0] != n or npth.shape[0] != n:
        raise ValueError("one count of each kind per item")
    off = np.zeros((max(n, 1), 5), dtype=np.uint64)
    total = C.c_uint64(0)
    check(lib().gfs_ctx_set_plan(_ptr(nn), _ptr(ns), _ptr(npth), C.c_uint64(n), _ptr(off), C.byref(total)))
    return off[:n], int(total.value)


def ctx_set_state_plan(nbytes):
    nb = np.ascontiguousarray(nbytes, dtype=np.uint64).reshape(-1, STATE_KINDS)
    off = np.zeros((max(nb.shape[0], 1), STATE_KINDS), dtype=np.uint64)
    total = C.c_uint64(0)
    check(lib().gfs_ctx_set_state_plan(_ptr(nb), C.c_uint64(nb.shape[0]), _ptr(off), C.byref(total)))
    return off[:nb.shape[0]], int(total.value)


class ContextSet:

    def __init__(self, graphs, device=0):
        self._h = C.c_void_p()
        self.contexts = []
        graphs = list(graphs)
        n = len(graphs)
        views, self._keep = [], []
        for g in graphs:
            v, keep = make_view(g)
            views.append(v)
            self._keep.append(keep)
        arr = (C.c_void_p * max(n, 1))(*[C.addressof(v) for v in views])
        check(lib().gfs_ctx_set_create(arr if n else None, C.c_uint64(n), C.c_int(device), C.byref(self._h)))
        self.contexts = [Context(g, _borrowed=lib().gfs_ctx_set_item(self._h, i)) for i, g in enumerate(graphs)]

    def close(self):
        if self._h:
            for c in self.contexts:
                c.close()
            lib().gfs_ctx_set_destroy(self._h)
            self._h = C.c_void_p()

    def __del__(self):
        try:
            self.close()
        except Exception:
            pass

    def info(self):
        out = ContextSetInfo()
        check(lib().gfs_ctx_set_get_info(self._h, C.byref(out)))
        return out

    def _setup(self, entry, make, params, cfgs, dims_of):
        n = len(self.contexts)
        params = list(params) if isinstance(params, (list, tuple)) else [params] * n
        cfgs = list(cfgs) if isinstance(cfgs, (list, tuple)) else [cfgs] * n
        if len(params) != n or len(cfgs) != n:
            raise ValueError("params / cfgs: one for all items or one per item")
        made = [make(p) for p in params]
        c_params = (type(made[0]) * n)(*made)
        c_cfgs = None if all(c is None for c in cfgs) else (LaunchConfig * n)(*[c if c is not None else LaunchConfig() for c in cfgs])
        rcs = np.zeros(n, dtype=np.int32)
        check(entry(self._h, c_params, c_cfgs, _ptr(rcs)))
        for ctx, p, c in zip(self.contexts, params, cfgs):
            ctx.params, ctx.cfg, ctx.dims = p, c, dims_of(p)
        return rcs.tolist()

    def setup_1d(self, params, cfgs=None):
        return self._setup(lib().gfs_ctx_set_setup_1d, make_sgd_params, params, cfgs, lambda p: 0)

    def setup_nd(self, params, cfgs=None):
        return self._setup(lib().gfs_ctx_set_setup_nd, make_layout_params, params, cfgs, lambda p: p.dimensions)

    @property
    def setup_info(self):
        out = ContextSetSetupInfo()
# ... 174 lines not shown
```

include/gfasort_hip.h:

```cpp
#ifndef GFASORT_HIP_H
#define GFASORT_HIP_H
#include <stdint.h>
#include <stddef.h>

#ifdef __cplusplus
extern "C" {
#endif

#define GFS_OK            0
#define GFS_NOTHING_TO_DO 1
#define GFS_E_ARG        (-1)
#define GFS_E_HIP        (-2)
#define GFS_E_NOMEM      (-3)
#define GFS_E_STATE      (-4)
#define GFS_E_UNSUPPORTED (-5)

#define GFS_NO_NODE 0xFFFFFFFFu
#define GFS_MAX_DIMS 8

typedef struct gfs_graph_view {
    uint64_t        n_nodes;
    uint64_t        n_steps;
    uint64_t        n_paths;
    const uint32_t *node_len;
    const uint32_t *step_node;
    const uint8_t  *step_is_rev;
    const uint64_t *path_first_step;
} gfs_graph_view;

typedef struct gfs_sgd_params {
    uint64_t iter_max;
    uint64_t iter_with_max_learning_rate;
    uint64_t min_term_updates;
    double   delta;
    double   eps;
    double   eta_max;
    double   theta;
    uint64_t space;
    uint64_t space_max;
    uint64_t space_quantization_step;
    double   cooling_start;
    uint64_t nthreads;
    uint8_t  progress;
    uint8_t  _pad[7];
    uint64_t seed;
} gfs_sgd_params;

typedef struct gfs_layout_params {
    uint64_t dimensions;
    gfs_sgd_params sgd;
} gfs_layout_params;

typedef struct gfs_launch_config {
    uint64_t n_streams;
    uint64_t stream_base;
    uint64_t term_updates_per_iteration;
    uint64_t attempt_factor;
    uint32_t block_size;
    uint32_t flags;
    uint64_t trace_per_stream;
} gfs_launch_config;

#define GFS_F_PLAIN_LOADS   1u
#define GFS_F_NO_LDS_TABLES 2u
#define GFS_F_BUNDLE(n) (((uint32_t)(n) & 0xFFu) << 16)
#define GFS_F_CHAIN(k) (((uint32_t)(k) & 0xFFu) << 24)
#define GFS_F_NO_FUSE       4u
#define GFS_F_ONE_PARTNER   0x10u
#define GFS_F_PHASED        0x40u
#define GFS_F_DBG_NO_TWIN_TRIP 0x400u
#define GFS_F_DBG_FREE_RUNNING 0x20u
#define GFS_F_DBG_NO_ATOMICS 0x100u
#define GFS_F_DBG_NO_XLOADS  0x200u
#define GFS_F_DBG_ONE_COLOUR   0x800u
#define GFS_F_DBG_NO_ALIGN      0x1000u
#define GFS_F_DBG_ALIGN_FIRST   0x2000u
#define GFS_F_DBG_NO_FUSED_TRIP 0x8000u
#define GFS_F_DBG_WIDE_INDEX 0x4000u

typedef struct gfs_stats {
    uint64_t term_updates;
    uint64_t attempts;
    uint64_t iterations;
    uint64_t n_streams;
    uint64_t bundle;
    double   kernel_ms;
    double   total_ms;
    uint64_t launches;
    uint64_t run_trips;
} gfs_stats;

typedef struct gfs_term {
    uint32_t i, j;
    double   d_ij;
} gfs_term;

typedef struct gfs_ctx gfs_ctx;

const char *gfs_version(void);
const char *gfs_last_error(void);
int         gfs_device_count(void);
int         gfs_warmup(int device);

double   gfs_fast_precise_pow(double a, double b);
int      gfs_sgd_schedule(const gfs_sgd_params *p, double *etas);
uint64_t gfs_zeta_table_len(const gfs_sgd_params *p);
int      gfs_zeta_table(const gfs_sgd_params *p, double *zetas);
int      gfs_init_positions(const gfs_graph_view *g, double *x);
int      gfs_init_layout_dim0(const gfs_graph_view *g, uint64_t dims, double *coords);
int      gfs_init_layout(const gfs_graph_view *g, uint64_t dims, uint64_t seed, double *coords);
int      gfs_sort_order(const double *x, uint64_t n, uint64_t *order);

int gfs_path_linear_sgd(const gfs_graph_view *g, const gfs_sgd_params *p,
                        const gfs_launch_config *cfg, const double *etas, const double *zetas,
                        int init_x, double *x_inout, gfs_stats *stats);
int gfs_path_sgd_sort(const gfs_graph_view *g, const gfs_sgd_params *p,
                      const gfs_launch_config *cfg, const double *etas, const double *zetas,
                      int init_x, double *x_inout, uint64_t *order_out, gfs_stats *stats);
int gfs_path_linear_sgd_layout(const gfs_graph_view *g, const gfs_layout_params *p,
                               const gfs_launch_config *cfg, const double *etas, const double *zetas,
                               double *coords_inout, gfs_stats *stats);

int   gfs_ctx_create(const gfs_graph_view *g, int device, gfs_ctx **out);
int   gfs_ctx_create_with_layout(const gfs_graph_view *g, int device, const uint32_t *node_perm, gfs_ctx **out);
int   gfs_ctx_node_layout(const gfs_ctx *ctx, uint32_t *perm_out, uint64_t n_nodes);
void  gfs_ctx_destroy(gfs_ctx *ctx);
int   gfs_ctx_setup_1d(gfs_ctx *ctx, const gfs_sgd_params *p, const gfs_launch_config *cfg,
                       const double *etas, const double *zetas);
int   gfs_ctx_setup_nd(gfs_ctx *ctx, const gfs_layout_params *p, const gfs_launch_config *cfg,
                       const double *etas, const double *zetas);
uint64_t gfs_ctx_positions_len(const gfs_ctx *ctx);
int   gfs_ctx_upload_positions(gfs_ctx *ctx, const double *host, uint64_t n);
int   gfs_ctx_init_positions(gfs_ctx *ctx);
int   gfs_ctx_download_positions(gfs_ctx *ctx, double *host, uint64_t n);
void *gfs_ctx_positions_device(gfs_ctx *ctx);
int   gfs_ctx_bind_positions(gfs_ctx *ctx, void *device_ptr);
int   gfs_ctx_reset_streams(gfs_ctx *ctx);
int   gfs_ctx_run_iteration(gfs_ctx *ctx, uint64_t k, void *hip_stream);
int   gfs_phase_window(const gfs_sgd_params *p, uint64_t *k_begin, uint64_t *k_end);
int   gfs_ctx_run_range(gfs_ctx *ctx, const uint64_t *ks, uint64_t n, void *hip_stream);
int   gfs_ctx_run(gfs_ctx *ctx, void *hip_stream);
int   gfs_ctx_synchronize(gfs_ctx *ctx, void *hip_stream);
int   gfs_ctx_stats(gfs_ctx *ctx, gfs_stats *out);
int   gfs_ctx_sort_order(gfs_ctx *ctx, uint64_t *order, uint64_t n_nodes);
int   gfs_ctx_trace(gfs_ctx *ctx, gfs_term *out, uint64_t n_terms, uint64_t *counts, uint64_t n_streams);
int   gfs_ctx_debug_step_records(const gfs_ctx *ctx, uint32_t *out, uint64_t n_words);
int   gfs_ctx_debug_kshift(gfs_ctx *ctx, int32_t set, int32_t *kshift_out);
int   gfs_ctx_phase_window(gfs_ctx *ctx, int64_t set_begin, int64_t set_end, uint64_t *begin_out, uint64_t *end_out);

typedef struct gfs_pair_error {
    uint64_t step_distance;
    uint64_t pairs;
    double   sum_rel_sq;
    double   max_rel_sq;
    double   sum_abs;
    double   sum_sq;
} gfs_pair_error;

typedef struct gfs_sort_quality {
    uint64_t steps;
    uint64_t abs_err_sum;
    uint64_t genomic_sum;
    double   sq_err_sum;
} gfs_sort_quality;

int gfs_ctx_pair_errors(gfs_ctx *ctx, const uint64_t *zs, uint64_t n_z, gfs_pair_error *out, void *hip_stream);
int gfs_stress_sample_pairs(const gfs_graph_view *g, uint64_t sample_count, uint64_t seed, uint64_t *step_a, uint64_t *step_b,
                            uint64_t *n_out);
int gfs_ctx_stress_of_pairs(gfs_ctx *ctx, const uint64_t *step_a, const uint64_t *step_b, uint64_t n, double *rel_sq_out ,
                            uint64_t *counted, double *stress);
int gfs_ctx_sort_quality(gfs_ctx *ctx, gfs_sort_quality *out);
int gfs_pair_errors(const gfs_graph_view *g, uint64_t dims, const double *positions, const uint64_t *zs, uint64_t n_z,
                    gfs_pair_error *out);
int gfs_sort_quality_of(const gfs_graph_view *g, const double *positions, gfs_sort_quality *out);

typedef struct gfs_path_error {
    uint64_t steps;
    uint64_t reverse_steps;
    uint64_t pairs;
    double   sum_rel_sq;
    double   max_rel_sq;
    double   sum_abs;
    double   sum_sq;
    uint64_t stretched;
} gfs_path_error;

typedef struct gfs_stretched_pair {
    uint64_t step_a, step_b;
    uint64_t path;
    double   d_path, d_layout;
} gfs_stretched_pair;

typedef struct gfs_node_error {
    uint64_t pairs;
    uint64_t stretched;
    double   max_rel_sq;
} gfs_node_error;

int gfs_ctx_path_errors(gfs_ctx *ctx, uint64_t z, double ratio, gfs_path_error *out, uint64_t n_paths, void *hip_stream);
int gfs_ctx_stretched_pairs(gfs_ctx *ctx, uint64_t z, double ratio, gfs_stretched_pair *out, uint64_t cap, uint64_t *total,
                            void *hip_stream);
int gfs_ctx_node_errors(gfs_ctx *ctx, uint64_t z, double ratio, gfs_node_error *out, uint64_t n_nodes, void *hip_stream);
int gfs_diagnose(const gfs_graph_view *g, uint64_t dims, const double *positions, uint64_t z, double ratio,
                 gfs_path_error *paths_out, gfs_stretched_pair *pairs_out, uint64_t cap, uint64_t *total);

#define GFS_SEGMENT_SORT_CAP 8192
typedef struct gfs_batch gfs_batch;
typedef struct gfs_batch_config {
    uint64_t max_blocks_per_launch;
    uint64_t reserved[3];
} gfs_batch_config;
typedef struct gfs_batch_stats {
    uint64_t items, items_run;
    uint64_t launches;
    uint64_t blocks;
    uint64_t term_updates, attempts;
    double   kernel_ms, total_ms;
} gfs_batch_stats;

int  gfs_batch_plan(const uint64_t *blocks_of_item, uint64_t n, uint64_t max_blocks, uint32_t *launch_of_item, uint32_t *n_launches);
int  gfs_batch_create(gfs_ctx *const *ctxs, uint64_t n, const gfs_batch_config *cfg , gfs_batch **out);
int  gfs_batch_run(gfs_batch *b, void *hip_stream);
int  gfs_batch_get_stats(gfs_batch *b, gfs_batch_stats *out);
void gfs_batch_destroy(gfs_batch *b);
int  gfs_batch_result_offsets(const gfs_batch *b, uint64_t *offsets, uint64_t n);
int  gfs_batch_init_positions(gfs_batch *b, void *hip_stream);
int  gfs_batch_results(gfs_batch *b, double *positions, uint32_t *order, uint64_t total, double *kernel_ms, void *hip_stream);
int  gfs_batch_debug_sort_cap(gfs_batch *b, uint64_t cap);
int  gfs_batch_upload_coords(gfs_batch *b, const double *coords, uint64_t total, void *hip_stream);
int  gfs_batch_coords(gfs_batch *b, double *coords, uint64_t total, double *kernel_ms , void *hip_stream);
// ... 120 lines not shown
```

Baseline: 104.5 billion.

## Add compact 8-byte trip records for 1D team SGD kernels

Builds a second, compact per-step record array (slot plus 32-bit position) during index construction and records graph facts such as max position and crowd exponents. When those facts show that the crowd shift is always zero and positions fit in 32 bits, the 1D bundle-64 team kernels are instantiated with COMPACT=true and read 8-byte records instead of 16-byte ones. The goal is to halve gather traffic for the random step-record loads in the SGD inner loop. The cost is extra memory, a host readback of the facts, and new kernel variants whose occupancy is capped at the minimum of both.

```diff
diff --git a/gfasort_amd/csrc/capi.hip b/gfasort_amd/csrc/capi.hip
--- a/gfasort_amd/csrc/capi.hip
+++ b/gfasort_amd/csrc/capi.hip
@@ -145,7 +145,8 @@
     return hipLaunchKernel(fn, grid, block, args, s.lds_bytes, st);
 }
 
-static int plan_launches(int cu_count, gfs::LaunchShape &s, LaunchPlan &pl, std::string *err) {
+static int plan_launches(int cu_count, const gfs::RecordFacts &rec, int32_t kshift_override, uint64_t n_steps, gfs::LaunchShape &s, LaunchPlan &pl,
+                         std::string *err) {
     pl = LaunchPlan{};
     const gfs::KernelShape shape{s.dims, s.bundle, s.lds_tables, s.atomic_loads, s.trace};
     const bool team = s.team, ref = s.bundle == 1;
@@ -161,13 +162,30 @@
                " trace=" + std::to_string(s.trace) + " phased=" + std::to_string(s.phased);
         return GFS_E_UNSUPPORTED;
     }
+    gfs::LaunchShape probe = s;
+    probe.flags &= ~GFS_F_FULL_RECORDS;
+    const bool has_compact = rec.have_trip_rec && gfs::compact_records(probe, gfs::RecordFacts{0, 0, 0, true}, 0);
+    const gfs::KernelShape compact{s.dims, s.bundle, s.lds_tables, s.atomic_loads, s.trace, true};
+    const void *pooled_compact = has_compact ? fused_kernel(compact, true) : nullptr;
+    const void *free_compact = has_compact && free_running ? fused_kernel(compact, false) : nullptr;
+    if (has_compact) pl.iteration_compact = iteration_kernel(compact);
+    if (has_compact && (!pl.iteration_compact || !pooled_compact || (free_running && !free_compact))) {
+        *err = "no kernel is built for 8-byte trip records in this shape"; return GFS_E_UNSUPPORTED;
+    }
     int per_cu = 0;
     if (team) {
         int rc = resident_blocks_per_cu(s, pooled_kernel, &per_cu, err);
         if (rc) return rc;
+        if (has_compact) {
+            int per_cu_compact = 0;
+            if ((rc = resident_blocks_per_cu(s, pooled_compact, &per_cu_compact, err))) return rc;
+            per_cu = std::min(per_cu, per_cu_compact);
+        }
     }
     gfs::shape_after_residency(per_cu, gfs::DeviceFacts{cu_count}, &s);
     if (s.fused) pl.fused = s.pooled ? pooled_kernel : free_kernel;
+    if (s.fused && has_compact) pl.fused_compact = s.pooled ? pooled_compact : free_compact;
+    gfs::shape_records(rec, kshift_override >= 0 ? kshift_override : gfs::crowd_kshift(n_steps, s.n_streams), &s);
     return GFS_OK;
 }
 
@@ -186,7 +204,7 @@
     const gfs::GraphFacts graph{c->n_nodes, c->n_steps, c->n_paths, c->max_path_steps, c->valid_paths, c->path_counts.data()};
     int rc = gfs::shape_before_residency(graph, gfs::DeviceFacts{c->cu_count}, p, dims, cfg, &sp.shape, err);
     if (rc) return rc;
-    rc = plan_launches(c->cu_count, sp.shape, sp.plan, err);
+    rc = plan_launches(c->cu_count, c->record_facts, c->kshift_override, c->n_steps, sp.shape, sp.plan, err);
     if (rc) return rc;
     sp.etas.resize(p->iter_max + 1);
     if (etas) std::copy(etas, etas + p->iter_max + 1, sp.etas.begin());
@@ -212,6 +230,11 @@
     if (rc) return fail(rc, err);
     HIPCHK(hipSetDevice(c->device));
     gfs::free_sgd_state(c);
+    if (dims != 0 && c->d_trip_rec) {
+        HIPCHK(hipDeviceSynchronize());
+        c->d_trip_rec.reset();
+        c->record_facts.have_trip_rec = false;
+    }
     gfs::SetupPlan sp;
     const int planned = gfs::plan_setup(c, p, dims, cfg, etas, &sp, &err);
     uint64_t bytes[GFS_STATE_KINDS];
@@ -400,6 +423,7 @@
     if (const char *e = std::getenv("GFS_DBG_REF_CHUNK")) { const long v = std::atol(e); if (v >= 1 && v <= 4096) a.ref_chunk = (uint32_t)v; }
     a.n_nodes = (uint32_t)c->n_nodes;
     a.kshift = c->kshift_override >= 0 ? c->kshift_override : gfs::crowd_kshift(c->n_steps, c->shape.n_streams);
+    if (c->shape.compact) a.trip_rec = c->d_trip_rec;
 }
 
 extern "C" {
@@ -438,7 +462,7 @@
     int rc = next_event_pair(c, ev);
     if (rc) return rc;
     HIPCHK(ev->start(st));
-    hipError_t e = launch(c, window ? c->plan.window_iteration : c->plan.iteration, a, nullptr, 0, nullptr, st);
+    hipError_t e = launch(c, window ? c->plan.window_iteration : c->shape.compact ? c->plan.iteration_compact : c->plan.iteration, a, nullptr, 0, nullptr, st);
     if (e != hipSuccess) return fail(GFS_E_HIP, std::string("kernel launch: ") + hipGetErrorString(e));
     HIPCHK(ev->stop(st));
     c->iterations++;
@@ -504,7 +528,7 @@
     int rc = next_event_pair(c, ev);
     if (rc) return rc;
     HIPCHK(ev->start(st));
-    hipError_t e = launch(c, pl.fused, a, d_slice, (uint32_t)n, pool, st);
+    hipError_t e = launch(c, c->shape.compact ? pl.fused_compact : pl.fused, a, d_slice, (uint32_t)n, pool, st);
     if (e != hipSuccess) return fail(GFS_E_HIP, std::string("fused kernel launch: ") + hipGetErrorString(e));
     HIPCHK(ev->stop(st));
     c->iterations += n;
@@ -610,7 +634,11 @@
 }
 int gfs_ctx_debug_kshift(gfs_ctx *c, int32_t set, int32_t *kshift_out) {
     if (!c) return fail(GFS_E_ARG, "ctx is null");
-    if (set >= -1) c->kshift_override = set;
+    if (set >= -1) {
+        c->kshift_override = set;
+        if (c->configured && c->shape.n_streams)
+            gfs::shape_records(c->record_facts, set >= 0 ? set : gfs::crowd_kshift(c->n_steps, c->shape.n_streams), &c->shape);
+    }
     if (kshift_out) {
         if (!c->configured || !c->shape.n_streams) return fail(GFS_E_STATE, "context not set up");
         gfs::KArgs a{};
@@ -618,6 +646,11 @@
         *kshift_out = a.kshift;
     }
     return GFS_OK;
+}
+
+uint32_t gfs_ctx_record_bytes(const gfs_ctx *c) {
+    if (!c || !c->configured || !c->shape.n_streams) return 0;
+    return c->shape.compact ? (uint32_t)sizeof(uint2) : (uint32_t)sizeof(uint4);
 }
 
 int gfs_ctx_phase_window(gfs_ctx *c, int64_t set_begin, int64_t set_end, uint64_t *begin_out, uint64_t *end_out) {
diff --git a/gfasort_amd/csrc/capi_ctx.h b/gfasort_amd/csrc/capi_ctx.h
--- a/gfasort_amd/csrc/capi_ctx.h
+++ b/gfasort_amd/csrc/capi_ctx.h
@@ -24,6 +24,7 @@
     const void *iteration = nullptr;
     const void *window_iteration = nullptr;
     const void *fused = nullptr;
+    const void *iteration_compact = nullptr, *fused_compact = nullptr;
 };
 
 struct gfs_ctx {
@@ -37,6 +38,8 @@
     std::vector<uint32_t> perm;
     gfs::Buffer arena;
     gfs::Array<uint4> d_step_rec;
+    gfs::Array<uint2> d_trip_rec;
+    gfs::RecordFacts record_facts;
     gfs::Array<uint4> d_path_rec;
     gfs::Array<uint64_t> d_path_len;
     gfs::Array<uint32_t> d_perm;
diff --git a/gfasort_amd/csrc/capi_set.hip b/gfasort_amd/csrc/capi_set.hip
--- a/gfasort_amd/csrc/capi_set.hip
+++ b/gfasort_amd/csrc/capi_set.hip
@@ -103,10 +103,14 @@
     u.items = reinterpret_cast<const gfs::SetItem *>(d_in + in.at_items);
     u.step_is_rev = d_in + in.at_rev;
     u.arena = d_arena;
+    gfs_ctx *single = staged || n != 1 ? nullptr : ctxs[0];
+    if (single && S && single->d_trip_rec.grow((S + 1) * sizeof(uint2)) != hipSuccess) (void)hipGetLastError();
+    u.trip = single ? (uint2 *)single->d_trip_rec : nullptr;
     uint32_t bad_item = gfs::SET_NO_BAD_ITEM;
     e = gfs::index_set_layout_device(u, d_in + in.bytes, node_perm != nullptr, &bad_item, &info->launches);
     lap("node layout");
-    if (e == hipSuccess && bad_item == gfs::SET_NO_BAD_ITEM) e = gfs::index_set_records_device(u, d_in + in.bytes, &info->launches);
+    if (e == hipSuccess && bad_item == gfs::SET_NO_BAD_ITEM)
+        e = gfs::index_set_records_device(u, d_in + in.bytes, &info->launches, single ? &single->record_facts : nullptr);
     if (e != hipSuccess || bad_item != gfs::SET_NO_BAD_ITEM) (void)hipDeviceSynchronize();
     if (e != hipSuccess) return fail(GFS_E_HIP, std::string("build_index_set: ") + hipGetErrorString(e));
     if (bad_item != gfs::SET_NO_BAD_ITEM) return fail(GFS_E_ARG, (staged ? item_prefix(bad_item) : "") + "step_node out of range");
@@ -117,6 +121,10 @@
     }
     if ((e = hipDeviceSynchronize()) != hipSuccess) return fail(GFS_E_HIP, std::string("hipDeviceSynchronize: ") + hipGetErrorString(e));
     lap("K3");
+    if (single) {
+        if (single->record_facts.max_pos >= (1ull << 32) || single->record_facts.max_b > 0) single->d_trip_rec.reset();
+        single->record_facts.have_trip_rec = single->d_trip_rec != nullptr;
+    }
     for (uint64_t i = 0; i < n; ++i) {
         gfs_ctx *c = ctxs[i];
         const uint64_t *at = &offsets[KINDS * i];
diff --git a/gfasort_amd/csrc/index_set.h b/gfasort_amd/csrc/index_set.h
--- a/gfasort_amd/csrc/index_set.h
+++ b/gfasort_amd/csrc/index_set.h
@@ -1,5 +1,6 @@
 #pragma once
 #include "index_set_plan.h"
+#include "launch_policy.h"
 #include <hip/hip_runtime.h>
 #include <stdint.h>
 
@@ -19,6 +20,7 @@
     const uint8_t *step_is_rev;
     const uint64_t *path_first;
     unsigned char *arena;
+    uint2 *trip;
 };
 
 constexpr uint32_t SET_NO_BAD_ITEM = 0xFFFFFFFFu;
@@ -26,7 +28,7 @@
 
 hipError_t index_set_work_bytes(uint64_t n_nodes, uint64_t n_steps, uint64_t *bytes);
 hipError_t index_set_layout_device(const SetUnion &u, void *d_work, bool layout_given, uint32_t *bad_item, uint64_t *launches);
-hipError_t index_set_records_device(const SetUnion &u, void *d_work, uint64_t *launches);
+hipError_t index_set_records_device(const SetUnion &u, void *d_work, uint64_t *launches, RecordFacts *facts = nullptr);
 hipError_t warm_module_index_set();
 
 }
diff --git a/gfasort_amd/csrc/index_set_kernels.hip b/gfasort_amd/csrc/index_set_kernels.hip
--- a/gfasort_amd/csrc/index_set_kernels.hip
+++ b/gfasort_amd/csrc/index_set_kernels.hip
@@ -132,8 +132,9 @@
         if (c > 1 && rep[v] < c) atomicMax(&rep[v], c);
     }
 }
-__global__ void set_fill_records_kernel(SetUnion u, const uint64_t *scan, const uint32_t *cnt, const uint32_t *rep) {
-    const uint64_t stride = (uint64_t)gridDim.x * blockDim.x;
+__global__ void set_fill_records_kernel(SetUnion u, const uint64_t *scan, const uint32_t *cnt, const uint32_t *rep, unsigned long long *facts) {
+    const uint64_t stride = (uint64_t)gridDim.x * blockDim.x;
+    unsigned long long max_pos = 0, max_a = 0, max_b = 0;
     for (uint64_t s = (uint64_t)blockIdx.x * blockDim.x + threadIdx.x; s < u.n_steps; s += stride) {
         const uint32_t p = path_of(u.path_first, (uint32_t)u.n_paths, s);
         const SetItem it = u.items[item_of(u.items, u.n_items, s, &SetItem::step_off)];
@@ -145,10 +146,24 @@
         if (n != NO_NODE_U32) {
             const uint32_t a = set_ceil_log2(cnt[it.node_off + n]), b = set_ceil_log2(rep[it.node_off + n]);
             crowd = ((a > 63u ? 63u : a) << 23) | ((b > 7u ? 7u : b) << 29);
-        }
+            if (a > max_a) max_a = a;
+            if (b > max_b) max_b = b;
+        }
+        if (pos > max_pos) max_pos = pos;
         r.y = (uint32_t)(p - it.path_off) | ((uint32_t)(u.step_is_rev[s] & 1) << 31);
         r.z = (uint32_t)pos; r.w = ((uint32_t)(pos >> 32) & 0x7FFFFFu) | crowd;
         reinterpret_cast<uint4 *>(u.arena + it.rec)[s - it.step_off] = r;
+        if (u.trip) u.trip[s] = make_uint2(r.x, r.z);
+    }
+    if (!facts) return;
+    for (int off = 32; off > 0; off >>= 1) {
+        const unsigned long long p = __shfl_xor(max_pos, off, 64), a = __shfl_xor(max_a, off, 64), b = __shfl_xor(max_b, off, 64);
+        max_pos = p > max_pos ? p : max_pos; max_a = a > max_a ? a : max_a; max_b = b > max_b ? b : max_b;
+    }
+    if ((threadIdx.x & 63) == 0) {
+        if (max_pos) atomicMax(&facts[0], max_pos);
+        if (max_a) atomicMax(&facts[1], max_a);
+        if (max_b) atomicMax(&facts[2], max_b);
     }
 }
 __global__ void set_paths_kernel(SetUnion u, const uint64_t *scan) {
@@ -157,6 +172,7 @@
         if (t >= u.n_paths) {
             const uint32_t i = (uint32_t)(t - u.n_paths);
             reinterpret_cast<uint4 *>(u.arena + u.items[i].rec)[u.items[i + 1].step_off - u.items[i].step_off] = make_uint4(0, 0, 0, 0);
+            if (u.trip) u.trip[u.n_steps] = make_uint2(0, 0);
             continue;
         }
         const SetItem it = u.items[item_of(u.items, u.n_items, t, &SetItem::path_off)];
@@ -173,6 +189,7 @@
     uint32_t *ids_a, *ids_b, *a, *b, *cnt, *rep;
     uint64_t *scan;
     uint32_t *flags;
+    unsigned long long *facts;
     void *tmp;
     size_t tmp_bytes;
     uint64_t cnt_rep_bytes, bytes;
@@ -200,6 +217,7 @@
     w.cnt_rep_bytes = round256(N ? N * 4 : 1) + N * 4;
     take(w.scan, S ? (S + 1) * 8 : 0);
     take(w.flags, (1 + 2 * JUMP_ROUNDS) * sizeof(uint32_t));
+    take(w.facts, 3 * sizeof(unsigned long long));
     w.tmp_bytes = std::max(sort_tmp, scan_tmp);
     take(w.tmp, w.tmp_bytes);
     w.bytes = at;
@@ -274,7 +292,7 @@
     return hipGetLastError();
 }
 
-hipError_t index_set_records_device(const SetUnion &u, void *d_work, uint64_t *launches) {
+hipError_t index_set_records_device(const SetUnion &u, void *d_work, uint64_t *launches, RecordFacts *facts) {
     const uint64_t N = u.n_nodes, S = u.n_steps;
     Work w{};
     hipError_t e = plan_work(N, S, d_work, w);
@@ -285,11 +303,20 @@
         if (e != hipSuccess) return e;
         if ((e = hipMemsetAsync(w.cnt, 0, w.cnt_rep_bytes, 0)) != hipSuccess) return e;
         hipLaunchKernelGGL(set_node_stats_kernel, over_steps, block, 0, 0, u, w.cnt, w.rep);
-        hipLaunchKernelGGL(set_fill_records_kernel, over_steps, block, 0, 0, u, w.scan, w.cnt, w.rep);
+        if (facts) {
+            if ((e = hipMemsetAsync(w.facts, 0, 3 * sizeof(unsigned long long), 0)) != hipSuccess) return e;
+            ++*launches;
+        }
+        hipLaunchKernelGGL(set_fill_records_kernel, over_steps, block, 0, 0, u, w.scan, w.cnt, w.rep, facts ? w.facts : (unsigned long long *)nullptr);
         *launches += 4;
     }
     hipLaunchKernelGGL(set_paths_kernel, dim3(SET_PATH_BLOCKS), block, 0, 0, u, S ? w.scan : (const uint64_t *)nullptr);
     ++*launches;
+    if (facts) {
+        unsigned long long h[3] = {0, 0, 0};
+        if (S && (e = hipMemcpy(h, w.facts, sizeof h, hipMemcpyDeviceToHost)) != hipSuccess) return e;
+        facts->max_pos = h[0]; facts->max_a = (uint32_t)h[1]; facts->max_b = (uint32_t)h[2];
+    }
     return hipGetLastError();
 }
 
diff --git a/gfasort_amd/csrc/launch_policy.h b/gfasort_amd/csrc/launch_policy.h
--- a/gfasort_amd/csrc/launch_policy.h
+++ b/gfasort_amd/csrc/launch_policy.h
@@ -39,6 +39,13 @@
     bool fuse_one = false;
     bool fuse_one_probe = false;
     uint32_t one_chunk = 0;
+    bool compact = false;
+};
+
+struct RecordFacts {
+    uint64_t max_pos = 0;
+    uint32_t max_a = 0, max_b = 0;
+    bool have_trip_rec = false;
 };
 
 inline bool has_fused_team_kernel(int dims, uint32_t bundle) { return (dims == 0 && bundle >= 16) || (dims >= 2 && bundle == 64); }
@@ -183,6 +190,13 @@
     return lg + 2;
 }
 
+inline bool compact_records(const LaunchShape &s, const RecordFacts &r, int32_t kshift) {
+    const bool kernel = s.dims == 0 && s.bundle == 64 && !s.trace && !s.phased;
+    const bool graph = r.have_trip_rec && r.max_pos < (1ull << 32) && (int64_t)r.max_a <= (int64_t)kshift && r.max_b == 0;
+    return kernel && graph && !(s.flags & GFS_F_FULL_RECORDS);
+}
+inline void shape_records(const RecordFacts &r, int32_t kshift, LaunchShape *shape) { shape->compact = compact_records(*shape, r, kshift); }
+
 inline bool wide_index(uint64_t n_steps, uint32_t flags) { return n_steps > 0xFFFFFFFFull || (flags & GFS_F_DBG_WIDE_INDEX); }
 
 inline bool batch_eligible(const LaunchShape &s, bool trace, bool has_resident_schedule, bool idle) {
diff --git a/gfasort_amd/csrc/sgd_1d.h b/gfasort_amd/csrc/sgd_1d.h
--- a/gfasort_amd/csrc/sgd_1d.h
+++ b/gfasort_amd/csrc/sgd_1d.h
@@ -60,10 +60,27 @@
     uint32_t done = 0, att = 0, ntr = 0;
 };
 
+template <bool COMPACT> struct TripRec;
+template <> struct TripRec<false> {
+    uint4 r = make_uint4(0, 0, 0, 0);
+    static __device__ __forceinline__ TripRec load(const KArgs &a, uint64_t s) { TripRec t; t.r = a.step_rec[s]; return t; }
+    __device__ __forceinline__ uint32_t slot() const { return r.x; }
+    __device__ __forceinline__ double pos() const { return rec_pos(r); }
+    static __device__ __forceinline__ int crowd(const KArgs &a, const TripRec &ra, const TripRec &rb) { return crowd_shift<true>(a, ra.r, rb.r); }
+};
+template <> struct TripRec<true> {
+    uint2 r = make_uint2(0, 0);
+    static __device__ __forceinline__ TripRec load(const KArgs &a, uint64_t s) { TripRec t; t.r = a.trip_rec[s]; return t; }
+    __device__ __forceinline__ uint32_t slot() const { return r.x; }
+    __device__ __forceinline__ double pos() const { return (double)r.y; }
+    static __device__ __forceinline__ int crowd(const KArgs &, const TripRec &, const TripRec &) { return 0; }
+};
+
+template <bool COMPACT>
 struct Trip {
     uint64_t sa = 0, sb = 0;
-    uint4 ra = make_uint4(0, 0, 0, 0), rb = make_uint4(0, 0, 0, 0);
-    uint4 rc = make_uint4(0, 0, 0, 0);
+    TripRec<COMPACT> ra, rb;
+    TripRec<COMPACT> rc;
     bool twin = false;
     bool valid = false;
     int mshift = 0;
@@ -73,8 +90,9 @@
     uint32_t off = 0;
 };
 
-template <int B>
-__device__ __forceinline__ void expand_trip(const KArgs &a, const Leader &L, int t, uint32_t seg, uint32_t p, uint32_t colour, int sub, int q, Trip &tr) {
+template <int B, bool COMPACT>
+__device__ __forceinline__ void expand_trip(const KArgs &a, const Leader &L, int t, uint32_t seg, uint32_t p, uint32_t colour, int sub, int q, Trip<COMPACT> &tr) {
+    using Rec = TripRec<COMPACT>;
     constexpr int RUNS = 64 / B;
     const int ll = t * RUNS + q;
     const uint32_t okw = bcast<B>(L.ok, ll), cnt = bcast<B>(L.cnt, ll);
@@ -86,7 +104,7 @@
     tr.mshift = merged_trip_shift<B>(ok, cnt, ra0, rb0, tr.off);
     const bool two = !(a.dbg & 0x08u) && two_colour<B>(ok, cnt, ra0, rb0);
     tr.two = B == 64 ? two : (__any(two) != 0);
-    tr.ra = make_uint4(0, 0, 0, 0); tr.rb = make_uint4(0, 0, 0, 0); tr.rc = make_uint4(0, 0, 0, 0);
+    tr.ra = Rec(); tr.rb = Rec(); tr.rc = Rec();
     tr.fused = B == 64 && tr.mshift != 0 && colour == 0 && two && !(a.dbg & 0x100u);
     tr.twin = B == 64 && p == 0u && a.partners == 2u && (okw & 3u) == 3u && ((okw >> 8) & 3u) == 3u && !(a.dbg & 0x04u);
     const uint32_t rb1 = bcast<B>(L.rb1, ll);
@@ -99,7 +117,7 @@
         tr.sb = first + rb0 + tr.off + (((uint32_t)sub + ((okw >> 2) & 7u)) & 63u);
         const uint64_t sc = first + rb1 + tr.off + (((uint32_t)sub + ((okw >> 10) & 7u)) & 63u);
         tr.valid = true;
-        tr.ra = a.step_rec[tr.sa]; tr.rb = a.step_rec[tr.sb]; tr.rc = a.step_rec[sc];
+        tr.ra = Rec::load(a, tr.sa); tr.rb = Rec::load(a, tr.sb); tr.rc = Rec::load(a, sc);
         return;
     }
     if (tr.fused) {
@@ -107,12 +125,12 @@
         tr.sa = first + merged_trip_base(cnt, ra0, tr.off) + (uint32_t)sub;
         tr.sb = (uint64_t)((int64_t)tr.sa + tr.mshift);
         tr.valid = dst < 0 || dst > 63;
-        tr.ra = a.step_rec[tr.sa];
-        tr.rb = a.step_rec[tr.sb];
+        tr.ra = Rec::load(a, tr.sa);
+        tr.rb = Rec::load(a, tr.sb);
         return;
     }
     tr.valid = expand_run<B>(ok, first, cnt, ra0, rb0, sub, colour, tr.off, tr.sa, tr.sb);
-    if (tr.valid) { tr.ra = a.step_rec[tr.sa]; tr.rb = a.step_rec[tr.sb]; }
+    if (tr.valid) { tr.ra = Rec::load(a, tr.sa); tr.rb = Rec::load(a, tr.sb); }
 }
 
 __device__ __forceinline__ double term_move(const KArgs &a, double term_dist, double xi, double xj, int crowd) {
@@ -127,8 +145,8 @@
 
 __device__ __forceinline__ double shfl_f64(double v, int src) { return __shfl(v, src, 64); }
 
-template <bool ATOMIC_LOADS, bool TRACE>
-__device__ __forceinline__ bool fused_trip(const KArgs &a, TeamState &ts, const Trip &cur, const int lane,
+template <bool ATOMIC_LOADS, bool TRACE, bool COMPACT>
+__device__ __forceinline__ bool fused_trip(const KArgs &a, TeamState &ts, const Trip<COMPACT> &cur, const int lane,
                                            const uint32_t tid, const uint64_t wave_quota, uint64_t &wave_done) {
     double *x = a.x;
     const int s = cur.mshift, z = s < 0 ? -s : s;
@@ -136,14 +154,14 @@
     const bool out = cur.valid;
     const int dstc = out ? lane : dst, srcc = (src < 0 || src > 63) ? lane : src;
     const uint32_t grp = ((cur.off + (uint32_t)lane) / (uint32_t)z) & 1u;
-    const uint32_t node = cur.ra.x, pnode = cur.rb.x;
+    const uint32_t node = cur.ra.slot(), pnode = cur.rb.slot();
     double xo = 0.0, xp = 0.0;
     if (!(a.dbg & 2u)) {
         if (node != 0xFFFFFFFFu) xo = load_pos<ATOMIC_LOADS>(x + node);
         if (out && pnode != 0xFFFFFFFFu) xp = load_pos<ATOMIC_LOADS>(x + pnode);
     } else { xo = (double)node; xp = (double)pnode; }
-    const double term_dist = fabs(rec_pos(cur.ra) - rec_pos(cur.rb));
-    const int crowd = crowd_shift<true>(a, cur.ra, cur.rb);
+    const double term_dist = fabs(cur.ra.pos() - cur.rb.pos());
+    const int crowd = TripRec<COMPACT>::crowd(a, cur.ra, cur.rb);
     const bool term_ok = term_dist != 0.0 && node != 0xFFFFFFFFu && pnode != 0xFFFFFFFFu;
     double acc = 0.0;
     bool touched = false, second = true;
@@ -173,30 +191,30 @@
     return second;
 }
 
-template <bool ATOMIC_LOADS, bool TRACE>
-__device__ __forceinline__ bool twin_trip(const KArgs &a, TeamState &ts, const Trip &cur, const int lane,
+template <bool ATOMIC_LOADS, bool TRACE, bool COMPACT>
+__device__ __forceinline__ bool twin_trip(const KArgs &a, TeamState &ts, const Trip<COMPACT> &cur, const int lane,
                                           const uint32_t tid, const uint64_t wave_quota, uint64_t &wave_done) {
     double *x = a.x;
-    const uint32_t node = cur.ra.x, nb = cur.rb.x, nc = cur.rc.x;
+    const uint32_t node = cur.ra.slot(), nb = cur.rb.slot(), nc = cur.rc.slot();
     double xa = 0.0, xb = 0.0, xc = 0.0;
     if (!(a.dbg & 2u)) {
         if (node != 0xFFFFFFFFu) xa = load_pos<ATOMIC_LOADS>(x + node);
         if (nb != 0xFFFFFFFFu) xb = load_pos<ATOMIC_LOADS>(x + nb);
         if (nc != 0xFFFFFFFFu) xc = load_pos<ATOMIC_LOADS>(x + nc);
     } else { xa = (double)node; xb = (double)nb; xc = (double)nc; }
-    const double pa = rec_pos(cur.ra);
+    const double pa = cur.ra.pos();
     double acc = 0.0;
     bool touched = false, second = true;
 #pragma unroll
     for (uint32_t p = 0; p < 2u; ++p) {
         ++ts.att;
-        const uint4 &rp = p ? cur.rc : cur.rb;
+        const TripRec<COMPACT> &rp = p ? cur.rc : cur.rb;
         const uint32_t pn = p ? nc : nb;
-        const double term_dist = fabs(pa - rec_pos(rp));
+        const double term_dist = fabs(pa - rp.pos());
         const bool valid = quota_cut(term_dist != 0.0 && node != 0xFFFFFFFFu && pn != 0xFFFFFFFFu,
                                      lane, wave_quota, wave_done);
         if (valid) {
-            const double r_x = term_move(a, term_dist, xa, p ? xc : xb, crowd_shift<true>(a, cur.ra, rp));
+            const double r_x = term_move(a, term_dist, xa, p ? xc : xb, TripRec<COMPACT>::crowd(a, cur.ra, rp));
             ++ts.done;
             if (TRACE) record_trace(a, tid, ts.ntr, node, pn, term_dist);
             xa = xa - r_x;
@@ -209,9 +227,10 @@
     return second;
 }
 
-template <int B, bool LDS_TABLES, bool ATOMIC_LOADS, bool TRACE>
+template <int B, bool LDS_TABLES, bool ATOMIC_LOADS, bool TRACE, bool COMPACT = false>
 __device__ __forceinline__ void team_iteration(const KArgs &a, const uint4 *path_tab, const double *zeta_tab,
                                                TeamState &ts, const uint32_t tid, const uint64_t wave_quota, const IterConsts *itp = nullptr) {
+    static_assert(B == 64 || !COMPACT, "trip records are read by the trips of B = 64 only");
     const int lane = threadIdx.x & 63;
     const int sub = lane & (B - 1);
     const int q = lane / B;
@@ -234,7 +253,7 @@
         const Leader &L = ts.L;
         int t = B - (int)ts.left;
         uint32_t colour = ts.colour, seg = ts.seg, p = ts.p;
-        Trip cur;
+        Trip<COMPACT> cur;
         expand_trip<B>(a, L, t, seg, p, colour, sub, q, cur);
         for (;;) {
             int t_n = t; uint32_t colour_n = 0u, seg_n = seg, p_n = p;
@@ -243,7 +262,7 @@
             else if (seg + 1u < cur.k) { seg_n = seg + 1u; p_n = 0u; }
             else { t_n = t + 1; seg_n = 0u; p_n = 0u; }
             const bool have_n = t_n < B;
-            Trip nxt;
+            Trip<COMPACT> nxt;
             if (have_n) expand_trip<B>(a, L, t_n, seg_n, p_n, colour_n, sub, q, nxt);
             if (B == 64 && cur.twin) {
                 if (!twin_trip<ATOMIC_LOADS, TRACE>(a, ts, cur, lane, tid, wave_quota, wave_done)) {
@@ -271,13 +290,13 @@
             ts.colour = colour_n; ts.seg = seg_n; ts.p = p_n;
             if (t_n != t) --ts.left;
             bool valid = cur.valid;
-            const uint4 ra = cur.ra, rb = cur.rb;
+            const TripRec<COMPACT> ra = cur.ra, rb = cur.rb;
             const int mshift = cur.mshift;
             double term_dist = 0.0;
             uint32_t i = 0, j = 0;
             if (valid) {
-                term_dist = fabs(rec_pos(ra) - rec_pos(rb));
-                i = ra.x; j = rb.x;
+                term_dist = fabs(ra.pos() - rb.pos());
+                i = ra.slot(); j = rb.slot();
                 valid = term_dist != 0.0 && i != 0xFFFFFFFFu && j != 0xFFFFFFFFu;
             }
             valid = quota_cut(valid, lane, wave_quota, wave_done);
@@ -288,7 +307,7 @@
             }
             double r_x = 0.0;
             if (valid) {
-                r_x = term_move(a, term_dist, xi, xj, crowd_shift<true>(a, ra, rb));
+                r_x = term_move(a, term_dist, xi, xj, TripRec<COMPACT>::crowd(a, ra, rb));
                 ++ts.done;
                 if (TRACE) record_trace(a, tid, ts.ntr, i, j, term_dist);
             }
diff --git a/gfasort_amd/csrc/sgd_device.h b/gfasort_amd/csrc/sgd_device.h
--- a/gfasort_amd/csrc/sgd_device.h
+++ b/gfasort_amd/csrc/sgd_device.h
@@ -64,7 +64,10 @@
     double         *x;
     uint64_t       *rng;
     unsigned long long *counters;
-    void           *trace;
+    union {
+        void       *trace;
+        const uint2 *trip_rec;
+    };
     uint32_t       *trace_cnt;
     uint32_t       *lead;
     uint64_t n_steps, steps_thresh;
diff --git a/gfasort_amd/csrc/sgd_host.h b/gfasort_amd/csrc/sgd_host.h
--- a/gfasort_amd/csrc/sgd_host.h
+++ b/gfasort_amd/csrc/sgd_host.h
@@ -7,7 +7,7 @@
 
 namespace gfs {
 
-struct KernelShape { int dims; uint32_t bundle; bool lds_tables, atomic_loads, trace; };
+struct KernelShape { int dims; uint32_t bundle; bool lds_tables, atomic_loads, trace; bool compact = false; };
 
 template <typename... A> inline const void *kernel_addr(void (*k)(A...)) { return reinterpret_cast<const void *>(k); }
 template <typename F> inline auto with_flag(bool b, F f) { return b ? f(std::true_type{}) : f(std::false_type{}); }
diff --git a/gfasort_amd/csrc/sgd_kernels_1d.hip b/gfasort_amd/csrc/sgd_kernels_1d.hip
--- a/gfasort_amd/csrc/sgd_kernels_1d.hip
+++ b/gfasort_amd/csrc/sgd_kernels_1d.hip
@@ -46,7 +46,7 @@
 }
 
 
-template <int B, bool LDS_TABLES, bool ATOMIC_LOADS, bool TRACE>
+template <int B, bool LDS_TABLES, bool ATOMIC_LOADS, bool TRACE, bool COMPACT = false>
 __global__ void __attribute__((amdgpu_waves_per_eu(4, 4))) sgd1d_team_kernel(const KArgs a) {
     extern __shared__ __align__(16) unsigned char smem[];
     const uint4 *path_tab; const double *zeta_tab;
@@ -60,14 +60,14 @@
     load_pass(a, tid, ts, no_flips);
     const uint64_t wq = wave_quota_of(a, tid & ~63u);
     for (uint64_t done = 0; done < wq; done += a.chunk)
-        team_iteration<B, LDS_TABLES, ATOMIC_LOADS, TRACE>(a, path_tab, zeta_tab, ts, tid, wq - done < a.chunk ? wq - done : a.chunk);
+        team_iteration<B, LDS_TABLES, ATOMIC_LOADS, TRACE, COMPACT>(a, path_tab, zeta_tab, ts, tid, wq - done < a.chunk ? wq - done : a.chunk);
     store_rng(a, tid, ts.rng);
     if (TRACE) a.trace_cnt[tid] = ts.ntr;
     store_pass(a, tid, ts, 0u);
     flush_counters(a, ts.done, ts.att);
 }
 
-template <int B, bool LDS_TABLES, bool POOL>
+template <int B, bool LDS_TABLES, bool POOL, bool COMPACT = false>
 __global__ void __attribute__((amdgpu_waves_per_eu(4, 4))) sgd1d_team_fused_kernel(const KArgs a0, const IterConsts *its, const uint32_t n_iters,
                                                                                    uint32_t *pool) {
     constexpr bool ATOMIC_LOADS = true;
@@ -85,14 +85,14 @@
         const uint32_t wave = (uint32_t)__builtin_amdgcn_readfirstlane((int)(tid >> 6));
         pool_walk(a, its, n_iters, pool, pool_share(a0, wave, a0.n_streams >> 6), [&]() __attribute__((always_inline)) { return a0.chunk; },
                   [&](const uint32_t k, const uint32_t m) __attribute__((always_inline)) {
-            team_iteration<B, LDS_TABLES, ATOMIC_LOADS, false>(a, path_tab, zeta_tab, ts, tid, m, its + k);
+            team_iteration<B, LDS_TABLES, ATOMIC_LOADS, false, COMPACT>(a, path_tab, zeta_tab, ts, tid, m, its + k);
         });
     } else {
         const uint64_t wq = wave_quota_of(a, tid & ~63u);
         for (uint32_t k = 0; k < n_iters; ++k) {
             a.it = its[k];
             for (uint64_t done = 0; done < wq; done += a.chunk)
-                team_iteration<B, LDS_TABLES, ATOMIC_LOADS, false>(a, path_tab, zeta_tab, ts, tid, wq - done < a.chunk ? wq - done : a.chunk, its + k);
+                team_iteration<B, LDS_TABLES, ATOMIC_LOADS, false, COMPACT>(a, path_tab, zeta_tab, ts, tid, wq - done < a.chunk ? wq - done : a.chunk, its + k);
         }
     }
     store_rng(a, tid, ts.rng);
@@ -138,6 +138,10 @@
     return with_flag(pooled, [&](auto P) { return with_flag(s.lds_tables, [&](auto L) { return kernel_addr(sgd1d_team_fused_kernel<B, L(), P()>); }); });
 }
 const void *fused_kernel_1d(const KernelShape &s, bool pooled) {
+    if (s.compact) {
+        if (s.bundle != 64) return nullptr;
+        return with_flag(pooled, [&](auto P) { return with_flag(s.lds_tables, [&](auto L) { return kernel_addr(sgd1d_team_fused_kernel<64, L(), P(), true>); }); });
+    }
     switch (s.bundle) {
         case 16: return team_fused_kernel_1d<16>(s, pooled);
         case 32: return team_fused_kernel_1d<32>(s, pooled);
@@ -154,6 +158,10 @@
     }); }); });
 }
 const void *iteration_kernel_1d(const KernelShape &s) {
+    if (s.compact) {
+        if (s.bundle != 64 || s.trace) return nullptr;
+        return with_flag(s.lds_tables, [&](auto L) { return with_flag(s.atomic_loads, [&](auto A) { return kernel_addr(sgd1d_team_kernel<64, L(), A(), false, true>); }); });
+    }
     switch (s.bundle) {
         case 0: case 1:
             return with_flag(s.lds_tables, [&](auto L) { return with_flag(s.atomic_loads, [&](auto A) { return with_flag(s.trace, [&](auto T) {
diff --git a/gfasort_amd/hip.py b/gfasort_amd/hip.py
--- a/gfasort_amd/hip.py
+++ b/gfasort_amd/hip.py
@@ -15,6 +15,7 @@
 F_DBG_NO_ATOMICS, F_DBG_NO_XLOADS, F_DBG_ONE_COLOUR = 0x100, 0x200, 0x800
 F_DBG_NO_ALIGN, F_DBG_ALIGN_FIRST, F_DBG_WIDE_INDEX, F_DBG_NO_FUSED_TRIP = 0x1000, 0x2000, 0x4000, 0x8000
 F_ONE_PARTNER, F_DBG_NO_TWIN_TRIP, F_DBG_FREE_RUNNING = 0x10, 0x400, 0x20
+F_FULL_RECORDS = 0x80
 F_PHASED = 0x40
 
 
@@ -138,7 +139,7 @@
     "gfs_rank_positions_changed", "gfs_rank_get_positions", "gfs_rank_exchange_count", "gfs_rank_exchange_buffer",
     "gfs_rank_bind_exchange_buffer", "gfs_rank_window_begin", "gfs_rank_window_end", "gfs_rank_finish_begin",
     "gfs_rank_finish_buffer", "gfs_rank_finish_end", "gfs_rank_run",
-    "gfs_ctx_debug_step_records", "gfs_ctx_debug_kshift", "gfs_phase_window", "gfs_ctx_phase_window",
+    "gfs_ctx_debug_step_records", "gfs_ctx_debug_kshift", "gfs_ctx_record_bytes", "gfs_phase_window", "gfs_ctx_phase_window",
     "gfs_ctx_pair_errors", "gfs_stress_sample_pairs", "gfs_ctx_stress_of_pairs", "gfs_ctx_sort_quality", "gfs_pair_errors",
     "gfs_sort_quality_of", "gfs_batch_sort_quality",
     "gfs_ctx_path_errors", "gfs_ctx_stretched_pairs", "gfs_ctx_node_errors", "gfs_diagnose",
@@ -192,6 +193,8 @@
         L.gfs_ctx_node_layout.argtypes = [C.c_void_p, C.c_void_p, C.c_uint64]
         L.gfs_ctx_debug_step_records.argtypes = [C.c_void_p, C.c_void_p, C.c_uint64]
         L.gfs_ctx_debug_kshift.argtypes = [C.c_void_p, C.c_int32, C.c_void_p]
+        L.gfs_ctx_record_bytes.argtypes = [C.c_void_p]
+        L.gfs_ctx_record_bytes.restype = C.c_uint32
         L.gfs_phase_window.argtypes = [C.c_void_p, C.c_void_p, C.c_void_p]
         L.gfs_ctx_phase_window.argtypes = [C.c_void_p, C.c_int64, C.c_int64, C.c_void_p, C.c_void_p]
         L.gfs_ctx_setup_1d.argtypes = [C.c_void_p] + [C.c_void_p] * 4
@@ -704,6 +707,9 @@
         check(lib().gfs_ctx_debug_kshift(self._h, C.c_int32(-2 if set is None else int(set)), C.byref(v)))
         return int(v.value)
 
+    def record_bytes(self):
+        return int(lib().gfs_ctx_record_bytes(self._h))
+
     def phase_window(self, set_begin=-1, set_end=-1):
         b, e = C.c_uint64(0), C.c_uint64(0)
         check(lib().gfs_ctx_phase_window(self._h, C.c_int64(int(set_begin)), C.c_int64(int(set_end)), C.byref(b), C.byref(e)))
diff --git a/include/gfasort_hip.h b/include/gfasort_hip.h
--- a/include/gfasort_hip.h
+++ b/include/gfasort_hip.h
@@ -68,6 +68,7 @@
 #define GFS_F_NO_FUSE       4u
 #define GFS_F_ONE_PARTNER   0x10u
 #define GFS_F_PHASED        0x40u
+#define GFS_F_FULL_RECORDS  0x80u
 #define GFS_F_DBG_NO_TWIN_TRIP 0x400u
 #define GFS_F_DBG_FREE_RUNNING 0x20u
 #define GFS_F_DBG_NO_ATOMICS 0x100u
@@ -146,6 +147,7 @@
 int   gfs_ctx_trace(gfs_ctx *ctx, gfs_term *out, uint64_t n_terms, uint64_t *counts, uint64_t n_streams);
 int   gfs_ctx_debug_step_records(const gfs_ctx *ctx, uint32_t *out, uint64_t n_words);
 int   gfs_ctx_debug_kshift(gfs_ctx *ctx, int32_t set, int32_t *kshift_out);
+uint32_t gfs_ctx_record_bytes(const gfs_ctx *ctx);
 int   gfs_ctx_phase_window(gfs_ctx *ctx, int64_t set_begin, int64_t set_end, uint64_t *begin_out, uint64_t *end_out);
 
 typedef struct gfs_pair_error {
```

New measurement: 107.3 billion, median of 6. 2.7% higher.
